# tberriel/OVO

Hardware: AMD Instinct MI355X
Metric: frames/s (CLIP+SAM2+fusion+query), 640x480 ScanNet, 1/2/4/8 MI355X (higher is better)
Workload: dtype bf16; 1 GPU; BASELINE.json configs[2]: PE-Core-L14-336 TextRegion descriptors (2 x 336^2 crops of a 640x480 frame) + SAM2 hiera_b+ image encoder @1024^2 + back-projection + cull/project/match/vote on a 1000000-point map + multi-view fusion + dense per-point fusion + 10-prompt instance and dense-map query; every frame a keyframe; masks from the precomputed-mask seam (32/frame); map_points=1000000, texts=10, masks_per_frame=32, sam2=image encoder, masks=precomputed-mask seam (mask_generator.py:94-95), encoder_batch=14, dense_query=resident class map, rows touched by the keyframe re-evaluated, parallelism=single GPU, points_end=1366868, instances_end=242

## Files before the change

include/ovo_hip.h:

```cpp
#ifndef OVO_HIP_H
#define OVO_HIP_H

#include <stddef.h>
#include <stdint.h>

#ifdef __cplusplus
extern "C" {
#endif

#define OVO_OK 0
#define OVO_E_ARG (-1)
#define OVO_E_LAUNCH (-2)
#define OVO_E_UNSUPPORTED (-3)

typedef void *ovo_stream_t;

const char *ovo_hip_last_error(void);
int ovo_hip_abi_version(void);

int ovo_marker(int id, ovo_stream_t stream);
int ovo_profile_start(void);
int ovo_profile_stop(double *ms, double *work, int64_t *launches, int n_kinds);
int ovo_profile_bytes(double *bytes, int n_kinds);

// ... 91 lines not shown
} ovo_gemm_t;
int ovo_gemm(const ovo_gemm_t *g, ovo_stream_t stream);
typedef struct {
    const float *cos, *sin;
    int32_t T, hd, cols, t0;
} ovo_rope_t;
int ovo_gemm_rope(const ovo_gemm_t *g, const ovo_rope_t *rope, ovo_stream_t stream);
int ovo_gemm_periodic(const ovo_gemm_t *g, int64_t add_rows, ovo_stream_t stream);
typedef struct {
    int32_t B, H, W, wh, ww;
} ovo_window_t;
int ovo_gemm_unwindow(const ovo_gemm_t *g, const ovo_window_t *win, ovo_stream_t stream);
int ovo_gemm_rowln(const ovo_gemm_t *g, const ovo_window_t *win, const float *ln_g, const float *ln_b, float eps, void *ln_out, int64_t ld_ln,
                   ovo_stream_t stream);
int ovo_gemm_fold_out(const ovo_gemm_t *g, void *xb, int64_t ld_xb, float *stats, int64_t ld_stats, ovo_stream_t stream);
int ovo_gemm_fold_stats(const float *x, int64_t ldx, int M, int D, void *xb, int64_t ld_xb, float *stats, ovo_stream_t stream);
int ovo_gemm_fold_in(const ovo_gemm_t *g, const ovo_rope_t *rope, const float *stats, int64_t ld_stats, int parts, int D, const float *rowsum, float eps,
                     ovo_stream_t stream);
int ovo_gemm_f32a(const ovo_gemm_t *g, const ovo_window_t *win, const float *x, int d, const float *gamma, const float *beta,
                  float eps, int mode, int pool2x2, ovo_stream_t stream);
int ovo_mlp_f32(float *x, int64_t rows, int d, const float *ln_g, const float *ln_b, float eps, const void *w1, int64_t ldw1,
                const float *b1, int hidden, const void *w2, int64_t ldw2, const float *b2, ovo_stream_t stream);
int ovo_neck_f32(const float *x, int64_t rows, int d, const void *w1, int64_t ldw1, const float *b1, int hidden, const void *w2, int64_t ldw2,
                 const float *b2, float *out, int n_out, ovo_stream_t stream);
int ovo_window_attention_f32(const float *x, int B, int H, int W, int window, int d, int d_out, int heads, int pool, const float *ln_g,
                             const float *ln_b, float eps, const void *qkv_w, int64_t ldw, const float *qkv_b, void *att, int ld_att,
                             ovo_stream_t stream);
int ovo_gemm_argmax(const ovo_gemm_t *g, uint64_t *best, int store_scores, int n_valid, ovo_stream_t stream);
int ovo_decode_best(const uint64_t *best, int64_t n, float th, int64_t *out_cls, float *out_conf, ovo_stream_t stream);

typedef struct {
    const void *q, *k, *v;
    void *o;
    int64_t q_sb, q_sh, q_st, k_sb, k_sh, k_st, v_sb, v_sh, v_st, o_sb, o_sh, o_st;
    int32_t B, H, Tq, Tk, hd;
    float scale;
    int32_t causal;
} ovo_attention_t;
int ovo_attention(const ovo_attention_t *a, ovo_stream_t stream);

int ovo_gemm_fewrows(const ovo_gemm_t *g, ovo_stream_t stream);
int ovo_attention_short(const void *qkv, int B, int T, int H, int hd, float scale, void *out, ovo_stream_t stream);
int ovo_merge_clips(const float *logits, int64_t ld_logits, int per_row, const float *clips, int B, int D, float *out, ovo_stream_t stream);

int ovo_layernorm(const float *x, int64_t x_stride, int64_t rows, int d, const float *gamma, const float *beta,
                  float eps, void *y, int64_t y_stride, int out_dtype, ovo_stream_t stream);

int ovo_vit_embed(const float *patch, const float *prefix, int n_prefix, const float *pos, int B, int P, int d,
                  const float *gamma, const float *beta, float eps, float *x, ovo_stream_t stream);

int ovo_im2col(const float *img, int B, int C, int H, int W, int ksz, int stride, int pad, void *out, int kpad,
               ovo_stream_t stream);

int ovo_resize_normalize(const void *src, int src_dtype, int C, int H, int W, int y0, int x0, int ch, int cw,
                         float *out, int oh, int ow, int antialias, float scale, const float *mean3_host,
                         const float *std3_host, ovo_stream_t stream);

int ovo_resize_window_normalize(const void *src, int src_dtype, int C, int H, int W, int y0, int x0, int ch, int cw, float *out,
                                int oh, int ow, int virt_h, int virt_w, int top, int left, int filter, float scale,
                                const float *mean3_host, const float *std3_host, ovo_stream_t stream);
int ovo_resize_normalize_batch(const void *const *srcs_host, int n_src, int src_dtype, int C, int H, int W, const int32_t *crops_host, int n_crop,
                               float *out, int oh, int ow, int antialias, float scale, const float *mean3_host, const float *std3_host,
                               ovo_stream_t stream);

int ovo_mask_boxes(const uint8_t *masks, int n, int H, int W, int32_t *boxes_xywh, ovo_stream_t stream);
int ovo_mask_crops(const void *image, int img_dtype, int H, int W, const uint8_t *masks, const int32_t *boxes_xywh, int n,
                   int also_bbox, int margin, int R, int round_out, float *out, ovo_stream_t stream);

int ovo_rope_qk(void *qkv, int B, int T, int H, int hd, const float *cos_t, const float *sin_t, int t0,
                ovo_stream_t stream);

int ovo_feature_masks(const uint8_t *masks, int N, int H, int W, int gh, int gw, void *w, int gpad, float *cnt,
                      ovo_stream_t stream);

int ovo_stitch_tokens_t(const float *tokens, int tokens_per_crop, int t0, int d, int P, int nh, int nw, void *out,
                        int gpad, ovo_stream_t stream);

int ovo_unit_tokens(const void *x_t, int d, int G, int gpad, void *u_t, void *u, ovo_stream_t stream);
int ovo_global_patch_filter(const float *r_t, void *weights, int N, int G, int gpad, float th, float *cnt, ovo_stream_t stream);

int ovo_scale_rows_bf16(const float *x, const float *cnt, int N, int d, void *y, ovo_stream_t stream);
int ovo_l2_normalize_rows(const float *x, int64_t N, int d, float *y, ovo_stream_t stream);
int ovo_cast_f32(const float *x, int64_t n, void *y, int dtype, ovo_stream_t stream);

typedef struct {
    int32_t image_size, patch, width, layers, heads, mlp_dim, out_dim;
    int32_t n_prefix;
    int32_t act;
    int32_t pre_ln;
    int32_t use_rope;
    int32_t pool;
    int32_t kpad;
    float ln_eps;
    int32_t q_prescaled;
} ovo_vit_config_t;

typedef struct {
    const float *ln1_g, *ln1_b;
    const void *qkv_w; const float *qkv_b;
    const void *out_w; const float *out_b;
    const float *ln2_g, *ln2_b;
    const void *fc1_w; const float *fc1_b;
    const void *fc2_w; const float *fc2_b;
    const void *qkv_wf; const float *qkv_bf, *qkv_cs;
    const void *fc1_wf; const float *fc1_bf, *fc1_cs;
} ovo_vit_layer_t;

typedef struct {
    const void *patch_w; const float *patch_b;
    const float *prefix;
    const float *pos;
    const float *ln_pre_g, *ln_pre_b, *ln_post_g, *ln_post_b;
    const void *proj_w;
    const float *rope_cos, *rope_sin;
    const ovo_vit_layer_t *layers;
    const void *map_q;
    const void *map_kv_w; const float *map_kv_b;
    const void *map_proj_w; const float *map_proj_b;
    const float *map_ln_g, *map_ln_b;
    const void *map_fc1_w; const float *map_fc1_b;
    const void *map_fc2_w; const float *map_fc2_b;
} ovo_vit_weights_t;

size_t ovo_vit_workspace_bytes(const ovo_vit_config_t *cfg, int B);
int ovo_vit_forward(const ovo_vit_config_t *cfg, const ovo_vit_weights_t *w, const float *images, int B, float *out,
                    void *ws, size_t ws_bytes, ovo_stream_t stream);

typedef struct {
    int32_t image_size;
    int32_t dims[4], heads[4], blocks[4], window[4];
    int32_t n_global, global_blocks[8];
    int32_t fpn_dim;
    int32_t hi_res;
    float ln_eps;
    int32_t q_prescaled;
} ovo_hiera_config_t;

typedef struct {
    const float *ln1_g, *ln1_b;
    const void *qkv_w; const float *qkv_b;
    const void *out_w; const float *out_b;
    const float *ln2_g, *ln2_b;
    const void *fc1_w; const float *fc1_b;
    const void *fc2_w; const float *fc2_b;
    const void *res_w; const float *res_b;
} ovo_hiera_block_t;

typedef struct {
    const void *patch_w; const float *patch_b;
    const float *pos;
    const ovo_hiera_block_t *blocks;
    const void *neck_w[4]; const float *neck_b[4];
    const void *s0_w; const float *s0_b;
    const void *s1_w; const float *s1_b;
} ovo_hiera_weights_t;

size_t ovo_hiera_workspace_bytes(const ovo_hiera_config_t *cfg, int B);
int ovo_hiera_patch_embed(const float *images, int B, int S, int E, const void *patch_w, int ldw, const float *bias, const float *pos,
                          float *x, ovo_stream_t stream);
int ovo_hiera_forward(const ovo_hiera_config_t *cfg, const ovo_hiera_weights_t *w, const float *images, int B,
                      float *feat0, float *feat1, float *feat2, void *ws, size_t ws_bytes, ovo_stream_t stream);


int ovo_row_epilogue(const float *x, int64_t R, int C, const float *base, int64_t base_rows, const float *gamma, const float *beta,
                     float eps, const float *pe, int64_t pe_rows, float *y, void *y16, void *ype16, ovo_stream_t stream);

int ovo_sam_upscale_ln(const void *g, const float *bias, const float *feat, const float *gamma, const float *beta, float eps,
                       int64_t P, int s, int C1, void *out, ovo_stream_t stream);

int ovo_sam_upscale_masks(const void *g, const float *bias, const float *feat, const float *hyper, int n_mask, int first, int64_t P,
                          int s2, int C2, float *out, ovo_stream_t stream);

int ovo_sam_linear(const void *A, const void *W, const float *bias, const float *add, int64_t add_rows, int ld_add, void *C, int ldc, int64_t M,
                   int N, int K, ovo_stream_t stream);
int ovo_sam_proj_ln(const void *A, const void *W, const float *bias, const float *res, const void *res16, int64_t res_rows, const float *gamma, const float *beta,
                    float eps, const float *pe, int64_t pe_rows, float *y32, void *y16, void *ype16, int64_t M, int N, int K, ovo_stream_t stream);
int ovo_sam_up1_ln(const void *A, const void *W, const float *bias, const float *feat, const float *gamma, const float *beta, float eps,
                   int64_t P, int s, int C1, int K, void *out, ovo_stream_t stream);
int ovo_sam_up2_masks(const void *A, const void *W, const float *bias, const float *feat, const float *hyper, int n_mask, int first, int64_t P,
                      int s2, int C2, int K, float *out, ovo_stream_t stream);

int ovo_sam_i2t_attention(const void *q, int64_t q_batch_stride, int q_token_stride, const void *k, const void *v, void *o, int64_t P, int S, int T,
                          int H, float scale, ovo_stream_t stream);
int ovo_sam_t2i_attention(const void *q, const void *k, const void *v, int64_t kv_batch_stride, int kv_token_stride, void *o, int64_t P, int S, int T,
                          int H, float scale, ovo_stream_t stream);

int ovo_amg_mask_stats(const float *logits, int n, int h, int w, int H, int W, float thr, float offset, int32_t *stats,
                       ovo_stream_t stream);
int ovo_amg_binarize(const float *logits, const int32_t *sel, int n_sel, int h, int w, int H, int W, float thr, uint8_t *out,
                     ovo_stream_t stream);
int ovo_paint_segmap(const uint8_t *masks, int n, int64_t pixels, int32_t *seg, ovo_stream_t stream);


int ovo_instance_moments(const float *xyz, const int32_t *ins, int64_t n, int n_slots, double *sums, int32_t *cnt, ovo_stream_t stream);

int ovo_near_fraction(const float *pts_by_instance, const int64_t *offsets, const int32_t *pairs, int n_pairs, int64_t max_points_a,
                      float th, int32_t *near_count, ovo_stream_t stream);

int ovo_remap_instances(int32_t *ins, int64_t n, const int32_t *table, int n_slots, ovo_stream_t stream);

size_t ovo_map_reanchor_workspace_bytes(int K);
int ovo_map_reanchor(const float *xyz, const int32_t *ids, const int32_t *ins, const uint8_t *rgb, int64_t n_src, float *xyz_out, int32_t *ids_out,
                     int32_t *ins_out, uint8_t *rgb_out, int64_t cap_out, const int64_t *seg_src_host, const int64_t *seg_dst_host,
                     const float *seg_T_host, int K, void *ws, size_t ws_bytes, ovo_stream_t stream);

size_t ovo_dense_repack_workspace_bytes(int K);
int ovo_dense_repack(const float *acc, const int32_t *cnt, const int64_t *cls, const float *conf, int D, int src_shards, int64_t src_rows_local,
                     int64_t n_src, float *acc_out, int32_t *cnt_out, int64_t *cls_out, float *conf_out, int64_t rows_out, int shard_rank,
                     int shard_count, int shard_block, int64_t n_fill, int64_t empty_cls, float empty_conf, const int64_t *seg_src_host,
                     const int64_t *seg_dst_host, int K, void *ws, size_t ws_bytes, ovo_stream_t stream);

typedef struct {
    float w2c[16];
    float K[9];
// ... 122 lines not shown
```

ovo_amd/_lib.py:

```python
from __future__ import annotations

import ctypes as C
import os
from typing import Optional

import torch

_HERE = os.path.dirname(os.path.abspath(__file__))
SO_PATH = os.path.join(_HERE, "lib", "libovo_hip.so")
ABI_VERSION = 20
E_UNSUPPORTED = -3


class OvoHipError(RuntimeError):
    pass


class Camera(C.Structure):
    _fields_ = [("aabb", C.c_float * 6), ("planes", C.c_float * 24), ("w2c", C.c_float * 16),
                ("K", C.c_float * 9), ("th", C.c_float), ("h", C.c_int32), ("w", C.c_int32)]


class Ratio(C.Structure):
    _fields_ = [("enabled", C.c_int32), ("r_h", C.c_float), ("r_w", C.c_float), ("crop_edge", C.c_int32)]


_P, _I64, _I32, _F32, _SZ = C.c_void_p, C.c_int64, C.c_int, C.c_float, C.c_size_t
_CAM = C.POINTER(Camera)


class Gemm(C.Structure):
    _fields_ = [("A", _P), ("lda", _I64), ("W", _P), ("ldw", _I64), ("bias", _P), ("C", _P), ("ldc", _I64),
                ("add", _P), ("ld_add", _I64), ("M", C.c_int32), ("N", C.c_int32), ("K", C.c_int32),
                ("in_dtype", C.c_int32), ("out_dtype", C.c_int32), ("act", C.c_int32), ("alpha", _F32)]


class Rope(C.Structure):
    _fields_ = [("cos", _P), ("sin", _P), ("T", C.c_int32), ("hd", C.c_int32), ("cols", C.c_int32), ("t0", C.c_int32)]


class Window(C.Structure):
    _fields_ = [(n, C.c_int32) for n in ("B", "H", "W", "wh", "ww")]


class Attention(C.Structure):
    _fields_ = [("q", _P), ("k", _P), ("v", _P), ("o", _P)] + \
               [(n, _I64) for n in ("q_sb", "q_sh", "q_st", "k_sb", "k_sh", "k_st", "v_sb", "v_sh", "v_st", "o_sb", "o_sh", "o_st")] + \
               [(n, C.c_int32) for n in ("B", "H", "Tq", "Tk", "hd")] + [("scale", _F32), ("causal", C.c_int32)]


class VitConfig(C.Structure):
    _fields_ = [(n, C.c_int32) for n in ("image_size", "patch", "width", "layers", "heads", "mlp_dim", "out_dim", "n_prefix",
                                          "act", "pre_ln", "use_rope", "pool", "kpad")] + [("ln_eps", _F32), ("q_prescaled", C.c_int32)]


class VitLayer(C.Structure):
    _fields_ = [(n, _P) for n in ("ln1_g", "ln1_b", "qkv_w", "qkv_b", "out_w", "out_b", "ln2_g", "ln2_b",
                                   "fc1_w", "fc1_b", "fc2_w", "fc2_b",
                                   "qkv_wf", "qkv_bf", "qkv_cs", "fc1_wf", "fc1_bf", "fc1_cs")]


class VitWeights(C.Structure):
    _fields_ = [(n, _P) for n in ("patch_w", "patch_b", "prefix", "pos", "ln_pre_g", "ln_pre_b", "ln_post_g", "ln_post_b",
# ... 72 lines not shown
    "ovo_frustum_ids": (_I32, [_P, _I64, _CAM, _P, _P, _P, _SZ, _P]),
    "ovo_project_points": (_I32, [_P, _I64, _I32, _CAM, _P, _P]),
    "ovo_match_points": (_I32, [_P, _I64, _I32, _CAM, _P, _P, _P, _P, _P, _SZ, _P]),
    "ovo_depth_filter": (_I32, [_P, _I32, _I32, _I32, _F32, _F32, _P, _P]),
    "ovo_track_project": (_I32, [_P, _P, _I64, _CAM, _P, _P, _I32, _I32, Ratio, _P, _P, _I32, _I32, _P, _P]),
    "ovo_vote_stats": (_I32, [_P, _I32, _I32, _P, _I64, _P, _P]),
    "ovo_assign_instances": (_I32, [_P, _P, _I64, _P, _I32, _P, _P, _P]),
    "ovo_map_explained": (_I32, [_P, _I64, _CAM, _P, _P, _P]),
    "ovo_map_backproject": (_I32, [_P, _P, _P, _I32, _I32, _I32, _I32, _P, _P, _I64, _I32, _P, _P, _P, _P, _P, _P, _SZ, _P]),
    "ovo_map_step": (_I32, [C.POINTER(MapStep), _P]),
    "ovo_track_step": (_I32, [C.POINTER(TrackStep), _P]),
    "ovo_track_workspace_bytes": (_SZ, [_I32, _I32]),
    "ovo_keyframe_step": (_I32, [C.POINTER(MapStep), C.POINTER(TrackStep), _P]),
    "ovo_round_chain_params_bytes": (_SZ, []),
    "ovo_round_chain": (_I32, [C.POINTER(RoundChain), C.POINTER(MapStep), C.POINTER(TrackStep), _I32, _P]),
    "ovo_host_alloc": (_P, [_SZ]),
    "ovo_host_free": (None, [_P]),
    "ovo_host_wait32": (_I32, [_P, C.c_int32, _I64]),
    "ovo_host_wait64": (_I32, [_P, _I64, _I64]),
    "ovo_fuse_views": (_I32, [_P, _I32, _P, _P, _I32, _I32, _P, _P, _P, _P]),
    "ovo_fuse_views_add": (_I32, [_P, _I32, _P, _P, _P, _I32, _P, _P, _P, _P]),
    "ovo_scatter_accum": (_I32, [_P, _I64, _P, _I32, _P, _I32, _P, _P, _P]),
    "ovo_similarity": (_I32, [_P, _I32, _I64, _I32, _P, _I32, _P, _I32, _F32, _F32, _F32, _P, _P, _P, _P]),
    "ovo_similarity_rows": (_I32, [_P, _I32, _P, _P, _I64, _I32, _P, _I32, _P, _I32, _F32, _F32, _F32, _P, _P, _P]),
    "ovo_scatter_accum_touched": (_I32, [_P, _I64, _P, _I32, _P, _I32, _P, _P, _P, _P, _P, _I32, _I32, _I32, _P]),
    "ovo_scatter_accum_query": (_I32, [_P, _P, _I64, _P, _P, _I32, _P, _I32, _P, _P, _I32, _I32, _I32, _P, _I32, _I32, _F32, _F32, _F32, _P, _P, _P]),
    "ovo_mask_boxes": (_I32, [_P, _I32, _I32, _I32, _P, _P]),
    "ovo_mask_crops": (_I32, [_P, _I32, _I32, _I32, _P, _P, _I32, _I32, _I32, _I32, _I32, _P, _P]),
    "ovo_row_argmax": (_I32, [_P, _I64, _I32, _I32, _F32, _F32, _F32, _P, _P, _P]),
    "ovo_mask_intersections": (_I32, [_P, _I32, _I64, _P, _P]),
    "ovo_pack_masks": (_I32, [_P, _I32, _I64, _P, _I64, _P]),
    "ovo_unpack_masks": (_I32, [_P, _I32, _I64, _I64, _P, _P]),
    "ovo_mask_or": (_I32, [_P, _I64, _P, _I32, _P]),
    "ovo_gather_rows": (_I32, [_P, _I64, _P, _I32, _P, _P]),
    "ovo_mask_area": (_I32, [_P, _I64, _P, _I32, _P, _P]),
    "ovo_gemm": (_I32, [C.POINTER(Gemm), _P]),
    "ovo_gemm_argmax": (_I32, [C.POINTER(Gemm), _P, _I32, _I32, _P]),
    "ovo_gemm_rope": (_I32, [C.POINTER(Gemm), C.POINTER(Rope), _P]),
    "ovo_gemm_periodic": (_I32, [C.POINTER(Gemm), _I64, _P]),
    "ovo_gemm_unwindow": (_I32, [C.POINTER(Gemm), C.POINTER(Window), _P]),
    "ovo_gemm_fold_out": (_I32, [C.POINTER(Gemm), _P, _I64, _P, _I64, _P]),
    "ovo_gemm_fold_stats": (_I32, [_P, _I64, _I32, _I32, _P, _I64, _P, _P]),
    "ovo_gemm_fold_in": (_I32, [C.POINTER(Gemm), C.POINTER(Rope), _P, _I64, _I32, _I32, _P, _F32, _P]),
    "ovo_gemm_rowln": (_I32, [C.POINTER(Gemm), C.POINTER(Window), _P, _P, _F32, _P, _I64, _P]),
    "ovo_gemm_f32a": (_I32, [C.POINTER(Gemm), C.POINTER(Window), _P, C.c_int, _P, _P, C.c_float, C.c_int, C.c_int, _P]),
    "ovo_decode_best": (_I32, [_P, _I64, _F32, _P, _P, _P]),
    "ovo_attention": (_I32, [C.POINTER(Attention), _P]),
    "ovo_gemm_fewrows": (_I32, [C.POINTER(Gemm), _P]),
    "ovo_attention_short": (_I32, [_P, _I32, _I32, _I32, _I32, _F32, _P, _P]),
    "ovo_merge_clips": (_I32, [_P, _I64, _I32, _P, _I32, _I32, _P, _P]),
    "ovo_layernorm": (_I32, [_P, _I64, _I64, _I32, _P, _P, _F32, _P, _I64, _I32, _P]),
    "ovo_vit_embed": (_I32, [_P, _P, _I32, _P, _I32, _I32, _I32, _P, _P, _F32, _P, _P]),
    "ovo_im2col": (_I32, [_P, _I32, _I32, _I32, _I32, _I32, _I32, _I32, _P, _I32, _P]),
    "ovo_resize_normalize": (_I32, [_P, _I32, _I32, _I32, _I32, _I32, _I32, _I32, _I32, _P, _I32, _I32, _I32, _F32,
                                    C.POINTER(C.c_float), C.POINTER(C.c_float), _P]),
    "ovo_resize_normalize_batch": (_I32, [_P, _I32, _I32, _I32, _I32, _I32, _P, _I32, _P, _I32, _I32, _I32, _F32, _P, _P, _P]),
    "ovo_resize_window_normalize": (_I32, [_P, _I32, _I32, _I32, _I32, _I32, _I32, _I32, _I32, _P, _I32, _I32, _I32, _I32, _I32, _I32, _I32, _F32,
                                           C.POINTER(C.c_float), C.POINTER(C.c_float), _P]),
    "ovo_rope_qk": (_I32, [_P, _I32, _I32, _I32, _I32, _P, _P, _I32, _P]),
    "ovo_feature_masks": (_I32, [_P, _I32, _I32, _I32, _I32, _I32, _P, _I32, _P, _P]),
    "ovo_stitch_tokens_t": (_I32, [_P, _I32, _I32, _I32, _I32, _I32, _I32, _P, _I32, _P]),
    "ovo_unit_tokens": (_I32, [_P, _I32, _I32, _I32, _P, _P, _P]),
    "ovo_global_patch_filter": (_I32, [_P, _P, _I32, _I32, _I32, _F32, _P, _P]),
    "ovo_scale_rows_bf16": (_I32, [_P, _P, _I32, _I32, _P, _P]),
    "ovo_mlp_f32": (_I32, [_P, _I64, _I32, _P, _P, _F32, _P, _I64, _P, _I32, _P, _I64, _P, _P]),
    "ovo_neck_f32": (_I32, [_P, _I64, _I32, _P, _I64, _P, _I32, _P, _I64, _P, _P, _I32, _P]),
    "ovo_window_attention_f32": (_I32, [_P, _I32, _I32, _I32, _I32, _I32, _I32, _I32, _I32, _P, _P, _F32, _P, _I64, _P, _P, _I32, _P]),
    "ovo_l2_normalize_rows": (_I32, [_P, _I64, _I32, _P, _P]),
    "ovo_cast_f32": (_I32, [_P, _I64, _P, _I32, _P]),
    "ovo_row_epilogue": (_I32, [_P, _I64, _I32, _P, _I64, _P, _P, _F32, _P, _I64, _P, _P, _P, _P]),
    "ovo_sam_upscale_ln": (_I32, [_P, _P, _P, _P, _P, _F32, _I64, _I32, _I32, _P, _P]),
    "ovo_sam_upscale_masks": (_I32, [_P, _P, _P, _P, _I32, _I32, _I64, _I32, _I32, _P, _P]),
    "ovo_sam_linear": (_I32, [_P, _P, _P, _P, _I64, _I32, _P, _I32, _I64, _I32, _I32, _P]),
    "ovo_sam_proj_ln": (_I32, [_P, _P, _P, _P, _P, _I64, _P, _P, _F32, _P, _I64, _P, _P, _P, _I64, _I32, _I32, _P]),
    "ovo_sam_up1_ln": (_I32, [_P, _P, _P, _P, _P, _P, _F32, _I64, _I32, _I32, _I32, _P, _P]),
    "ovo_sam_up2_masks": (_I32, [_P, _P, _P, _P, _P, _I32, _I32, _I64, _I32, _I32, _I32, _P, _P]),
    "ovo_instance_moments": (_I32, [_P, _P, _I64, _I32, _P, _P, _P]),
    "ovo_near_fraction": (_I32, [_P, _P, _P, _I32, _I64, _F32, _P, _P]),
    "ovo_remap_instances": (_I32, [_P, _I64, _P, _I32, _P]),
    "ovo_map_reanchor_workspace_bytes": (_SZ, [_I32]),
    "ovo_map_reanchor": (_I32, [_P, _P, _P, _P, _I64, _P, _P, _P, _P, _I64, _P, _P, _P, _I32, _P, _SZ, _P]),
    "ovo_dense_repack_workspace_bytes": (_SZ, [_I32]),
    "ovo_dense_repack": (_I32, [_P, _P, _P, _P, _I32, _I32, _I64, _I64, _P, _P, _P, _P, _I64, _I32, _I32, _I32, _I64, _I64, _F32, _P, _P, _I32, _P, _SZ, _P]),
    "ovo_render_workspace_bytes": (_SZ, [_I32, _I32]),
    "ovo_render_points": (_I32, [_P, _I64, C.POINTER(View), _P, _P, _P, _SZ, _P]),
    "ovo_render_resolve": (_I32, [_P, _I32, _I32, _I64, _P, _P, C.c_uint32, _P, _P, _P, _P, _I32, _I64, _F32, _P, _P, _P, _P, _P, _P, _P]),
    "ovo_instance_geometry": (_I32, [_P, _P, _I64, _I32, _P, _P, _P, _P, _P, _P, _P]),
    "ovo_render_boxes_workspace_bytes": (_SZ, [_I32]),
    "ovo_render_boxes": (_I32, [_P, _P, _I32, C.POINTER(View), _F32, _P, _F32, _P, _P, _P, _SZ, _P]),
    "ovo_icp_pyramid_bytes": (_SZ, [_I32, _I32, _I32]),
    "ovo_icp_prepare": (_I32, [_P, C.POINTER(IcpFrame), _P, _SZ, _P]),
    "ovo_icp_align_workspace_bytes": (_SZ, []),
    "ovo_icp_align": (_I32, [_P, C.POINTER(IcpFrame), _P, C.POINTER(IcpFrame), C.POINTER(IcpAlign), _P, _P, _P, _SZ, _P]),
    "ovo_sam_i2t_attention": (_I32, [_P, _I64, _I32, _P, _P, _P, _I64, _I32, _I32, _I32, _F32, _P]),
    "ovo_sam_t2i_attention": (_I32, [_P, _P, _P, _I64, _I32, _P, _I64, _I32, _I32, _I32, _F32, _P]),
    "ovo_paint_segmap": (_I32, [_P, _I32, _I64, _P, _P]),
    "ovo_amg_mask_stats": (_I32, [_P, _I32, _I32, _I32, _I32, _I32, _F32, _F32, _P, _P]),
    "ovo_amg_binarize": (_I32, [_P, _P, _I32, _I32, _I32, _I32, _I32, _F32, _P, _P]),
    "ovo_vit_workspace_bytes": (_SZ, [C.POINTER(VitConfig), _I32]),
    "ovo_vit_forward": (_I32, [C.POINTER(VitConfig), C.POINTER(VitWeights), _P, _I32, _P, _P, _SZ, _P]),
    "ovo_hiera_workspace_bytes": (_SZ, [C.POINTER(HieraConfig), _I32]),
    "ovo_hiera_forward": (_I32, [C.POINTER(HieraConfig), C.POINTER(HieraWeights), _P, _I32, _P, _P, _P, _P, _SZ, _P]),
    "ovo_hiera_patch_embed": (_I32, [_P, _I32, _I32, _I32, _P, _I32, _P, _P, _P, _P]),
    "ovo_eval_cell_keys": (_I32, [_P, _I64, C.POINTER(EvalGrid), _P, _P]),
    "ovo_eval_grid_records": (_I32, [_P, _P, _I64, _P, _P]),
    "ovo_knn5_labels": (_I32, [_P, _P, _I64, C.POINTER(EvalGrid), _P, _P, _I64, _P, _P, _P, _P, _P, _P]),
    "ovo_confusion": (_I32, [_P, _P, _I64, _I32, C.POINTER(C.c_int64), _I32, _P, _P, _P]),
}

_lib: Optional[C.CDLL] = None


def exported_symbols():
    return sorted(_SIGNATURES)


def load() -> C.CDLL:
    global _lib
    if _lib is not None:
        return _lib
    if not os.path.exists(SO_PATH):
        raise OvoHipError(f"{SO_PATH} is missing: run `python -m ovo_amd.build` (needs hipcc). "
                          "ovo_amd has no CPU fallback.")
    lib = C.CDLL(SO_PATH)
    for name, (res, args) in _SIGNATURES.items():
        fn = getattr(lib, name)
        fn.restype, fn.argtypes = res, args
    if lib.ovo_hip_abi_version() != ABI_VERSION:
        raise OvoHipError(f"ABI mismatch: library {lib.ovo_hip_abi_version()} vs binding {ABI_VERSION}")
    _lib = lib
    return lib


def check(status: int) -> None:
    if status != 0:
        raise OvoHipError(f"libovo_hip error {status}: {load().ovo_hip_last_error().decode()}")


_raw_stream = getattr(torch._C, "_cuda_getCurrentRawStream", None)


def stream() -> C.c_void_p:
    if _raw_stream is not None:
        return C.c_void_p(_raw_stream(torch.cuda.current_device()))
    return C.c_void_p(torch.cuda.current_stream().cuda_stream)


def ptr(t: Optional[torch.Tensor]) -> C.c_void_p:
    if t is None:
        return C.c_void_p(0)
    return C.c_void_p(t.data_ptr())


def dev(t: torch.Tensor, dtype: torch.dtype, name: str = "tensor") -> torch.Tensor:
    if not t.is_cuda:
        raise OvoHipError(f"{name} must live on the GPU (got {t.device}); ovo_amd has no CPU path")
# ... 128 lines not shown
```

ovo_amd/csrc/core.hip:

```cpp
#include <stdarg.h>
#include <stdio.h>
#include <stdlib.h>

#include <string.h>

#include <atomic>
#include <chrono>
#include <vector>

#include "common.h"

static thread_local char g_err[512] = "";

void ovo_set_error(const char *fmt, ...) {
    va_list ap;
    va_start(ap, fmt);
    vsnprintf(g_err, sizeof(g_err), fmt, ap);
    va_end(ap);
}

namespace {
struct Rec { hipEvent_t a, b; int kind; double work, bytes; int shape[3], flags; int cslot; double per_item, fixed; };
struct Prof {
    bool on = false;
// ... 20 lines not shown
void ovo_prof_shape(int a, int b, int c) {
    if (!g_prof.on || g_prof.recs.empty()) return;
    Rec &r = g_prof.recs.back();
    r.shape[0] = a; r.shape[1] = b; r.shape[2] = c;
}
void ovo_prof_flags(int flags) {
    if (!g_prof.on || g_prof.recs.empty()) return;
    g_prof.recs.back().flags = flags;
}
void ovo_prof_bytes(double bytes) {
    if (!g_prof.on || g_prof.recs.empty()) return;
    g_prof.recs.back().bytes = bytes;
}
static double g_last_bytes[OVO_PROF_KINDS];
void ovo_prof_end(hipStream_t s) {
    if (!g_prof.on || g_prof.recs.empty()) return;
    (void)hipEventRecord(g_prof.recs.back().b, s);
}
void ovo_prof_count(const int32_t *device_count, double per_item, double fixed, hipStream_t s) {
    constexpr int SLOTS = 1 << 16;
    if (!g_prof.on || g_prof.recs.empty() || !device_count) return;
    if (!g_prof.counts && hipHostMalloc((void **)&g_prof.counts, SLOTS * sizeof(int32_t), hipHostMallocDefault) != hipSuccess) { g_prof.counts = nullptr; return; }
    if (g_prof.n_counts >= SLOTS) return;
    Rec &r = g_prof.recs.back();
    r.cslot = g_prof.n_counts++; r.per_item = per_item; r.fixed = fixed;
    (void)hipMemcpyAsync(g_prof.counts + r.cslot, device_count, sizeof(int32_t), hipMemcpyDeviceToHost, s);
}

template <typename T>
static int host_wait(const T *flag, T value, int64_t timeout_us) {
    OVO_REQUIRE(flag, "null flag");
    const volatile T *f = flag;
    const auto t0 = std::chrono::steady_clock::now();
    for (unsigned spin = 0;; ++spin) {
        if (*f == value) { std::atomic_thread_fence(std::memory_order_acquire); return OVO_OK; }
        if ((spin & 255) == 255 &&
            std::chrono::duration_cast<std::chrono::microseconds>(std::chrono::steady_clock::now() - t0).count() > timeout_us) {
            ovo_set_error("ovo_host_wait: timed out after %lld us (flag %lld, expected %lld)", (long long)timeout_us, (long long)*f, (long long)value);
            return OVO_E_LAUNCH;
        }
        __builtin_ia32_pause();
    }
}

__global__ void k_marker(int id, int *sink) { if (sink && id < 0) *sink = id; }

extern "C" {
int ovo_marker(int id, ovo_stream_t stream) {
    k_marker<<<1, 1, 0, (hipStream_t)stream>>>(id, nullptr);
    OVO_CHECK_LAUNCH();
    return OVO_OK;
}
const char *ovo_hip_last_error(void) { return g_err; }
int ovo_hip_abi_version(void) { return 20; }

int ovo_profile_start(void) {
    g_prof.recs.clear();
    g_prof.used = 0;
    g_prof.n_counts = 0;
    g_prof.on = true;
    return OVO_OK;
}

int ovo_profile_stop(double *ms, double *work, int64_t *launches, int n_kinds) {
    g_prof.on = false;
    OVO_REQUIRE(ms && work && launches && n_kinds > 0 && n_kinds <= OVO_PROF_KINDS, "bad argument");
    for (int i = 0; i < n_kinds; ++i) { ms[i] = 0; work[i] = 0; launches[i] = 0; }
    for (int i = 0; i < OVO_PROF_KINDS; ++i) g_last_bytes[i] = 0;
    OVO_HIP(hipDeviceSynchronize());
    FILE *dump = getenv("OVO_PROF_DUMP") ? fopen(getenv("OVO_PROF_DUMP"), "a") : nullptr;
    for (const Rec &r : g_prof.recs) {
        float t = 0.f;
        if (hipEventElapsedTime(&t, r.a, r.b) != hipSuccess || r.kind >= n_kinds) continue;
        double wk = r.work, by = r.bytes;
        if (r.cslot >= 0 && g_prof.counts) wk = by = r.per_item * (double)g_prof.counts[r.cslot] + r.fixed;
        ms[r.kind] += t; work[r.kind] += wk; launches[r.kind] += 1; g_last_bytes[r.kind] += by;
        if (dump) fprintf(dump, "%d %d %d %d %.0f %.4f %d\n", r.kind, r.shape[0], r.shape[1], r.shape[2], wk, t, r.flags);
    }
    if (dump) fclose(dump);
    g_prof.recs.clear();
    g_prof.used = 0;
    return OVO_OK;
}

int ovo_profile_bytes(double *bytes, int n_kinds) {
    OVO_REQUIRE(bytes && n_kinds > 0 && n_kinds <= OVO_PROF_KINDS, "bad argument");
    for (int i = 0; i < n_kinds; ++i) bytes[i] = g_last_bytes[i];
    return OVO_OK;
}

void *ovo_host_alloc(size_t bytes) {
    void *p = nullptr;
    if (hipHostMalloc(&p, bytes ? bytes : 1, hipHostMallocMapped | hipHostMallocCoherent) != hipSuccess) {
        ovo_set_error("ovo_host_alloc: hipHostMalloc(%zu) failed", bytes);
        return nullptr;
    }
    memset(p, 0, bytes);
    return p;
}
void ovo_host_free(void *p) { if (p) (void)hipHostFree(p); }

int ovo_host_wait32(const int32_t *flag, int32_t value, int64_t timeout_us) { return host_wait(flag, value, timeout_us); }
int ovo_host_wait64(const int64_t *flag, int64_t value, int64_t timeout_us) { return host_wait(flag, value, timeout_us); }
}
```

ovo_amd/csrc/encoder.hip:

```cpp
#include <hip/hip_fp16.h>

#include "common.h"

namespace {

__device__ __forceinline__ float bf2f(uint16_t v) { return __uint_as_float((uint32_t)v << 16); }
__device__ __forceinline__ uint16_t f2bf(float x) {
    const __bf16 h = (__bf16)x;
    return *(const uint16_t *)&h;
}
__device__ __forceinline__ uint2 pack4_bf16(float a, float b, float c, float d) {
    return make_uint2((uint32_t)f2bf(a) | ((uint32_t)f2bf(b) << 16), (uint32_t)f2bf(c) | ((uint32_t)f2bf(d) << 16));
}

__device__ __forceinline__ void ln_row_wide(const float *__restrict__ x, int d, const float *__restrict__ gamma,
                                            const float *__restrict__ beta, float eps, void *__restrict__ y, int out_bf16, int lane,
                                            const float *__restrict__ extra_add) {
    const int d4 = d >> 2;
    float s = 0.f;
    for (int i = lane; i < d4; i += 64) {
        float4 v = ((const float4 *)x)[i];
        if (extra_add) { const float4 e = ((const float4 *)extra_add)[i]; v.x += e.x; v.y += e.y; v.z += e.z; v.w += e.w; }
        s += (v.x + v.y) + (v.z + v.w);
    }
    const float mean = wave_sum(s) / (float)d;
    float q = 0.f;
    for (int i = lane; i < d4; i += 64) {
        float4 v = ((const float4 *)x)[i];
        if (extra_add) { const float4 e = ((const float4 *)extra_add)[i]; v.x += e.x; v.y += e.y; v.z += e.z; v.w += e.w; }
        const float a = v.x - mean, b = v.y - mean, c = v.z - mean, e2 = v.w - mean;
        q += (a * a + b * b) + (c * c + e2 * e2);
    }
    const float rstd = rsqrtf(wave_sum(q) / (float)d + eps);
    for (int i = lane; i < d4; i += 64) {
        float4 v = ((const float4 *)x)[i];
        if (extra_add) { const float4 e = ((const float4 *)extra_add)[i]; v.x += e.x; v.y += e.y; v.z += e.z; v.w += e.w; }
        const float4 g = ((const float4 *)gamma)[i], b = ((const float4 *)beta)[i];
        const float o0 = (v.x - mean) * rstd * g.x + b.x, o1 = (v.y - mean) * rstd * g.y + b.y;
        const float o2 = (v.z - mean) * rstd * g.z + b.z, o3 = (v.w - mean) * rstd * g.w + b.w;
        if (out_bf16) ((uint2 *)y)[i] = pack4_bf16(o0, o1, o2, o3);
        else ((float4 *)y)[i] = make_float4(o0, o1, o2, o3);
    }
}

template <int NV>
__device__ __forceinline__ void ln_row_regs(const float *__restrict__ x, int d, const float *__restrict__ gamma,
                                            const float *__restrict__ beta, float eps, void *__restrict__ y, int out_bf16, int lane,
                                            const float *__restrict__ extra_add) {
    const int d4 = d >> 2;
    float4 v[NV];
#pragma unroll
    for (int j = 0; j < NV; ++j) {
        const int i = lane + 64 * j;
        v[j] = i < d4 ? ((const float4 *)x)[i] : make_float4(0.f, 0.f, 0.f, 0.f);
    }
// ... 20 lines not shown
#pragma unroll
    for (int j = 0; j < NV; ++j) {
        const int i = lane + 64 * j;
        if (i < d4) {
            const float4 g = ((const float4 *)gamma)[i], b = ((const float4 *)beta)[i];
            const float o0 = (v[j].x - mean) * rstd * g.x + b.x, o1 = (v[j].y - mean) * rstd * g.y + b.y;
            const float o2 = (v[j].z - mean) * rstd * g.z + b.z, o3 = (v[j].w - mean) * rstd * g.w + b.w;
            if (out_bf16) ((uint2 *)y)[i] = pack4_bf16(o0, o1, o2, o3);
            else ((float4 *)y)[i] = make_float4(o0, o1, o2, o3);
        }
    }
}

__device__ __forceinline__ void ln_row(const float *__restrict__ x, int d, const float *__restrict__ gamma,
                                       const float *__restrict__ beta, float eps, void *__restrict__ y, int out_bf16, int lane,
                                       const float *__restrict__ extra_add = nullptr) {
    const int nv = ((d >> 2) + 63) >> 6;
    if (nv <= 2) ln_row_regs<2>(x, d, gamma, beta, eps, y, out_bf16, lane, extra_add);
    else if (nv <= 4) ln_row_regs<4>(x, d, gamma, beta, eps, y, out_bf16, lane, extra_add);
    else if (nv <= 8) ln_row_regs<8>(x, d, gamma, beta, eps, y, out_bf16, lane, extra_add);
    else ln_row_wide(x, d, gamma, beta, eps, y, out_bf16, lane, extra_add);
}

__global__ void __launch_bounds__(256) k_layernorm(const float *__restrict__ x, long long xs, long long rows, int d,
                                                   const float *__restrict__ gamma, const float *__restrict__ beta, float eps,
                                                   char *__restrict__ y, long long ys, int out_bf16) {
    const int lane = threadIdx.x & 63;
    const long long waves = (long long)gridDim.x * 4;
    for (long long r = (long long)blockIdx.x * 4 + (threadIdx.x >> 6); r < rows; r += waves)
        ln_row(x + r * xs, d, gamma, beta, eps, y + r * ys * (out_bf16 ? 2 : 4), out_bf16, lane);
}

__global__ void __launch_bounds__(256) k_vit_embed(const float *__restrict__ patch, const float *__restrict__ prefix, int n_prefix,
                                                   const float *__restrict__ pos, int B, int P, int d, const float *__restrict__ gamma,
                                                   const float *__restrict__ beta, float eps, float *__restrict__ x) {
    const int lane = threadIdx.x & 63;
    const int T = n_prefix + P;
    const long long rows = (long long)B * T, waves = (long long)gridDim.x * 4;
    for (long long r = (long long)blockIdx.x * 4 + (threadIdx.x >> 6); r < rows; r += waves) {
        const int b = (int)(r / T), t = (int)(r % T);
        const float *src = t < n_prefix ? prefix + (long long)t * d : patch + ((long long)b * P + (t - n_prefix)) * d;
        const float *pe = pos ? pos + (long long)t * d : nullptr;
        float *dst = x + r * d;
        if (gamma) ln_row(src, d, gamma, beta, eps, dst, 0, lane, pe);
        else
            for (int i = lane; i < (d >> 2); i += 64) {
                float4 v = ((const float4 *)src)[i];
                if (pe) { const float4 e = ((const float4 *)pe)[i]; v.x += e.x; v.y += e.y; v.z += e.z; v.w += e.w; }
                ((float4 *)dst)[i] = v;
            }
    }
}

__global__ void __launch_bounds__(256) k_im2col(const float *__restrict__ img, int B, int C, int H, int W, int ksz, int stride, int pad,
                                                int oh, int ow, uint16_t *__restrict__ out, int kpad) {
    const uint32_t k8 = (uint32_t)kpad >> 3;
    const uint32_t total = (uint32_t)B * oh * ow * k8;
    const int kk = ksz * ksz, kreal = C * kk;
    for (uint32_t i = blockIdx.x * blockDim.x + threadIdx.x; i < total; i += gridDim.x * blockDim.x) {
        const uint32_t row = i / k8, kb = (i - row * k8) * 8;
        const uint32_t t1 = row / (uint32_t)ow, ox = row - t1 * (uint32_t)ow;
        const uint32_t b = t1 / (uint32_t)oh, oy = t1 - b * (uint32_t)oh;
        int c = (int)(kb / (uint32_t)kk), rem = (int)kb - c * kk, ky = rem / ksz, kx = rem - ky * ksz;
        const int y0 = (int)oy * stride - pad, x0 = (int)ox * stride - pad;
        uint16_t v[8];
#pragma unroll
        for (int e = 0; e < 8; ++e) {
            float f = 0.f;
            if ((int)kb + e < kreal) {
                const int y = y0 + ky, x = x0 + kx;
                if (y >= 0 && y < H && x >= 0 && x < W) f = img[(((long long)b * C + c) * H + y) * W + x];
            }
            v[e] = f2bf(f);
            if (++kx == ksz) { kx = 0; if (++ky == ksz) { ky = 0; ++c; } }
        }
        uint4 p;
        p.x = v[0] | ((uint32_t)v[1] << 16); p.y = v[2] | ((uint32_t)v[3] << 16); p.z = v[4] | ((uint32_t)v[5] << 16); p.w = v[6] | ((uint32_t)v[7] << 16);
        *(uint4 *)(out + (long long)row * kpad + kb) = p;
    }
}

struct ResizeArgs {
    const void *src; int src_u8, hwc; int C, H, W, y0, x0, ch, cw, oh, ow, aa;
    int vh, vw, top, left;
    float scale, mean[4], std[4];
};
__device__ __forceinline__ float src_px(const ResizeArgs &a, int c, int y, int x) {
    const long long i = a.hwc ? ((long long)(a.y0 + y) * a.W + (a.x0 + x)) * a.C + c : ((long long)c * a.H + (a.y0 + y)) * a.W + (a.x0 + x);
    return a.src_u8 ? (float)((const uint8_t *)a.src)[i] : ((const float *)a.src)[i];
}
typedef uint32_t __attribute__((aligned(1))) u32_unaligned;
__device__ __forceinline__ void src_px_all(const ResizeArgs &a, int y, int x, float (&v)[4]) {
    if (a.hwc && a.src_u8 && a.C == 3) {
        const long long i = ((long long)(a.y0 + y) * a.W + (a.x0 + x)) * 3;
        const uint8_t *p = (const uint8_t *)a.src + i;
        if (i + 4 <= (long long)a.H * a.W * 3) {
            const uint32_t w = *(const u32_unaligned *)p;
            v[0] = (float)(w & 0xffu); v[1] = (float)((w >> 8) & 0xffu); v[2] = (float)((w >> 16) & 0xffu);
        } else { v[0] = (float)p[0]; v[1] = (float)p[1]; v[2] = (float)p[2]; }
        return;
    }
    for (int c = 0; c < a.C; ++c) v[c] = src_px(a, c, y, x);
}
__device__ __forceinline__ float tri(float x) { x = fabsf(x); return x < 1.f ? 1.f - x : 0.f; }
__device__ __forceinline__ float cubic_aa(float x) {
    x = fabsf(x);
    if (x < 1.f) return ((1.5f * x - 2.5f) * x) * x + 1.f;
    if (x < 2.f) return (((x - 5.f) * x + 8.f) * x - 4.f) * -0.5f;
    return 0.f;
}
__device__ __forceinline__ float aa_filter(int kind, float x) { return kind == 2 ? cubic_aa(x) : tri(x); }

template <int T>
__device__ __forceinline__ void aa_taps(const ResizeArgs &a, int ymin, int xmin, int ny, int nx, float cy, float cx, float ivy, float ivx, float wy_tot,
                                        float wx_tot, float (&v)[4]) {
    float wy[T], wx[T];
#pragma unroll
    for (int i = 0; i < T; ++i) {
        wy[i] = i < ny ? aa_filter(a.aa, ((float)(ymin + i) - cy + 0.5f) * ivy) / wy_tot : 0.f;
        wx[i] = i < nx ? aa_filter(a.aa, ((float)(xmin + i) - cx + 0.5f) * ivx) / wx_tot : 0.f;
    }
#pragma unroll
    for (int iy = 0; iy < T; ++iy) {
        if (iy >= ny) break;
        float rowacc[4] = {0.f, 0.f, 0.f, 0.f};
#pragma unroll
        for (int ix = 0; ix < T; ++ix) {
            if (ix >= nx) break;
            float px[4];
            src_px_all(a, ymin + iy, xmin + ix, px);
            for (int c = 0; c < a.C; ++c) rowacc[c] += wx[ix] * px[c];
        }
        for (int c = 0; c < a.C; ++c) v[c] += wy[iy] * rowacc[c];
    }
}

#define OVO_RS_TAPS 10
__device__ __forceinline__ void resize_norm_body(const ResizeArgs &a, float *__restrict__ out) {
    const int wx_ = blockIdx.x * 64 + (threadIdx.x & 63), wy_ = blockIdx.y * 4 + (threadIdx.x >> 6);
    if (wx_ >= a.ow || wy_ >= a.oh) return;
    const int ox = wx_ + a.left, oy = wy_ + a.top;
    const float sy = (float)a.ch / (float)a.vh, sx = (float)a.cw / (float)a.vw;
    float v[4] = {0.f, 0.f, 0.f, 0.f};
    if (!a.aa) {
        float fy = sy * ((float)oy + 0.5f) - 0.5f; fy = fy < 0.f ? 0.f : fy;
        float fx = sx * ((float)ox + 0.5f) - 0.5f; fx = fx < 0.f ? 0.f : fx;
        const int y0 = (int)fy, x0 = (int)fx;
        const int y1 = y0 + (y0 < a.ch - 1 ? 1 : 0), x1 = x0 + (x0 < a.cw - 1 ? 1 : 0);
        const float ly = fy - (float)y0, lx = fx - (float)x0;
        float p00[4], p01[4], p10[4], p11[4];
        src_px_all(a, y0, x0, p00); src_px_all(a, y0, x1, p01); src_px_all(a, y1, x0, p10); src_px_all(a, y1, x1, p11);
        for (int c = 0; c < a.C; ++c)
            v[c] = (1.f - ly) * ((1.f - lx) * p00[c] + lx * p01[c]) + ly * ((1.f - lx) * p10[c] + lx * p11[c]);
    } else {
        const float half = a.aa == 2 ? 2.f : 1.f;
        const float supy = (sy >= 1.f ? sy : 1.f) * half, supx = (sx >= 1.f ? sx : 1.f) * half;
        const float ivy = sy >= 1.f ? 1.f / sy : 1.f, ivx = sx >= 1.f ? 1.f / sx : 1.f;
        const float cy = sy * ((float)oy + 0.5f), cx = sx * ((float)ox + 0.5f);
        int ymin = (int)(cy - supy + 0.5f); ymin = ymin < 0 ? 0 : ymin;
        int ymax = (int)(cy + supy + 0.5f); ymax = ymax > a.ch ? a.ch : ymax;
        int xmin = (int)(cx - supx + 0.5f); xmin = xmin < 0 ? 0 : xmin;
        int xmax = (int)(cx + supx + 0.5f); xmax = xmax > a.cw ? a.cw : xmax;
        float wy_tot = 0.f, wx_tot = 0.f;
        for (int y = ymin; y < ymax; ++y) wy_tot += aa_filter(a.aa, ((float)y - cy + 0.5f) * ivy);
        for (int x = xmin; x < xmax; ++x) wx_tot += aa_filter(a.aa, ((float)x - cx + 0.5f) * ivx);
        const int ny = ymax - ymin, nx = xmax - xmin;
        const int bound = (int)(2.f * (supy > supx ? supy : supx)) + 1;
        if (bound <= 3 && ny <= 3 && nx <= 3) aa_taps<3>(a, ymin, xmin, ny, nx, cy, cx, ivy, ivx, wy_tot, wx_tot, v);
        else if (bound <= 6 && ny <= 6 && nx <= 6) aa_taps<6>(a, ymin, xmin, ny, nx, cy, cx, ivy, ivx, wy_tot, wx_tot, v);
        else if (ny <= OVO_RS_TAPS && nx <= OVO_RS_TAPS) {
            aa_taps<OVO_RS_TAPS>(a, ymin, xmin, ny, nx, cy, cx, ivy, ivx, wy_tot, wx_tot, v);
        } else {
            for (int c = 0; c < a.C; ++c) {
                float acc = 0.f;
                for (int y = ymin; y < ymax; ++y) {
                    const float wyy = aa_filter(a.aa, ((float)y - cy + 0.5f) * ivy) / wy_tot;
                    float rowacc = 0.f;
                    for (int x = xmin; x < xmax; ++x) rowacc += (aa_filter(a.aa, ((float)x - cx + 0.5f) * ivx) / wx_tot) * src_px(a, c, y, x);
                    acc += wyy * rowacc;
                }
                v[c] = acc;
            }
        }
    }
    for (int c = 0; c < a.C; ++c) out[((long long)c * a.oh + wy_) * a.ow + wx_] = (v[c] * a.scale - a.mean[c]) / a.std[c];
}
__global__ void __launch_bounds__(256) k_resize_norm(ResizeArgs a, float *__restrict__ out) { resize_norm_body(a, out); }

constexpr int RESIZE_BATCH_MAX = 64;
struct ResizeBatch { const void *src[RESIZE_BATCH_MAX]; int y0[RESIZE_BATCH_MAX], x0[RESIZE_BATCH_MAX], ch[RESIZE_BATCH_MAX], cw[RESIZE_BATCH_MAX]; };
__global__ void __launch_bounds__(256) k_resize_norm_batch(ResizeArgs a, ResizeBatch b, float *__restrict__ out) {
    const int z = blockIdx.z;
    a.src = b.src[z]; a.y0 = b.y0[z]; a.x0 = b.x0[z]; a.ch = b.ch[z]; a.cw = b.cw[z];
    resize_norm_body(a, out + (long long)z * a.C * a.oh * a.ow);
}

template <int T>
__global__ void __launch_bounds__(256) k_resize_tri_hwc3(ResizeArgs a, ResizeBatch b, float *__restrict__ out) {
    const int z = blockIdx.z;
    const uint8_t *src = (const uint8_t *)b.src[z];
    const int y0c = b.y0[z], x0c = b.x0[z], ch = b.ch[z], cw = b.cw[z];
    const int wx_ = blockIdx.x * 64 + (threadIdx.x & 63), wy_ = blockIdx.y * 4 + (threadIdx.x >> 6);
    if (wx_ >= a.ow || wy_ >= a.oh) return;
    const int ox = wx_ + a.left, oy = wy_ + a.top;
    const float sy = (float)ch / (float)a.vh, sx = (float)cw / (float)a.vw;
    const float supy = sy >= 1.f ? sy : 1.f, supx = sx >= 1.f ? sx : 1.f;
    const float ivy = sy >= 1.f ? 1.f / sy : 1.f, ivx = sx >= 1.f ? 1.f / sx : 1.f;
    const float cy = sy * ((float)oy + 0.5f), cx = sx * ((float)ox + 0.5f);
    int ymin = (int)(cy - supy + 0.5f); ymin = ymin < 0 ? 0 : ymin;
    int ymax = (int)(cy + supy + 0.5f); ymax = ymax > ch ? ch : ymax;
    int xmin = (int)(cx - supx + 0.5f); xmin = xmin < 0 ? 0 : xmin;
    int xmax = (int)(cx + supx + 0.5f); xmax = xmax > cw ? cw : xmax;
    float wy[T], wx[T], wy_tot = 0.f, wx_tot = 0.f;
#pragma unroll
    for (int i = 0; i < T; ++i) {
        wy[i] = ymin + i < ymax ? tri(((float)(ymin + i) - cy + 0.5f) * ivy) : 0.f;
        wx[i] = xmin + i < xmax ? tri(((float)(xmin + i) - cx + 0.5f) * ivx) : 0.f;
        wy_tot += wy[i]; wx_tot += wx[i];
    }
#pragma unroll
    for (int i = 0; i < T; ++i) { wy[i] = wy[i] / wy_tot; wx[i] = wx[i] / wx_tot; }
    const long long last = (long long)a.H * a.W * 3 - 4;
    float v0 = 0.f, v1 = 0.f, v2 = 0.f;
#pragma unroll
    for (int iy = 0; iy < T; ++iy) {
        int y = ymin + iy; y = y < ch - 1 ? y : ch - 1;
        const long long row = (long long)(y0c + y) * a.W + x0c;
        float r0 = 0.f, r1 = 0.f, r2 = 0.f;
#pragma unroll
        for (int ix = 0; ix < T; ++ix) {
            int x = xmin + ix; x = x < cw - 1 ? x : cw - 1;
            const long long off = (row + x) * 3;
            uint32_t w;
            if (off <= last) w = *(const u32_unaligned *)(src + off);
            else w = (uint32_t)src[off] | ((uint32_t)src[off + 1] << 8) | ((uint32_t)src[off + 2] << 16);
            r0 += wx[ix] * (float)(w & 0xffu); r1 += wx[ix] * (float)((w >> 8) & 0xffu); r2 += wx[ix] * (float)((w >> 16) & 0xffu);
        }
        v0 += wy[iy] * r0; v1 += wy[iy] * r1; v2 += wy[iy] * r2;
    }
    float *o = out + (long long)z * 3 * a.oh * a.ow + (long long)wy_ * a.ow + wx_;
    const long long plane = (long long)a.oh * a.ow;
    o[0] = (v0 * a.scale - a.mean[0]) / a.std[0];
    o[plane] = (v1 * a.scale - a.mean[1]) / a.std[1];
    o[2 * plane] = (v2 * a.scale - a.mean[2]) / a.std[2];
}
inline int resize_tap_bound(int ch, int cw, int vh, int vw) {
    const float sy = (float)ch / (float)vh, sx = (float)cw / (float)vw;
    const float supy = sy >= 1.f ? sy : 1.f, supx = sx >= 1.f ? sx : 1.f;
    return (int)(2.f * (supy > supx ? supy : supx)) + 1;
}
inline void launch_resize_batch(const ResizeArgs &a, const ResizeBatch &b, int nz, float *out, hipStream_t s) {
    dim3 grid((a.ow + 63) / 64, (a.oh + 3) / 4, nz);
    int bound = 0;
    for (int z = 0; z < nz; ++z) { const int t = resize_tap_bound(b.ch[z], b.cw[z], a.vh, a.vw); bound = t > bound ? t : bound; }
    const bool generic = ovo_knob_set("OVO_RESIZE_GENERIC");
    if (!generic && a.hwc && a.src_u8 && a.C == 3 && a.aa == 1 && bound <= 3) k_resize_tri_hwc3<3><<<grid, 256, 0, s>>>(a, b, out);
    else if (!generic && a.hwc && a.src_u8 && a.C == 3 && a.aa == 1 && bound <= 6) k_resize_tri_hwc3<6><<<grid, 256, 0, s>>>(a, b, out);
    else k_resize_norm_batch<<<grid, 256, 0, s>>>(a, b, out);
}

__global__ void __launch_bounds__(256) k_mask_boxes(const uint8_t *__restrict__ masks, int H, int W, int32_t *__restrict__ boxes) {
    __shared__ int s[4];
    if (threadIdx.x == 0) { s[0] = W; s[1] = H; s[2] = -1; s[3] = -1; }
    __syncthreads();
    const uint8_t *m = masks + (long long)blockIdx.x * H * W;
    int x0 = W, y0 = H, x1 = -1, y1 = -1;
    for (int i = threadIdx.x; i < H * W; i += blockDim.x) {
        if (m[i]) {
            const int y = i / W, x = i - y * W;
            x0 = x < x0 ? x : x0; x1 = x > x1 ? x : x1; y0 = y < y0 ? y : y0; y1 = y > y1 ? y : y1;
        }
    }
    if (x1 >= 0) { atomicMin(&s[0], x0); atomicMin(&s[1], y0); atomicMax(&s[2], x1); atomicMax(&s[3], y1); }
    __syncthreads();
    if (threadIdx.x == 0) {
        int32_t *b = boxes + 4 * blockIdx.x;
        if (s[2] < 0) { b[0] = b[1] = b[2] = b[3] = 0; }
        else { b[0] = s[0]; b[1] = s[1]; b[2] = s[2] - s[0]; b[3] = s[3] - s[1]; }
    }
}

struct CropArgs {
    const void *img; int img_u8, H, W;
    const uint8_t *masks; const int32_t *boxes;
    int n, also_bbox, margin, R, round_out;
};
__global__ void __launch_bounds__(256) k_mask_crops(CropArgs a, float *__restrict__ out) {
    const int ox = blockIdx.x * 64 + (threadIdx.x & 63), oy = blockIdx.y * 4 + (threadIdx.x >> 6);
    const int parts = a.also_bbox ? 2 : 1, i = blockIdx.z / parts, part = blockIdx.z % parts;
    if (ox >= a.R || oy >= a.R) return;
    const int32_t *b = a.boxes + 4 * i;
    int bx = b[0], by = b[1], bw = b[2], bh = b[3];
    int ch, cw, offy = 0, offx = 0;
    const uint8_t *mask = nullptr;
    if (part == 0) {
        mask = a.masks + (long long)i * a.H * a.W;
        if (a.also_bbox) { ch = bh; cw = bw; }
        else {
            ch = cw = bh > bw ? bh : bw;
            if (bh > bw) offx = (bh - bw) / 2; else offy = (bw - bh) / 2;
        }
    } else {
        bx -= a.margin; by -= a.margin; bw += 2 * a.margin; bh += 2 * a.margin;
        if (bx < 0) { bw += bx; bx = 0; }
        if (by < 0) { bh += by; by = 0; }
        if (bx + bw > a.W) bw = a.W - bx;
        if (by + bh > a.H) bh = a.H - by;
        ch = bh; cw = bw;
    }
    float *o = out + ((long long)(i * parts + part) * 3) * a.R * a.R + (long long)oy * a.R + ox;
    const long long plane = (long long)a.R * a.R;
// ... 178 lines not shown

__global__ void __launch_bounds__(256) k_cast(const float4 *__restrict__ x, long long n4, uint2 *__restrict__ y, int dtype) {
    for (long long i = (long long)blockIdx.x * blockDim.x + threadIdx.x; i < n4; i += (long long)gridDim.x * blockDim.x) {
        const float4 v = x[i];
        if (dtype == 2) y[i] = pack4_bf16(v.x, v.y, v.z, v.w);
        else {
            const __half2 a = __floats2half2_rn(v.x, v.y), b = __floats2half2_rn(v.z, v.w);
            y[i] = make_uint2(*(const uint32_t *)&a, *(const uint32_t *)&b);
        }
    }
}

}

extern "C" {

int ovo_layernorm(const float *x, int64_t x_stride, int64_t rows, int d, const float *gamma, const float *beta, float eps,
                  void *y, int64_t y_stride, int out_dtype, ovo_stream_t stream) {
    OVO_REQUIRE(rows >= 0 && d > 0 && d % 4 == 0, "d must be a multiple of 4");
    OVO_REQUIRE(out_dtype == 0 || out_dtype == 2, "out_dtype: 0 = f32, 2 = bf16");
    if (rows == 0) return OVO_OK;
    OVO_REQUIRE(x && gamma && beta && y && x_stride % 4 == 0 && y_stride % 4 == 0, "null pointer / misaligned stride");
    k_layernorm<<<ovo_grid(rows * 64, 256), 256, 0, (hipStream_t)stream>>>(x, x_stride, rows, d, gamma, beta, eps, (char *)y,
                                                                          y_stride, out_dtype == 2);
    OVO_CHECK_LAUNCH();
    return OVO_OK;
}

int ovo_vit_embed(const float *patch, const float *prefix, int n_prefix, const float *pos, int B, int P, int d,
                  const float *gamma, const float *beta, float eps, float *x, ovo_stream_t stream) {
    OVO_REQUIRE(patch && x && B > 0 && P > 0 && d > 0 && d % 4 == 0 && n_prefix >= 0, "bad argument");
    OVO_REQUIRE(n_prefix == 0 || prefix, "prefix tokens missing");
    OVO_REQUIRE((gamma == nullptr) == (beta == nullptr), "gamma and beta go together");
    k_vit_embed<<<ovo_grid((long long)B * (n_prefix + P) * 64, 256), 256, 0, (hipStream_t)stream>>>(patch, prefix, n_prefix, pos, B, P, d,
                                                                                                    gamma, beta, eps, x);
    OVO_CHECK_LAUNCH();
    return OVO_OK;
}

int ovo_im2col(const float *img, int B, int C, int H, int W, int ksz, int stride, int pad, void *out, int kpad,
               ovo_stream_t stream) {
    OVO_REQUIRE(img && out && B > 0 && C > 0 && H > 0 && W > 0 && ksz > 0 && stride > 0 && pad >= 0, "bad argument");
    OVO_REQUIRE(kpad >= C * ksz * ksz && kpad % 32 == 0, "kpad must cover C*k*k and be a multiple of 32");
    const int oh = (H + 2 * pad - ksz) / stride + 1, ow = (W + 2 * pad - ksz) / stride + 1;
    OVO_REQUIRE(oh > 0 && ow > 0, "empty output");
    OVO_REQUIRE(kpad % 8 == 0 && ((uintptr_t)out & 15) == 0, "kpad must be a multiple of 8 and the output 16-byte aligned");
    OVO_REQUIRE((long long)B * oh * ow * (kpad / 8) < (1ll << 32) - (1ll << 22), "more than 2^32 16-byte pieces: split the batch");
    k_im2col<<<ovo_grid((long long)B * oh * ow * (kpad / 8), 256), 256, 0, (hipStream_t)stream>>>(img, B, C, H, W, ksz, stride, pad, oh, ow,
                                                                                                 (uint16_t *)out, kpad);
    OVO_CHECK_LAUNCH();
    return OVO_OK;
}

int ovo_resize_window_normalize(const void *src, int src_dtype, int C, int H, int W, int y0, int x0, int ch, int cw, float *out,
                                int oh, int ow, int virt_h, int virt_w, int top, int left, int filter, float scale,
                                const float *mean3_host, const float *std3_host, ovo_stream_t stream) {
    OVO_REQUIRE(src && out && (src_dtype == 0 || src_dtype == 3 || src_dtype == 4), "src_dtype: 0 = f32 [C,H,W], 3 = u8 [C,H,W], 4 = u8 [H,W,C]");
    OVO_REQUIRE(C >= 1 && C <= 4 && ch > 0 && cw > 0 && oh > 0 && ow > 0, "bad shape");
    OVO_REQUIRE(y0 >= 0 && x0 >= 0 && y0 + ch <= H && x0 + cw <= W, "crop outside the image");
    OVO_REQUIRE(top >= 0 && left >= 0 && top + oh <= virt_h && left + ow <= virt_w, "window outside the resized image");
    OVO_REQUIRE(filter >= 0 && filter <= 2, "filter: 0 = bilinear, 1 = antialiased bilinear, 2 = antialiased bicubic");
    ResizeArgs a;
    a.src = src; a.src_u8 = src_dtype >= 3; a.hwc = src_dtype == 4; a.C = C; a.H = H; a.W = W; a.y0 = y0; a.x0 = x0; a.ch = ch; a.cw = cw;
    a.oh = oh; a.ow = ow; a.aa = filter; a.scale = scale;
    a.vh = virt_h; a.vw = virt_w; a.top = top; a.left = left;
    for (int c = 0; c < 4; ++c) { a.mean[c] = mean3_host && c < C ? mean3_host[c] : 0.f; a.std[c] = std3_host && c < C ? std3_host[c] : 1.f; }
    if (a.hwc && a.src_u8 && C == 3 && filter == 1) {
        ResizeBatch b = {};
        b.src[0] = src; b.y0[0] = y0; b.x0[0] = x0; b.ch[0] = ch; b.cw[0] = cw;
        launch_resize_batch(a, b, 1, out, (hipStream_t)stream);
    } else {
        dim3 grid((ow + 63) / 64, (oh + 3) / 4);
        k_resize_norm<<<grid, 256, 0, (hipStream_t)stream>>>(a, out);
    }
    OVO_CHECK_LAUNCH();
    return OVO_OK;
}

int ovo_resize_normalize(const void *src, int src_dtype, int C, int H, int W, int y0, int x0, int ch, int cw, float *out,
                         int oh, int ow, int antialias, float scale, const float *mean3_host, const float *std3_host,
                         ovo_stream_t stream) {
    return ovo_resize_window_normalize(src, src_dtype, C, H, W, y0, x0, ch, cw, out, oh, ow, oh, ow, 0, 0, antialias, scale, mean3_host,
                                       std3_host, stream);
}

int ovo_resize_normalize_batch(const void *const *srcs_host, int n_src, int src_dtype, int C, int H, int W, const int32_t *crops_host, int n_crop, float *out,
                               int oh, int ow, int antialias, float scale, const float *mean3_host, const float *std3_host, ovo_stream_t stream) {
    OVO_REQUIRE(srcs_host && crops_host && out && n_src > 0 && n_crop > 0, "null / empty argument");
    OVO_REQUIRE(src_dtype == 0 || src_dtype == 3 || src_dtype == 4, "src_dtype: 0 = f32 [C,H,W], 3 = u8 [C,H,W], 4 = u8 [H,W,C]");
    OVO_REQUIRE(C >= 1 && C <= 4 && oh > 0 && ow > 0 && antialias >= 0 && antialias <= 2, "bad shape");
    ResizeArgs a;
    a.src = nullptr; a.src_u8 = src_dtype >= 3; a.hwc = src_dtype == 4; a.C = C; a.H = H; a.W = W; a.y0 = a.x0 = 0; a.ch = H; a.cw = W;
    a.oh = oh; a.ow = ow; a.aa = antialias; a.scale = scale; a.vh = oh; a.vw = ow; a.top = 0; a.left = 0;
    for (int c = 0; c < 4; ++c) { a.mean[c] = mean3_host && c < C ? mean3_host[c] : 0.f; a.std[c] = std3_host && c < C ? std3_host[c] : 1.f; }
    for (int k = 0; k < n_crop; ++k) {
        const int32_t *r = crops_host + 4 * k;
        OVO_REQUIRE(r[2] > 0 && r[3] > 0 && r[0] >= 0 && r[1] >= 0 && r[0] + r[2] <= H && r[1] + r[3] <= W, "crop outside the image");
    }
    const int total = n_src * n_crop;
    for (int z0 = 0; z0 < total; z0 += RESIZE_BATCH_MAX) {
        const int nz = total - z0 < RESIZE_BATCH_MAX ? total - z0 : RESIZE_BATCH_MAX;
        ResizeBatch b;
        for (int z = 0; z < nz; ++z) {
            const int i = (z0 + z) / n_crop, k = (z0 + z) % n_crop;
            OVO_REQUIRE(srcs_host[i], "null source image");
            b.src[z] = srcs_host[i]; b.y0[z] = crops_host[4 * k]; b.x0[z] = crops_host[4 * k + 1]; b.ch[z] = crops_host[4 * k + 2]; b.cw[z] = crops_host[4 * k + 3];
// ... 104 lines not shown
```

ovo_amd/csrc/hiera.hip:

```cpp
#include <algorithm>
#include "gemm_common.h"

namespace {

__device__ __forceinline__ uint16_t f2bf(float x) {
    const __bf16 h = (__bf16)x;
    return *(const uint16_t *)&h;
}
__device__ __forceinline__ float bf2f(uint16_t v) { return __uint_as_float((uint32_t)v << 16); }

struct Grid {
    int B, H, W, ws;
    int nwh, nww, wh, ww;
    long long rows;
};
__host__ __device__ inline Grid make_grid(int B, int H, int W, int ws) {
    Grid g; g.B = B; g.H = H; g.W = W; g.ws = ws;
    if (ws > 0) { g.wh = g.ww = ws; g.nwh = (H + ws - 1) / ws; g.nww = (W + ws - 1) / ws; }
    else { g.wh = H; g.ww = W; g.nwh = g.nww = 1; }
    g.rows = (long long)B * g.nwh * g.nww * g.wh * g.ww;
    return g;
}
__device__ __forceinline__ long long row_of(const Grid &g, int b, int y, int x) {
    const int wy = y / g.wh, wx = x / g.ww;
    return ((((long long)b * g.nwh + wy) * g.nww + wx) * g.wh + (y - wy * g.wh)) * g.ww + (x - wx * g.ww);
}

template <int LPR, int NV>
__global__ void __launch_bounds__(256) k_ln_window(const float *__restrict__ x, Grid g, int d, int kp, const float *__restrict__ gamma,
                                                   const float *__restrict__ beta, float eps, uint16_t *__restrict__ out) {
    constexpr int RPW = 64 / LPR;
    const int lane = threadIdx.x & 63, sl = lane % LPR, sub = lane / LPR;
    const uint32_t waves = gridDim.x * 4u;
    const int d4 = d >> 2, kp4 = kp >> 2;
    const uint32_t per_win = (uint32_t)(g.wh * g.ww), n_rows = (uint32_t)g.rows;
    const uint32_t n_iter = (n_rows + RPW - 1) / RPW;
    for (uint32_t it = blockIdx.x * 4u + (threadIdx.x >> 6); it < n_iter; it += waves) {
        uint32_t r = it * RPW + sub;
        if (LPR == 64) r = __builtin_amdgcn_readfirstlane(r);
        bool real = r < n_rows;
        const float *src = x;
        if (real) {
            const uint32_t win = r / per_win, in = r - win * per_win;
            const uint32_t ly = in / (uint32_t)g.ww, lx = in - ly * (uint32_t)g.ww;
            const uint32_t q2 = win / (uint32_t)g.nww, wx = win - q2 * (uint32_t)g.nww;
            const uint32_t b = q2 / (uint32_t)g.nwh, wy = q2 - b * (uint32_t)g.nwh;
            const int y = (int)(wy * g.wh + ly), xx = (int)(wx * g.ww + lx);
            if (y >= g.H || xx >= g.W) {
                uint2 *o = (uint2 *)(out + (long long)r * kp);
                for (int i = sl; i < kp4; i += LPR) o[i] = make_uint2(0, 0);
                real = false;
            } else src = x + (((long long)b * g.H + y) * g.W + xx) * d;
        }
        float4 v[NV];
// ... 154 lines not shown
}

inline int padk(int v) { return (v + 63) / 64 * 64; }
inline size_t align256(size_t v) { return (v + 255) & ~(size_t)255; }

struct BlockShape {
    int din, dout, kin, kout, heads, hd, H, Ho;
    bool pool; int stage_end;
    Grid g, go, gi;
    long long n_win, tok_out, att_rows; int tk, tq;
    size_t n_x, n_h, n_qkv, n_att, n_u, n_tmp, n_cast;
};
struct Plan {
    int n_blocks, S4;
    Grid level[2];
    size_t n_col, n_cast, n_lat[4];
    BlockShape b[64];
};

int make_plan(const ovo_hiera_config_t &c, int B, Plan &p) {
    int idx = 0, H = p.S4 = c.image_size / 4;
    const size_t tok0 = (size_t)B * H * H;
    p.level[0] = make_grid(B, H, H, 0); p.level[1] = make_grid(B, H / 2, H / 2, 0);
    p.n_col = tok0 * 192; p.n_cast = tok0 * c.fpn_dim;
    for (int s = 0; s < 4; ++s) p.n_lat[s] = (tok0 >> (2 * s)) * c.fpn_dim;
    for (int s = 0; s < 4; ++s)
        for (int b = 0; b < c.blocks[s]; ++b) {
            if (idx >= 64) return -1;
            BlockShape &k = p.b[idx];
            const bool first = k.pool = s > 0 && b == 0;
            k.din = first ? c.dims[s - 1] : c.dims[s]; k.dout = c.dims[s]; k.kin = padk(k.din); k.kout = padk(k.dout);
            k.heads = c.heads[s]; k.hd = k.heads > 0 ? k.dout / k.heads : 0;
            int ws = first ? c.window[s - 1] : c.window[s];
            for (int j = 0; j < c.n_global; ++j) if (c.global_blocks[j] == idx) ws = 0;
            k.H = H;
            k.Ho = H = first ? H / 2 : H;
            k.stage_end = b == c.blocks[s] - 1 ? s : -1;
            k.g = make_grid(B, k.H, k.H, ws); k.go = make_grid(B, H, H, ws > 0 ? (first ? ws / 2 : ws) : 0); k.gi = make_grid(B, H, H, 0);
            k.n_win = (long long)B * k.g.nwh * k.g.nww; k.tk = k.g.wh * k.g.ww; k.tq = first ? k.tk / 4 : k.tk;
            k.tok_out = (long long)B * H * H; k.att_rows = k.n_win * k.tq;
            const size_t rows = (size_t)k.g.rows, tin = (size_t)B * k.H * k.H, tout = (size_t)k.tok_out;
            k.n_x = std::max(tin * k.din, tout * k.dout);
            k.n_h = std::max(rows * k.kin, tout * k.kout);
            k.n_qkv = rows * 3 * k.dout; k.n_tmp = rows * k.dout;
            k.n_att = (first ? rows / 4 : rows) * k.kout;
            k.n_u = tout * 4 * k.dout; k.n_cast = tout * k.kout;
            ++idx;
        }
    p.n_blocks = idx;
    return 0;
}
struct Ws {
    uint16_t *col; float *x, *xr, *tmp; uint16_t *h, *qkv, *qp, *att, *u, *cast; float *lat[4];
    size_t bytes;
};

bool neck_fused(const ovo_hiera_config_t &c, int B, int s) {
    if (!c.hi_res || s > 1 || ovo_knob_set("OVO_HIERA_NECK_TWO_PASS")) return false;
    const long long rows = ((long long)B * (c.image_size / 4) * (c.image_size / 4)) >> (2 * s);
    return ovo_gemm_detail::neck_stream_covers(rows, c.dims[s], padk(c.dims[s]), c.fpn_dim, s == 0 ? 32 : 64);
}

Ws carve(const ovo_hiera_config_t &c, const Plan &p, int B, void *base) {
    size_t max_x = 0, max_h = 0, max_qkv = 0, max_att = 0, max_u = 0, max_tmp = 0, max_cast = p.n_cast;
    for (int i = 0; i < p.n_blocks; ++i) {
        const BlockShape &k = p.b[i];
        max_x = std::max(max_x, k.n_x); max_h = std::max(max_h, k.n_h); max_qkv = std::max(max_qkv, k.n_qkv); max_att = std::max(max_att, k.n_att);
        max_u = std::max(max_u, k.n_u); max_tmp = std::max(max_tmp, k.n_tmp); max_cast = std::max(max_cast, k.n_cast);
    }
    Ws w; size_t off = 0;
    auto take = [&](size_t n) { char *r = base ? (char *)base + off : nullptr; off += align256(n); return r; };
    w.col = (uint16_t *)take(p.n_col * 2); w.x = (float *)take(max_x * 4); w.xr = (float *)take(max_x * 4); w.tmp = (float *)take(max_tmp * 4);
    w.h = (uint16_t *)take(max_h * 2); w.qkv = (uint16_t *)take(max_qkv * 2);
    w.qp = (uint16_t *)take(max_att * 2); w.att = (uint16_t *)take(max_att * 2);
    w.u = (uint16_t *)take(max_u * 2); w.cast = (uint16_t *)take(max_cast * 2);
    for (int s = 0; s < 4; ++s) w.lat[s] = neck_fused(c, B, s) ? nullptr : (float *)take(p.n_lat[s] * 4);
    w.bytes = off;
    return w;
}

ovo_gemm_t gemm_desc(const void *A, long long lda, const void *W, long long ldw, const float *bias, void *C, long long ldc, int out_dtype,
                     const float *add, long long ld_add, long long M, int N, int K, int act) {
    ovo_gemm_t g;
    g.A = A; g.lda = lda; g.W = W; g.ldw = ldw; g.bias = bias; g.C = C; g.ldc = ldc; g.add = add; g.ld_add = ld_add;
    g.M = (int)M; g.N = N; g.K = K; g.in_dtype = 2; g.out_dtype = out_dtype; g.act = act; g.alpha = 1.0f;
    return g;
}
ovo_window_t window_of(const Grid &g) { return {g.B, g.H, g.W, g.wh, g.ww}; }

#define TRY(call) do { const int rc__ = (call); if (rc__ != OVO_OK) return rc__; } while (0)
#define TRY_FUSED(ran, call) \
    do { const int rc__ = (call); if (rc__ != OVO_OK && rc__ != OVO_E_UNSUPPORTED) return rc__; (ran) = rc__ == OVO_OK; } while (0)
#define LAUNCHED() OVO_CHECK_LAUNCH()

int gemm(const void *A, long long lda, const void *W, long long ldw, const float *bias, void *C, long long ldc, int out_dtype,
         const float *add, long long ld_add, long long M, int N, int K, int act, ovo_stream_t s) {
    const ovo_gemm_t g = gemm_desc(A, lda, W, ldw, bias, C, ldc, out_dtype, add, ld_add, M, N, K, act);
    return ovo_gemm(&g, s);
}

int gemm_from_f32(const float *x, const Grid &g, int d, int kp, const float *gamma, const float *beta, float eps, int mode, uint16_t *h, bool &h_done,
                  const void *W, const float *bias, void *C, long long ldc, int out_dtype, int N, int act, ovo_stream_t s) {
    const ovo_gemm_t q = gemm_desc(h, kp, W, kp, bias, C, ldc, out_dtype, nullptr, 0, g.rows, N, kp, act);
    if (!h_done) {
        const ovo_window_t w = window_of(g); bool streamed;
        TRY_FUSED(streamed, ovo_gemm_detail::gemm_f32a_stream(&q, g.ws > 0 ? &w : nullptr, x, d, gamma, beta, eps, mode, 0, s));
        if (streamed) return OVO_OK;
        OVO_REQUIRE(d <= 2048 && g.rows < (1ll << 31), "LayerNorm rows of more than 2048 columns / more than 2^31 rows");
        if (mode == 1) launch_ln_window(x, g, d, kp, gamma, beta, eps, h, (hipStream_t)s);
        else k_cast_pad<<<ovo_grid(g.rows * kp, 256), 256, 0, (hipStream_t)s>>>(x, g.rows, d, kp, h);
        h_done = true;
    }
    return ovo_gemm(&q, s);
}

constexpr int PE_TH = 8, PE_TW = 32, PE_IH = 4 * PE_TH + 3, PE_RS = 136, PE_WS = 200;
template <int NT>
__global__ void __launch_bounds__(512) __attribute__((amdgpu_waves_per_eu(4, 4))) k_patch_embed7(const float *__restrict__ img, int S, const uint16_t *__restrict__ w, int ldw,
                                                      const float *__restrict__ bias, const float *__restrict__ pos, float *__restrict__ out, int B,
                                                      int n_tiles) {
    using namespace ovo_gemm_detail;
    constexpr int E = 16 * NT;
    extern __shared__ __attribute__((aligned(16))) unsigned char pe_lds[];
    uint16_t *s_img = (uint16_t *)pe_lds;
    uint16_t *s_w = s_img + 3 * PE_IH * PE_RS;
    const int S4 = S >> 2, tiles_x = S4 / PE_TW, n_pos = tiles_x * (S4 / PE_TH);
    for (int i = threadIdx.x; i < E * 24; i += 512) {
        const int e = i / 24, r = i - 24 * e;
        uint4 p = make_uint4(0u, 0u, 0u, 0u);
        if (r < 21) {
            const uint16_t *q = w + (long long)e * ldw + 7 * r;
            const uint32_t w0 = q[0], w1 = q[1], w2 = q[2], w3 = q[3], w4 = q[4], w5 = q[5], w6 = q[6];
            p.x = w0 << 16; p.y = w1 | (w2 << 16); p.z = w3 | (w4 << 16); p.w = w5 | (w6 << 16);
        }
        *(uint4 *)(s_w + e * PE_WS + 8 * r) = p;
    }
    for (int i = threadIdx.x; i < 3 * PE_IH; i += 512) s_img[i * PE_RS] = 0;
    const int lane = threadIdx.x & 63, wave = threadIdx.x >> 6, g = lane >> 4, l16 = lane & 15;
    constexpr int NV = (3 * PE_IH * 32 + 511) / 512;
    float4 v[NV];
    float h;
    auto load_tile = [&](int t) {
        const int tt = t % n_pos, b = t / n_pos;
        const int oy0 = (tt / tiles_x) * PE_TH, ox0 = (tt % tiles_x) * PE_TW;
        const int y_first = 4 * oy0 - 3, x_first = 4 * ox0 - 3;
        const float *src = img + (long long)b * 3 * S * S;
        const float *col0 = src + 4 * ox0 + 4 * (threadIdx.x & 31);
#pragma unroll
        for (int j = 0; j < NV; ++j) {
            int row = (threadIdx.x >> 5) + 16 * j;
            if (row > 3 * PE_IH - 1) row = 3 * PE_IH - 1;
            const int c = row / PE_IH, y = y_first + (row - c * PE_IH);
            const int yc = y < 0 ? 0 : (y > S - 1 ? S - 1 : y);
            const float4 u = *(const float4 *)(col0 + (c * S + yc) * S);
            const bool ok = y == yc;
            v[j].x = ok ? u.x : 0.f; v[j].y = ok ? u.y : 0.f; v[j].z = ok ? u.z : 0.f; v[j].w = ok ? u.w : 0.f;
        }
        {
            int row = threadIdx.x / 3;
            const int col = threadIdx.x - 3 * row;
            if (row > 3 * PE_IH - 1) row = 3 * PE_IH - 1;
            const int c = row / PE_IH, y = y_first + (row - c * PE_IH), x = x_first + col;
            const int yc = y < 0 ? 0 : (y > S - 1 ? S - 1 : y), xc = x < 0 ? 0 : x;
            const float u = src[(c * S + yc) * S + xc];
            h = (y == yc && x == xc) ? u : 0.f;
        }
    };
    if ((int)blockIdx.x < n_tiles) load_tile(blockIdx.x);
    for (int t = blockIdx.x; t < n_tiles; t += gridDim.x) {
        const int tt = t % n_pos, b = t / n_pos;
        const int oy0 = (tt / tiles_x) * PE_TH, ox0 = (tt % tiles_x) * PE_TW;
        __syncthreads();
        f32x4 acc[2][NT];
#pragma unroll
        for (int m = 0; m < 2; ++m) {
            const long long tok = (long long)(oy0 + wave) * S4 + ox0 + 16 * m + l16;
#pragma unroll
            for (int n = 0; n < NT; ++n) acc[m][n] = *(const f32x4 *)(pos + tok * E + 16 * n + 4 * g);
        }
#pragma unroll
        for (int j = 0; j < NV; ++j) {
            const int row = (threadIdx.x >> 5) + 16 * j;
            if (16 * j + 15 < 3 * PE_IH || row < 3 * PE_IH) {
                uint2 p;
                p.x = f2bf(v[j].x) | ((uint32_t)f2bf(v[j].y) << 16); p.y = f2bf(v[j].z) | ((uint32_t)f2bf(v[j].w) << 16);
                *(uint2 *)(s_img + row * PE_RS + 4 + 4 * (threadIdx.x & 31)) = p;
            }
        }
        {
            const int i = threadIdx.x, row = i / 3, col = i - 3 * row;
            if (row < 3 * PE_IH) s_img[row * PE_RS + 1 + col] = f2bf(h);
        }
        __syncthreads();
#pragma unroll
        for (int n = 0; n < NT; ++n) {
            const f32x4 bb = *(const f32x4 *)(bias + 16 * n + 4 * g);
#pragma unroll
            for (int m = 0; m < 2; ++m) acc[m][n] += bb;
        }
        if (t + (int)gridDim.x < n_tiles) load_tile(t + gridDim.x);
#pragma unroll 1
        for (int s = 0; s < 6; ++s) {
            int r = 4 * s + g;
            if (r > 20) r = 20;
            const int c = r / 7, ky = r - 7 * c;
            bf16x8 pb[2];
#pragma unroll
            for (int m = 0; m < 2; ++m) {
                const int oy = wave, ox = 16 * m + l16;
                const uint2 *q = (const uint2 *)(s_img + (c * PE_IH + 4 * oy + ky) * PE_RS + 4 * ox);
                const uint2 lo = q[0], hi = q[1];
                uint4 u; u.x = lo.x; u.y = lo.y; u.z = hi.x; u.w = hi.y;
                pb[m] = *(const bf16x8 *)&u;
            }
#pragma unroll
            for (int n = 0; n < NT; ++n) {
                const bf16x8 wa = *(const bf16x8 *)(s_w + (16 * n + l16) * PE_WS + 32 * s + 8 * g);
#pragma unroll
                for (int m = 0; m < 2; ++m) acc[m][n] = Mfma<bf16x8>::run(wa, pb[m], acc[m][n]);
            }
        }
#pragma unroll
        for (int m = 0; m < 2; ++m) {
            const long long tok = (long long)(oy0 + wave) * S4 + ox0 + 16 * m + l16;
            float *dst = out + ((long long)b * S4 * S4 + tok) * E;
#pragma unroll
            for (int n = 0; n < NT; ++n) {
                float4 o;
                o.x = acc[m][n][0]; o.y = acc[m][n][1]; o.z = acc[m][n][2]; o.w = acc[m][n][3];
                *(float4 *)(dst + 16 * n + 4 * g) = o;
            }
        }
    }
}

template <int NT>
int launch_patch_embed7(const float *img, int S, const void *w, int ldw, const float *bias, const float *pos, float *out, int B, hipStream_t s) {
    const size_t lds = (size_t)(3 * PE_IH * PE_RS + 16 * NT * PE_WS) * 2;
    static bool set = false;
    if (!set) {
        hipError_t e = hipFuncSetAttribute((const void *)k_patch_embed7<NT>, hipFuncAttributeMaxDynamicSharedMemorySize, (int)lds);
        if (e != hipSuccess) { ovo_set_error("ovo_hiera_forward: hipFuncSetAttribute: %s", hipGetErrorString(e)); return OVO_E_LAUNCH; }
        set = true;
    }
    const int S4 = S / 4, n_tiles = B * (S4 / PE_TH) * (S4 / PE_TW);
    const bool prof = ovo_prof_enabled();
    if (prof) {
        const double tok = (double)B * S4 * S4;
        ovo_prof_begin(8, 2.0 * tok * 147.0 * 16 * NT, s); ovo_prof_shape((int)tok, 16 * NT, 147); ovo_prof_flags(1 | 2 | 256);
        ovo_prof_bytes(12.0 * B * S * S + 4.0 * 16 * NT * (tok + (double)S4 * S4));
    }
    k_patch_embed7<NT><<<n_tiles < 512 ? n_tiles : 512, 512, lds, s>>>(img, S, (const uint16_t *)w, ldw, bias, pos, out, B, n_tiles);
    if (prof) ovo_prof_end(s);
    OVO_CHECK_LAUNCH();
    return OVO_OK;
}

int patch_embed_direct(const float *img, int S, int E, const void *w, int ldw, const float *bias, const float *pos, float *out, int B, hipStream_t s) {
    if (ovo_knob_set("OVO_HIERA_PATCH_GEMM")) return OVO_E_UNSUPPORTED;
    if (S % 128 != 0 || ldw < 147) return OVO_E_UNSUPPORTED;
    switch (E) {
        case 96: return launch_patch_embed7<6>(img, S, w, ldw, bias, pos, out, B, s);
        case 112: return launch_patch_embed7<7>(img, S, w, ldw, bias, pos, out, B, s);
        case 144: return launch_patch_embed7<9>(img, S, w, ldw, bias, pos, out, B, s);
        default: return OVO_E_UNSUPPORTED;
    }
}

struct Fwd {
    const ovo_hiera_config_t &c; const ovo_hiera_weights_t &w; const Ws &k;
    int B; float *feat0, *feat1; ovo_stream_t stream; hipStream_t hs;
    float *x, *spare;
    const float *residual;
    bool h_done;
    long long att_rows; int att_kout;
};

int patch_embed(const Plan &p, const float *images, Fwd &f) {
    const ovo_hiera_config_t &c = f.c;
    const long long T0 = (long long)p.S4 * p.S4; bool direct;
    TRY_FUSED(direct, patch_embed_direct(images, c.image_size, c.dims[0], f.w.patch_w, 192, f.w.patch_b, f.w.pos, f.x, f.B, f.hs));
    if (direct) return OVO_OK;
    TRY(ovo_im2col(images, f.B, 3, c.image_size, c.image_size, 7, 4, 3, f.k.col, 192, f.stream));
    for (int b = 0; b < f.B; ++b)
        TRY(gemm(f.k.col + (size_t)b * T0 * 192, 192, f.w.patch_w, 192, f.w.patch_b, f.x + (size_t)b * T0 * c.dims[0], c.dims[0], 0, f.w.pos, c.dims[0], T0,
                 c.dims[0], 192, 0, f.stream));
    return OVO_OK;
}

int skip_path(const BlockShape &s, const ovo_hiera_block_t &L, Fwd &f) {
    f.residual = s.din == s.dout ? f.x : f.spare;
    if (s.din == s.dout) return OVO_OK;
    bool streamed = false;
    if (s.g.ws > 0) {
        const ovo_gemm_t q = gemm_desc(nullptr, s.kin, L.res_w, s.kin, L.res_b, f.spare, s.dout, 0, nullptr, 0, s.g.rows, s.dout, s.kin, 0);
        const ovo_window_t wd = window_of(s.g);
        TRY_FUSED(streamed, ovo_gemm_detail::gemm_f32a_stream(&q, &wd, f.x, s.din, L.ln1_g, L.ln1_b, f.c.ln_eps, 1, 1, f.stream));
    }
    if (!streamed) {
        TRY(gemm_from_f32(f.x, s.g, s.din, s.kin, L.ln1_g, L.ln1_b, f.c.ln_eps, 1, f.k.h, f.h_done, L.res_w, L.res_b, f.k.tmp, s.dout, 0, s.dout, 0, f.stream));
        k_pool_unwindow<<<ovo_grid(s.tok_out * s.dout, 256), 256, 0, f.hs>>>(f.k.tmp, s.g, s.dout, f.spare);
    }
    return OVO_OK;
}

int attention(const BlockShape &s, const ovo_hiera_block_t &L, Fwd &f) {
    const Ws &k = f.k;
    const int dout = s.dout, hd = s.hd;
    if (s.kout != dout && (f.att_rows != s.att_rows || f.att_kout != s.kout)) {
        OVO_HIP(hipMemsetAsync(k.att, 0, (size_t)s.att_rows * s.kout * 2, f.hs));
        f.att_rows = s.att_rows; f.att_kout = s.kout;
    } else if (s.kout == dout) f.att_rows = -1;
    bool fused = false, q_pooled = false;
    if (s.g.ws > 0 && !f.h_done && f.c.q_prescaled)
        TRY_FUSED(fused, ovo_gemm_detail::win_attn_launch(f.x, f.B, s.H, s.H, s.g.ws, s.din, dout, s.heads, s.pool ? 1 : 0, L.ln1_g, L.ln1_b, f.c.ln_eps, L.qkv_w, s.kin,
                                                          L.qkv_b, k.att, s.kout, f.hs));
    if (fused) return OVO_OK;
    if (s.pool && s.g.ws > 0 && !f.h_done) {
        const ovo_gemm_t q = gemm_desc(nullptr, s.kin, L.qkv_w, s.kin, L.qkv_b, k.qkv, 3 * dout, 2, nullptr, 0, s.g.rows, 3 * dout, s.kin, 0);
        const ovo_window_t wd = window_of(s.g);
        TRY_FUSED(q_pooled, ovo_gemm_detail::gemm_f32a_stream(&q, &wd, f.x, s.din, L.ln1_g, L.ln1_b, f.c.ln_eps, 1, 0, f.stream, k.qp, dout));
    }
    if (!q_pooled) TRY(gemm_from_f32(f.x, s.g, s.din, s.kin, L.ln1_g, L.ln1_b, f.c.ln_eps, 1, k.h, f.h_done, L.qkv_w, L.qkv_b, k.qkv, 3 * dout, 2, 3 * dout, 0, f.stream));
    if (s.pool && !q_pooled) {
        const long long total8 = s.att_rows * (dout / 8);
        if (dout % 8 == 0 && total8 < (1ll << 32) - (1ll << 22) && (((uintptr_t)k.qkv | (uintptr_t)k.qp) & 15) == 0)
            k_qpool8<<<ovo_grid(total8, 256, 256 * 16), 256, 0, f.hs>>>(k.qkv, (uint32_t)total8, s.g.wh, s.g.ww, dout, k.qp);
        else k_qpool<<<ovo_grid(s.att_rows * dout, 256), 256, 0, f.hs>>>(k.qkv, s.n_win, s.g.wh, s.g.ww, dout, k.qp);
    }
    ovo_attention_t a = {};
    a.k = k.qkv + dout; a.v = k.qkv + 2 * dout; a.o = k.att;
    a.k_sb = a.v_sb = (int64_t)s.tk * 3 * dout; a.k_sh = a.v_sh = hd; a.k_st = a.v_st = 3 * dout;
// ... 38 lines not shown

int neck_level(const BlockShape &b, Fwd &f) {
    const int s = b.stage_end;
    if (s < 0) return OVO_OK;
    const ovo_hiera_weights_t &w = f.w;
    if (neck_fused(f.c, f.B, s)) {
        TRY(ovo_gemm_detail::neck_stream_launch(f.x, b.tok_out, b.dout, w.neck_w[s], b.kout, w.neck_b[s], f.c.fpn_dim, s == 0 ? w.s0_w : w.s1_w, f.c.fpn_dim,
                                                s == 0 ? w.s0_b : w.s1_b, s == 0 ? f.feat0 : f.feat1, s == 0 ? 32 : 64, f.hs));
        LAUNCHED();
        return OVO_OK;
    }
    bool cast_done = false;
    return gemm_from_f32(f.x, b.gi, b.dout, b.kout, nullptr, nullptr, 0.f, 2, f.k.cast, cast_done, w.neck_w[s], w.neck_b[s], f.k.lat[s], f.c.fpn_dim, 0, f.c.fpn_dim,
                         0, f.stream);
}

int neck_tail(const Plan &p, Fwd &f, float *feat2) {
    const ovo_hiera_config_t &c = f.c; const Ws &k = f.k;
    const int S16 = p.S4 / 4, fd = c.fpn_dim;
    float *top = ((uintptr_t)feat2 & 15) == 0 ? feat2 : k.lat[2];
    k_topdown_add<<<ovo_grid((long long)p.n_lat[2] / 4, 256), 256, 0, f.hs>>>(k.lat[2], k.lat[3], top, f.B, S16, S16, fd);
    LAUNCHED();
    if (top != feat2) OVO_HIP(hipMemcpyAsync(feat2, top, p.n_lat[2] * 4, hipMemcpyDeviceToDevice, f.hs));
    for (int s = 0; s < 2; ++s) {
        float *feat = s ? f.feat1 : f.feat0;
        const int n = s ? 64 : 32;
        bool cast_done = false;
        if (!c.hi_res) OVO_HIP(hipMemcpyAsync(feat, k.lat[s], p.n_lat[s] * 4, hipMemcpyDeviceToDevice, f.hs));
        else if (!neck_fused(c, f.B, s))
            TRY(gemm_from_f32(k.lat[s], p.level[s], fd, fd, nullptr, nullptr, 0.f, 2, k.cast, cast_done, s ? f.w.s1_w : f.w.s0_w, s ? f.w.s1_b : f.w.s0_b, feat, n, 0, n, 0, f.stream));
    }
    LAUNCHED();
    return OVO_OK;
}

}

extern "C" {

size_t ovo_hiera_workspace_bytes(const ovo_hiera_config_t *cfg, int B) {
    if (!cfg || B <= 0) return 0;
    Plan p;
    if (make_plan(*cfg, B, p) != 0) return 0;
    return carve(*cfg, p, B, nullptr).bytes;
}

int ovo_hiera_patch_embed(const float *images, int B, int S, int E, const void *patch_w, int ldw, const float *bias, const float *pos,
                          float *x, ovo_stream_t stream) {
    OVO_REQUIRE(images && patch_w && bias && pos && x && B > 0 && S > 0 && E > 0, "bad argument");
    OVO_REQUIRE((long long)B * (S / 4) * (S / 4) < (1ll << 31) / 256, "too many tokens for one launch");
    return patch_embed_direct(images, S, E, patch_w, ldw, bias, pos, x, B, (hipStream_t)stream);
}

int ovo_hiera_forward(const ovo_hiera_config_t *cfg, const ovo_hiera_weights_t *w, const float *images, int B, float *feat0,
                      float *feat1, float *feat2, void *ws, size_t ws_bytes, ovo_stream_t stream) {
    OVO_REQUIRE(cfg && w && images && feat0 && feat1 && feat2 && ws && B > 0, "null argument");
    const ovo_hiera_config_t &c = *cfg;
    OVO_REQUIRE(c.image_size % 32 == 0 && c.fpn_dim % 32 == 0 && c.n_global >= 0 && c.n_global <= 8, "bad config");
    for (int s = 0; s < 4; ++s)
        OVO_REQUIRE(c.dims[s] % 8 == 0 && c.heads[s] > 0 && c.dims[s] % c.heads[s] == 0 && (c.dims[s] / c.heads[s]) % 8 == 0 &&
                        c.blocks[s] > 0 && c.window[s] > 0, "bad stage config");
    Plan p;
    OVO_REQUIRE(make_plan(c, B, p) == 0, "too many blocks");
    OVO_REQUIRE(w->patch_w && w->patch_b && w->pos && w->blocks, "missing weights");
    for (int i = 0; i < p.n_blocks; ++i) {
        const BlockShape &s = p.b[i];
        OVO_REQUIRE(!s.pool || (s.g.wh % 2 == 0 && s.H % 2 == 0), "query pooling needs even windows");
        OVO_REQUIRE(s.din == s.dout || (w->blocks[i].res_w && w->blocks[i].res_b && s.pool), "stage-change block without projection weights");
        OVO_REQUIRE(s.stage_end < 0 || (w->neck_w[s.stage_end] && w->neck_b[s.stage_end]), "missing neck weights");
    }
    OVO_REQUIRE(!c.hi_res || (w->s0_w && w->s0_b && w->s1_w && w->s1_b), "missing conv_s0 / conv_s1 weights");
    for (int s = 0; s < 2; ++s)
        OVO_REQUIRE(!neck_fused(c, B, s) || (((uintptr_t)(s ? feat1 : feat0) | (uintptr_t)w->neck_w[s] | (uintptr_t)(s ? w->s1_w : w->s0_w)) & 15) == 0,
                    "feat0 / feat1 and the neck weights must be 16-byte aligned");
    const Ws k = carve(c, p, B, ws);
    OVO_REQUIRE(ws_bytes >= k.bytes, "workspace too small");
    Fwd f = {c, *w, k, B, feat0, feat1, stream, (hipStream_t)stream, k.x, k.xr, k.x, false, -1, 0};
    TRY(patch_embed(p, images, f));
    for (int i = 0; i < p.n_blocks; ++i) {
        const BlockShape &s = p.b[i]; const ovo_hiera_block_t &L = w->blocks[i];
        TRY(skip_path(s, L, f));
        TRY(attention(s, L, f));
        TRY(out_projection(s, L, f));
        TRY(mlp(s, L, f));
        TRY(neck_level(s, f));
    }
    return neck_tail(p, f, feat2);
}

}
```

ovo_amd/csrc/vit.hip:

```cpp
#include "common.h"
#include "gemm_common.h"

namespace {

struct Ws {
    uint16_t *col;
    float *patch;
    float *x;
    uint16_t *h;
    uint16_t *qkv;
    uint16_t *att;
    uint16_t *u;
    float *stats;
    size_t bytes;
};

inline size_t align256(size_t v) { return (v + 255) & ~(size_t)255; }

Ws carve(const ovo_vit_config_t &c, int B, void *base) {
    const size_t G = c.image_size / c.patch, P = G * G, T = P + c.n_prefix, M = (size_t)B * T;
    Ws w;
    char *p = (char *)base;
    size_t off = 0;
    auto take = [&](size_t n) { char *r = p ? p + off : nullptr; off += align256(n); return r; };
    w.col = (uint16_t *)take((size_t)B * P * c.kpad * 2);
    w.patch = (float *)take((size_t)B * P * c.width * 4);
    w.x = (float *)take(M * c.width * 4);
    w.h = (uint16_t *)take(M * c.width * 2);
    w.qkv = (uint16_t *)take(M * 3 * c.width * 2);
    w.att = (uint16_t *)take(M * c.width * 2);
    w.u = (uint16_t *)take(M * c.mlp_dim * 2);
    w.stats = (float *)take(M * 16 * 2 * 4);
    w.bytes = off;
    return w;
}

int gemm(const void *A, long long lda, const void *W, long long ldw, const float *bias, void *C, long long ldc, int out_dtype,
         const float *add, long long ld_add, int M, int N, int K, int act, ovo_stream_t s) {
    ovo_gemm_t g;
    g.A = A; g.lda = lda; g.W = W; g.ldw = ldw; g.bias = bias; g.C = C; g.ldc = ldc; g.add = add; g.ld_add = ld_add;
    g.M = M; g.N = N; g.K = K; g.in_dtype = 2; g.out_dtype = out_dtype; g.act = act; g.alpha = 1.0f;
    return ovo_gemm(&g, s);
}

}

#define TRY(call)                  \
    do {                           \
        const int rc__ = (call);   \
        if (rc__ != OVO_OK) return rc__; \
    } while (0)

extern "C" {

size_t ovo_vit_workspace_bytes(const ovo_vit_config_t *cfg, int B) {
    if (!cfg || B <= 0) return 0;
    return carve(*cfg, B, nullptr).bytes;
}

int ovo_vit_forward(const ovo_vit_config_t *cfg, const ovo_vit_weights_t *w, const float *images, int B, float *out,
                    void *ws, size_t ws_bytes, ovo_stream_t stream) {
    OVO_REQUIRE(cfg && w && images && out && ws && B > 0, "null argument");
    const ovo_vit_config_t &c = *cfg;
    OVO_REQUIRE(c.patch > 0 && c.image_size >= c.patch && c.width % c.heads == 0 && c.layers >= 0, "bad config");
    OVO_REQUIRE(c.width % 32 == 0 && c.mlp_dim % 32 == 0 && c.kpad % 32 == 0 && c.kpad >= 3 * c.patch * c.patch, "dims must be multiples of 32");
    OVO_REQUIRE(w->patch_w && w->layers && w->ln_post_g && w->ln_post_b, "missing weights");
    OVO_REQUIRE(c.n_prefix == 0 || w->prefix, "class embedding missing");
    OVO_REQUIRE(!c.pre_ln || (w->ln_pre_g && w->ln_pre_b), "ln_pre weights missing");
    OVO_REQUIRE(!c.use_rope || (w->rope_cos && w->rope_sin), "rope tables missing");
    OVO_REQUIRE(c.pool == 0 || c.pool == 2 || (c.pool == 1 && w->proj_w && c.n_prefix == 1 && c.out_dim % 4 == 0), "pool=1 needs a class token and proj");
    OVO_REQUIRE(c.pool != 2 || (w->map_q && w->map_kv_w && w->map_kv_b && w->map_proj_w && w->map_proj_b && w->map_ln_g && w->map_ln_b &&
                                w->map_fc1_w && w->map_fc1_b && w->map_fc2_w && w->map_fc2_b && c.out_dim == c.width), "pool=2 needs the map_* weights");
    const int G = c.image_size / c.patch, P = G * G, T = P + c.n_prefix, M = B * T, hd = c.width / c.heads;
    OVO_REQUIRE(hd % 8 == 0 && hd <= 128, "head_dim must be a multiple of 8, <= 128");
    Ws k = carve(c, B, ws);
    OVO_REQUIRE(ws_bytes >= k.bytes, "workspace too small");
    const int D = c.width;

    TRY(ovo_im2col(images, B, 3, c.image_size, c.image_size, c.patch, c.patch, 0, k.col, c.kpad, stream));
    TRY(gemm(k.col, c.kpad, w->patch_w, c.kpad, w->patch_b, k.patch, D, 0, nullptr, 0, B * P, D, c.kpad, 0, stream));
    TRY(ovo_vit_embed(k.patch, w->prefix, c.n_prefix, w->pos, B, P, D, c.pre_ln ? w->ln_pre_g : nullptr,
                      c.pre_ln ? w->ln_pre_b : nullptr, c.ln_eps, k.x, stream));

    const float scale = c.q_prescaled ? 0.0f : 1.0f / sqrtf((float)hd);
    namespace gd = ovo_gemm_detail;
    const int fold_env = ovo_knob_int("OVO_VIT_LNFOLD", 1);
    const int parts = gd::gemm_fold_parts(D);
    bool fold = fold_env && c.layers > 0 && parts <= 16 && gd::gemm_fold_ok(M, D, D) && gd::gemm_fold_ok(M, D, c.mlp_dim) && gd::gemm_fold_ok(M, 3 * D, D) &&
                gd::gemm_fold_ok(M, c.mlp_dim, D) && (c.act == 0 || c.act == 1) && (!c.use_rope || hd == 64);
    for (int l = 0; l < c.layers && fold; ++l) {
        const ovo_vit_layer_t &L = w->layers[l];
        fold = L.qkv_wf && L.qkv_bf && L.qkv_cs && L.fc1_wf && L.fc1_bf && L.fc1_cs;
    }
    if (fold) {
        TRY(gd::gemm_fold_rowstats(k.x, D, M, D, k.h, D, k.stats, stream));
        int have = 1;
        for (int l = 0; l < c.layers; ++l) {
            const ovo_vit_layer_t &L = w->layers[l];
            ovo_gemm_t g;
            g.A = k.h; g.lda = D; g.W = L.qkv_wf; g.ldw = D; g.bias = L.qkv_bf; g.C = k.qkv; g.ldc = 3 * D; g.add = nullptr; g.ld_add = 0;
            g.M = M; g.N = 3 * D; g.K = D; g.in_dtype = 2; g.out_dtype = 2; g.act = 0; g.alpha = 1.0f;
            const ovo_rope_t r = {w->rope_cos, w->rope_sin, T, hd, 2 * D, c.n_prefix};
            const gd::FoldIn f1 = {k.stats, M, have, D, L.qkv_cs, c.ln_eps};
            TRY(gd::gemm_fold_consumer(&g, c.use_rope ? &r : nullptr, f1, stream));
            ovo_attention_t a = {};
            a.q = k.qkv; a.k = k.qkv + D; a.v = k.qkv + 2 * D; a.o = k.att;
            a.q_sb = a.k_sb = a.v_sb = (int64_t)T * 3 * D; a.q_sh = a.k_sh = a.v_sh = hd; a.q_st = a.k_st = a.v_st = 3 * D;
            a.o_sb = (int64_t)T * D; a.o_sh = hd; a.o_st = D;
            a.B = B; a.H = c.heads; a.Tq = T; a.Tk = T; a.hd = hd; a.scale = scale;
            TRY(ovo_attention(&a, stream));
            const gd::FoldOut fo = {k.h, D, k.stats, M};
            g.A = k.att; g.lda = D; g.W = L.out_w; g.ldw = D; g.bias = L.out_b; g.C = k.x; g.ldc = D; g.add = k.x; g.ld_add = D;
            g.M = M; g.N = D; g.K = D; g.out_dtype = 0; g.act = 0;
            TRY(gd::gemm_fold_producer(&g, fo, stream));
            have = parts;
            g.A = k.h; g.lda = D; g.W = L.fc1_wf; g.ldw = D; g.bias = L.fc1_bf; g.C = k.u; g.ldc = c.mlp_dim; g.add = nullptr; g.ld_add = 0;
            g.M = M; g.N = c.mlp_dim; g.K = D; g.out_dtype = 2; g.act = c.act;
            const gd::FoldIn f2 = {k.stats, M, have, D, L.fc1_cs, c.ln_eps};
            TRY(gd::gemm_fold_consumer(&g, nullptr, f2, stream));
            if (l + 1 < c.layers) {
                g.A = k.u; g.lda = c.mlp_dim; g.W = L.fc2_w; g.ldw = c.mlp_dim; g.bias = L.fc2_b; g.C = k.x; g.ldc = D; g.add = k.x; g.ld_add = D;
                g.M = M; g.N = D; g.K = c.mlp_dim; g.out_dtype = 0; g.act = 0;
                TRY(gd::gemm_fold_producer(&g, fo, stream));
            } else {
                TRY(gemm(k.u, c.mlp_dim, L.fc2_w, c.mlp_dim, L.fc2_b, k.x, D, 0, k.x, D, M, D, c.mlp_dim, 0, stream));
            }
        }
    }
    for (int l = 0; l < c.layers && !fold; ++l) {
        const ovo_vit_layer_t &L = w->layers[l];
        TRY(ovo_layernorm(k.x, D, M, D, L.ln1_g, L.ln1_b, c.ln_eps, k.h, D, 2, stream));
        if (c.use_rope) {
            ovo_gemm_t g;
            g.A = k.h; g.lda = D; g.W = L.qkv_w; g.ldw = D; g.bias = L.qkv_b; g.C = k.qkv; g.ldc = 3 * D; g.add = nullptr; g.ld_add = 0;
            g.M = M; g.N = 3 * D; g.K = D; g.in_dtype = 2; g.out_dtype = 2; g.act = 0; g.alpha = 1.0f;
            const ovo_rope_t r = {w->rope_cos, w->rope_sin, T, hd, 2 * D, c.n_prefix};
            TRY(ovo_gemm_rope(&g, &r, stream));
        } else {
            TRY(gemm(k.h, D, L.qkv_w, D, L.qkv_b, k.qkv, 3 * D, 2, nullptr, 0, M, 3 * D, D, 0, stream));
        }
        ovo_attention_t a = {};
        a.q = k.qkv; a.k = k.qkv + D; a.v = k.qkv + 2 * D; a.o = k.att;
        a.q_sb = a.k_sb = a.v_sb = (int64_t)T * 3 * D; a.q_sh = a.k_sh = a.v_sh = hd; a.q_st = a.k_st = a.v_st = 3 * D;
        a.o_sb = (int64_t)T * D; a.o_sh = hd; a.o_st = D;
        a.B = B; a.H = c.heads; a.Tq = T; a.Tk = T; a.hd = hd; a.scale = scale;
        TRY(ovo_attention(&a, stream));
        TRY(gemm(k.att, D, L.out_w, D, L.out_b, k.x, D, 0, k.x, D, M, D, D, 0, stream));
        TRY(ovo_layernorm(k.x, D, M, D, L.ln2_g, L.ln2_b, c.ln_eps, k.h, D, 2, stream));
        TRY(gemm(k.h, D, L.fc1_w, D, L.fc1_b, k.u, c.mlp_dim, 2, nullptr, 0, M, c.mlp_dim, D, c.act, stream));
        TRY(gemm(k.u, c.mlp_dim, L.fc2_w, c.mlp_dim, L.fc2_b, k.x, D, 0, k.x, D, M, D, c.mlp_dim, 0, stream));
    }

    if (c.pool == 0) {
        TRY(ovo_layernorm(k.x, D, M, D, w->ln_post_g, w->ln_post_b, c.ln_eps, out, D, 0, stream));
    } else if (c.pool == 2) {
        float *y = k.patch;
        TRY(ovo_layernorm(k.x, D, M, D, w->ln_post_g, w->ln_post_b, c.ln_eps, k.h, D, 2, stream));
        TRY(gemm(k.h, D, w->map_kv_w, D, w->map_kv_b, k.qkv, 2 * D, 2, nullptr, 0, M, 2 * D, D, 0, stream));
        ovo_attention_t a = {};
        a.q = w->map_q; a.k = k.qkv; a.v = k.qkv + D; a.o = k.att;
        a.q_sb = 0; a.q_sh = hd; a.q_st = D;
        a.k_sb = a.v_sb = (int64_t)T * 2 * D; a.k_sh = a.v_sh = hd; a.k_st = a.v_st = 2 * D;
        a.o_sb = D; a.o_sh = hd; a.o_st = D;
        a.B = B; a.H = c.heads; a.Tq = 1; a.Tk = T; a.hd = hd; a.scale = scale;
        TRY(ovo_attention(&a, stream));
        TRY(gemm(k.att, D, w->map_proj_w, D, w->map_proj_b, y, D, 0, nullptr, 0, B, D, D, 0, stream));
        TRY(ovo_layernorm(y, D, B, D, w->map_ln_g, w->map_ln_b, c.ln_eps, k.h, D, 2, stream));
        TRY(gemm(k.h, D, w->map_fc1_w, D, w->map_fc1_b, k.u, c.mlp_dim, 2, nullptr, 0, B, c.mlp_dim, D, c.act, stream));
        TRY(gemm(k.u, c.mlp_dim, w->map_fc2_w, c.mlp_dim, w->map_fc2_b, out, D, 0, y, D, B, D, c.mlp_dim, 0, stream));
    } else {
        TRY(ovo_layernorm(k.x, (int64_t)T * D, B, D, w->ln_post_g, w->ln_post_b, c.ln_eps, k.h, D, 2, stream));
        TRY(gemm(k.h, D, w->proj_w, D, nullptr, out, c.out_dim, 0, nullptr, 0, B, c.out_dim, D, 0, stream));
    }
    return OVO_OK;
}

}
```

ovo_amd/encoders/hiera.py:

```python
from __future__ import annotations

import ctypes as C
from dataclasses import dataclass
from typing import Dict, List, Optional, Tuple

import numpy as np
import torch
import torch.nn.functional as F

from .. import _lib as L

IMAGENET_MEAN = (0.485, 0.456, 0.406)
IMAGENET_STD = (0.229, 0.224, 0.225)


@dataclass(frozen=True)
class HieraSpec:
    name: str
    embed_dim: int
    num_heads: int
    stages: Tuple[int, int, int, int]
    global_blocks: Tuple[int, ...]
    window_spec: Tuple[int, int, int, int]
    pos_bkg: Tuple[int, int]
# ... 158 lines not shown
        self._ws: Optional[torch.Tensor] = None

    def preprocess(self, image: torch.Tensor, out: Optional[torch.Tensor] = None) -> torch.Tensor:
        s = self.spec.image_size
        img = L.dev(image, image.dtype, "image")
        hwc = img.dtype == torch.uint8 and img.shape[-1] == 3 and img.shape[0] != 3
        h, w = (img.shape[0], img.shape[1]) if hwc else (img.shape[1], img.shape[2])
        if out is None:
            out = torch.empty((1, 3, s, s), dtype=torch.float32, device=img.device)
        mean, std = (C.c_float * 3)(*IMAGENET_MEAN), (C.c_float * 3)(*IMAGENET_STD)
        scale = 1.0 / 255.0 if img.dtype == torch.uint8 else 1.0
        L.check(L.load().ovo_resize_normalize(L.ptr(img), 4 if hwc else L.DTYPE_CODE[img.dtype], 3, h, w, 0, 0, h, w, L.ptr(out), s, s, 1, scale,
                                              mean, std, L.stream()))
        return out

    def preprocess_batch(self, images, out: Optional[torch.Tensor] = None) -> torch.Tensor:
        s = self.spec.image_size
        imgs = [L.dev(im, im.dtype, "image") for im in images]
        first = imgs[0]
        if out is None:
            out = torch.empty((len(imgs), 3, s, s), dtype=torch.float32, device=first.device)
        if not all(im.dtype == first.dtype and im.shape == first.shape and im.device == first.device for im in imgs) or first.dtype not in (torch.uint8, torch.float32):
            for k, im in enumerate(imgs):
                self.preprocess(im, out=out[k:k + 1])
            return out
        hwc = first.dtype == torch.uint8 and first.shape[-1] == 3 and first.shape[0] != 3
        h, w = (first.shape[0], first.shape[1]) if hwc else (first.shape[1], first.shape[2])
        mean, std = (C.c_float * 3)(*IMAGENET_MEAN), (C.c_float * 3)(*IMAGENET_STD)
        srcs = (C.c_void_p * len(imgs))(*[im.data_ptr() for im in imgs])
        rect = (C.c_int32 * 4)(0, 0, h, w)
        L.check(L.load().ovo_resize_normalize_batch(srcs, len(imgs), 4 if hwc else L.DTYPE_CODE[first.dtype], 3, h, w, rect, 1, L.ptr(out), s, s, 1,
                                                    1.0 / 255.0 if first.dtype == torch.uint8 else 1.0, mean, std, L.stream()))
        return out

    def forward(self, images: torch.Tensor):
        s = self.spec
        x = L.dev(images, torch.float32, "images")
        b = x.shape[0]
        if tuple(x.shape[1:]) != (3, s.image_size, s.image_size):
            raise L.OvoHipError(f"expected [B, 3, {s.image_size}, {s.image_size}], got {tuple(x.shape)}")
        lib = L.load()
        need = lib.ovo_hiera_workspace_bytes(C.byref(self._cfg), b)
        if self._ws is None or self._ws.numel() < need:
            self._ws = torch.empty(need, dtype=torch.uint8, device=self.device)
        c0, c1 = (32, 64) if self.hi_res else (s.fpn_dim, s.fpn_dim)
        s4 = s.image_size // 4
        f0 = torch.empty((b, s4, s4, c0), dtype=torch.float32, device=x.device)
        f1 = torch.empty((b, s4 // 2, s4 // 2, c1), dtype=torch.float32, device=x.device)
        f2 = torch.empty((b, s4 // 4, s4 // 4, s.fpn_dim), dtype=torch.float32, device=x.device)
        L.check(lib.ovo_hiera_forward(C.byref(self._cfg), C.byref(self._weights), L.ptr(x), b, L.ptr(f0), L.ptr(f1), L.ptr(f2),
                                      L.ptr(self._ws), need, L.stream()))
        return f0, f1, f2

    def encode_frame(self, image):
        if isinstance(image, np.ndarray):
            image = torch.from_numpy(np.ascontiguousarray(image.transpose(2, 0, 1))).to(self.device)
        f0, f1, f2 = self.forward(self.preprocess(image))
        return {"image_embed": f2, "high_res_feats": (f0, f1)}
```

ovo_amd/encoders/vit.py:

```python
from __future__ import annotations

import ctypes as C
import math
import os
from dataclasses import dataclass, field
from typing import Dict, List, Optional, Sequence, Tuple

import torch

from .. import _lib as L

CLIP_MEAN = (0.48145466, 0.4578275, 0.40821073)
CLIP_STD = (0.26862954, 0.26130258, 0.27577711)


@dataclass(frozen=True)
class ViTSpec:
    name: str
    image_size: int
    patch: int
    width: int
    layers: int
    heads: int
    mlp_dim: int
# ... 259 lines not shown
            out = torch.empty((len(imgs) * nc, 3, s.image_size, s.image_size), dtype=torch.float32, device=first.device)
        if not same:
            for i, im in enumerate(imgs):
                self.preprocess(im, given, scale, antialias, out=out[i * nc:(i + 1) * nc])
            return out
        mean, std = (C.c_float * 3)(*s.mean), (C.c_float * 3)(*s.std)
        srcs = (C.c_void_p * len(imgs))(*[im.data_ptr() for im in imgs])
        rects = (C.c_int32 * (4 * nc))(*[int(v) for r in crops for v in r])
        L.check(L.load().ovo_resize_normalize_batch(srcs, len(imgs), 4 if hwc else L.DTYPE_CODE[first.dtype], 3, h, w, rects, nc, L.ptr(out), s.image_size,
                                                    s.image_size, int(antialias), float(scale), mean, std, L.stream()))
        return out

    def clip_window(self, h: int, w: int) -> Tuple[int, int, int, int]:
        S = self.spec.image_size
        if self.spec.resize_mode == "squash":
            return S, S, 0, 0
        vh, vw = (int(S * h / w), S) if w <= h else (S, int(S * w / h))
        return vh, vw, int(round((vh - S) / 2.0)), int(round((vw - S) / 2.0))

    def preprocess_clip(self, images: torch.Tensor, scale: float = 1.0, out: Optional[torch.Tensor] = None) -> torch.Tensor:
        s = self.spec
        x = L.dev(images, images.dtype, "images")
        if x.dtype not in (torch.uint8, torch.float32):
            raise L.OvoHipError("images must be u8 or f32")
        b, _, h, w = x.shape
        if out is None:
            out = torch.empty((b, 3, s.image_size, s.image_size), dtype=torch.float32, device=x.device)
        vh, vw, top, left = self.clip_window(h, w)
        filt = 2 if s.interpolation == "bicubic" else 1
        mean, std = (C.c_float * 3)(*s.mean), (C.c_float * 3)(*s.std)
        lib = L.load()
        for i in range(b):
            L.check(lib.ovo_resize_window_normalize(L.ptr(x[i]), L.DTYPE_CODE[x.dtype], 3, h, w, 0, 0, h, w, L.ptr(out[i]), s.image_size, s.image_size,
                                                    vh, vw, top, left, filt, float(scale), mean, std, L.stream()))
        return out

    def forward(self, images: torch.Tensor, tokens: bool = False, out: Optional[torch.Tensor] = None) -> torch.Tensor:
        s = self.spec
        x = L.dev(images, torch.float32, "images")
        b = x.shape[0]
        if tuple(x.shape[1:]) != (3, s.image_size, s.image_size):
            raise L.OvoHipError(f"expected [B, 3, {s.image_size}, {s.image_size}], got {tuple(x.shape)}")
        cfg = self._config(0 if tokens else (2 if s.map_pool else 1))
        if out is None:
            shape = (b, s.tokens, s.width) if tokens else (b, s.out_dim)
            out = torch.empty(shape, dtype=torch.float32, device=x.device)
        lib = L.load()
        if self.split_streams and b >= 2:
            return self._forward_split(lib, cfg, x, out)
        ws, need = self._workspace(cfg, b)
        L.check(lib.ovo_vit_forward(C.byref(cfg), C.byref(self._weights), L.ptr(x), b, L.ptr(out), L.ptr(ws), need, L.stream()))
        return out

    def _forward_split(self, lib, cfg, x: torch.Tensor, out: torch.Tensor) -> torch.Tensor:
        b = x.shape[0]
        h0 = (b + 1) // 2
        main = torch.cuda.current_stream(x.device)
        if self._side is None:
            self._side = torch.cuda.Stream(device=x.device)
        need0 = lib.ovo_vit_workspace_bytes(C.byref(cfg), h0)
        need1 = lib.ovo_vit_workspace_bytes(C.byref(cfg), b - h0)
        if self._ws2 is None or self._ws2[0].numel() < need0 or self._ws2[1].numel() < need1:
            self._ws2 = (torch.empty(need0, dtype=torch.uint8, device=x.device), torch.empty(max(need1, 1), dtype=torch.uint8, device=x.device))
        self._side.wait_stream(main)
        L.check(lib.ovo_vit_forward(C.byref(cfg), C.byref(self._weights), L.ptr(x[:h0]), h0, L.ptr(out[:h0]), L.ptr(self._ws2[0]), need0, L.stream()))
        with torch.cuda.stream(self._side):
            L.check(lib.ovo_vit_forward(C.byref(cfg), C.byref(self._weights), L.ptr(x[h0:]), b - h0, L.ptr(out[h0:]), L.ptr(self._ws2[1]), need1,
                                        L.stream()))
        main.wait_stream(self._side)
        return out

    encode_image = forward
```

ovo_amd/entities/token_lookahead.py:

```python
from __future__ import annotations

import contextlib
import os
from typing import Dict

import torch

from .. import _lib as L
from ..utils.streams import side_stream


class TokenLookahead:
    def __init__(self, textregion, device) -> None:
        self.tr = textregion
        self.stream = side_stream(device, "OVO_VIT_CUS", int(os.environ.get("OVO_VIT_PRIORITY", "0")))
        self.widest = 0
        self._slots = [dict(batch=None, tokens=None, free=None, left=0) for _ in range(2)]
        self._next = 0
        self.reset()

    def reset(self) -> None:
        for slot in self._slots:
            slot["left"], slot["free"] = 0, None
        self._pending: Dict[int, tuple] = {}
        self._single = None
        self._newest = None
        self._outside = None
        self._last_read = None

    def idle(self) -> bool:
        return not self._pending and all(slot["left"] == 0 for slot in self._slots)

    def encode(self, images, ready=(), stream=None) -> bool:
        images = list(images)
        if not images or not all(isinstance(i, torch.Tensor) and i.is_cuda for i in images):
            return False
        slot = self._slots[self._next]
        if slot["left"] > 0:
            raise L.OvoHipError("TokenLookahead.encode: the batch before the previous one still has unconsumed images")
        self._next ^= 1
        tr, dev = self.tr, images[0].device
        h, w = images[0].shape[:2]
        crops = tr.forward_crops(h, w)
        nc, spec = len(crops), tr.vlm.spec
        n = len(images) * nc
        if slot["batch"] is None or slot["batch"].shape[0] < n:
            slot["batch"] = torch.empty((n, 3, spec.image_size, spec.image_size), dtype=torch.float32, device=dev)
            slot["tokens"] = torch.empty((n, spec.tokens, spec.width), dtype=torch.float32, device=dev)
        side = stream if stream is not None else self.stream
        for ev in (slot["free"], self._outside, *ready):
            if ev is not None:
                side.wait_event(ev)
        slot["free"] = self._outside = None
        with torch.cuda.stream(side):
            srcs = [image if image.dtype == torch.uint8 and image.is_contiguous() else image.permute(2, 0, 1).contiguous() for image in images]
            tr.vlm.preprocess_batch(srcs, crops, scale=1.0 / 255.0, out=slot["batch"][:n])
            tr.vlm.forward(slot["batch"][:n], tokens=True, out=slot["tokens"][:n])
            done = torch.cuda.Event()
            done.record(side)
        slot["left"] = len(images)
        self._newest = done
        self.widest = max(self.widest, len(images))
        for k, image in enumerate(images):
            self._pending[id(image)] = (image, slot["tokens"][k * nc:(k + 1) * nc], done, slot)
        return True

    def encode_one(self, image, ready=None) -> bool:
        if self._single is not None:
            self.discard(self._single)
        after = self._last_read
        if after is None:
            after = torch.cuda.Event()
            after.record()
        if not self.encode([image], [after, ready]):
            return False
        self._single = image
        return True

    def take(self, image):
        if self._single is not None and self._single is not image:
            self.discard(self._single)
        hit = self._pending.get(id(image))
        if hit is None or hit[0] is not image:
            return None
        torch.cuda.current_stream().wait_event(hit[2])
        return hit[1]

    def release(self, image) -> None:
        hit = self._drop(image)
        if hit is not None:
            slot = hit[3]
            slot["free"] = torch.cuda.Event()
            slot["free"].record()
            if slot["left"] == 0:
                self._last_read = slot["free"]

    def discard(self, image) -> None:
        hit = self._drop(image)
        if hit is not None and hit[3]["free"] is None:
            hit[3]["free"] = hit[2]

    def _drop(self, image):
        hit = self._pending.get(id(image))
        if hit is None or hit[0] is not image:
            return None
        del self._pending[id(image)]
        if image is self._single:
            self._single = None
        hit[3]["left"] -= 1
        return hit
# ... 9 lines not shown
```

ovo_amd/pipeline.py:

```python
from __future__ import annotations

import contextlib
import os
import time
from dataclasses import dataclass, field
from typing import Dict, List, Optional

import numpy as np
import torch

from . import _lib as L
from . import parallel, synthetic as syn
from .encoders.hiera import SPECS as HIERA_SPECS, HipHiera
from .encoders.vit import SPECS as VIT_SPECS, HipViT
from .entities.clip_generator import CLIPGenerator
from .entities.dense_map import DenseMap
from .entities.ovo import OVO
from .entities.round_chain import RoundLauncher
from .slam.orbslam import reanchor_map
from .slam.vanilla_mapper import VanillaMapper
from .utils import clip_utils, geometry_utils as G, segment_utils
from .utils.streams import side_stream


# ... 124 lines not shown
        self.last: Dict[str, object] = {}
        self.mask_source = None
        self.mask_exchanges = 0
        self._queued: Dict[int, QueuedRound] = {}
        self.slam.ring_slots(max(64, 4 * self.world + 8))
        self.ovo._track_ring_slots = max(32, 4 * self.world + 8)
        self.pipeline_rounds = not os.environ.get("OVO_NO_ROUND_PIPELINE")
        self.round_launcher = RoundLauncher(self.device)
        self.chain_stream = None if os.environ.get("OVO_NO_CHAIN_STREAM") else torch.cuda.Stream(device=self.device, priority=int(os.environ.get("OVO_CHAIN_PRIORITY", "0")))
        if self.world > 1:
            self.xchg = torch.zeros((self.MAX_DESC, self.D), dtype=torch.float32, device=self.device)
            self._gather(self.xchg)
            torch.cuda.synchronize()

    def exchange_device_ms(self, last: Optional[int] = None) -> Optional[float]:
        ev = self.exchange_events[-last:] if last else self.exchange_events
        return sum(a.elapsed_time(b) for a, b in ev) / len(ev) if ev else None

    def drain(self) -> None:
        for first in sorted(self._queued):
            q = self._queued.pop(first)
            for p in q.pend:
                self.ovo.detect_and_track_finish(p)
            self._record_keyframes(q)
        self.slam.settle()

    def _gather(self, t: torch.Tensor) -> torch.Tensor:
        if self.emulate:
            return t[None].expand(self.world, *t.shape).contiguous()
        return parallel.allgather(t)

    def prime(self, H: int, W: int) -> None:
        if self.encoder_batch <= 1:
            return
        for _ in range(2):
            blank = [Frame(-1 - k, torch.zeros((H, W, 3), dtype=torch.uint8, device=self.device), None, None, None, None, None)
                     for k in range(self.encoder_batch)]
            self._launch_encoders(blank)
            torch.cuda.synchronize()
            if self.ovo.lookahead is not None:
                self.ovo.lookahead.reset()
        self._sam_by_frame.clear(); self._encoded.clear(); self._group_first.clear()

    def _sam_side(self):
        return torch.cuda.current_stream() if self.serial else (self.sam_stream or torch.cuda.current_stream())

    def _launch_encoders(self, group: List[Frame]) -> None:
        if self.sam is not None:
            side = self._sam_side()
            for g in group:
                if g.ready is not None:
                    side.wait_event(g.ready)
            with torch.cuda.stream(side):
                s = self.sam.spec.image_size
                if self._sam_in is None or self._sam_in.shape[0] < len(group):
                    self._sam_in = torch.empty((len(group), 3, s, s), dtype=torch.float32, device=self.device)
                self.sam.preprocess_batch([_hwc(g.rgb) for g in group], out=self._sam_in[:len(group)])
                self.sam_out = self.sam.forward(self._sam_in[:len(group)])
                for k, g in enumerate(group):
                    self._sam_by_frame[g.index] = (self.sam_out, k)
        if self.prefetch:
            self.ovo.prefetch_image_features_batch([g.rgb for g in group], [g.ready for g in group if g.ready is not None],
                                                   stream=torch.cuda.current_stream() if self.serial else None)
        for g in group:
            self._encoded[g.index] = True
        self._group_first[group[0].index] = len(group)

    def _encoders_for(self, f: Frame, mine_upcoming: List[Frame]):
        if self.encoder_batch > 1:
            def width(rem):
                return min(self.encoder_batch, rem)
            if f.index not in self._encoded:
                self._launch_encoders([f] + mine_upcoming[:width(1 + len(mine_upcoming)) - 1])
            n_group = self._group_first.pop(f.index, 0)
            if n_group:
                rest = [g for g in mine_upcoming[n_group - 1:] if g.index not in self._encoded]
                nxt = rest[:width(len(rest))]
                if nxt:
                    self._launch_encoders(nxt)
            self._encoded.pop(f.index, None)
            if self.amg is None:
                return None
            hit = self._sam_by_frame.get(f.index)
            outs, k = hit
            emb = {"image_embed": outs[2][k:k + 1], "high_res_feats": (outs[0][k:k + 1], outs[1][k:k + 1])}
            side = self._sam_side()
            with torch.cuda.stream(side):
                return self.amg.generate_launch(f.rgb, embeddings=emb)
        amg_pending = None
        if self.sam is not None:
            side = self.sam_stream or torch.cuda.current_stream()
            if f.ready is not None:
                side.wait_event(f.ready)
            with torch.cuda.stream(side):
                if self.amg is not None:
                    amg_pending = self.amg.generate_launch(f.rgb)
                else:
                    self.sam_out = self.sam.forward(self.sam.preprocess(_hwc(f.rgb)))
                    self._sam_by_frame[f.index] = (self.sam_out, 0)
        if self.prefetch:
            self.ovo.prefetch_image_features(f.rgb, f.ready)
        return amg_pending

    def step(self, f: Frame, upcoming: Optional[List[Frame]] = None) -> Dict[str, object]:
        if self.world > 1:
            raise L.OvoHipError("several ranks step whole rounds: use step_round()")
        return self.step_round([f], upcoming)

    def step_round(self, group: List[Frame], upcoming: Optional[List[Frame]] = None) -> Dict[str, object]:
        if len(group) != self.world:
            raise L.OvoHipError(f"a round is {self.world} keyframes, got {len(group)}")
# ... 264 lines not shown
```

Before: 478.4 frames/s.

## Fuse frame resize/normalize into encoder patch im2col and add fused embed+stats kernel

Adds frame-direct forward paths for the ViT (CLIP) and Hiera (SAM2) encoders. Resampling and normalisation of the u8 HWC frames now happen inside the im2col / patch-embed kernels, so the full fp32 preprocessed image batch is never written and re-read. A fused embed+layernorm kernel also emits a bf16 copy and per-row sum statistics for the next layer. This cuts memory traffic and kernel launches in preprocessing, at the cost of new code paths and possible rounding differences from sampling directly into bf16.

After: 480.1 frames/s (median of 3 runs). Within noise of the previous version (+0.4%).

```diff
diff --git a/include/ovo_hip.h b/include/ovo_hip.h
--- a/include/ovo_hip.h
+++ b/include/ovo_hip.h
@@ -167,6 +167,12 @@
 int ovo_im2col(const float *img, int B, int C, int H, int W, int ksz, int stride, int pad, void *out, int kpad,
                ovo_stream_t stream);
 
+int ovo_vit_embed_stats(const float *patch, const float *prefix, int n_prefix, const float *pos, int B, int P, int d, const float *gamma,
+                        const float *beta, float eps, float *x, void *xb, float *stats, ovo_stream_t stream);
+
+int ovo_frames_im2col(const void *const *frames_host, int n_src, int H, int W, const int32_t *crops_host, int n_crop, int S, int patch, float scale,
+                      const float *mean3_host, const float *std3_host, void *col, int kpad, ovo_stream_t stream);
+
 int ovo_resize_normalize(const void *src, int src_dtype, int C, int H, int W, int y0, int x0, int ch, int cw,
                          float *out, int oh, int ow, int antialias, float scale, const float *mean3_host,
                          const float *std3_host, ovo_stream_t stream);
@@ -240,6 +246,9 @@
 size_t ovo_vit_workspace_bytes(const ovo_vit_config_t *cfg, int B);
 int ovo_vit_forward(const ovo_vit_config_t *cfg, const ovo_vit_weights_t *w, const float *images, int B, float *out,
                     void *ws, size_t ws_bytes, ovo_stream_t stream);
+int ovo_vit_forward_frames(const ovo_vit_config_t *cfg, const ovo_vit_weights_t *w, const void *const *frames_host, int n_src, int H, int W,
+                           const int32_t *crops_host, int n_crop, float scale, const float *mean3_host, const float *std3_host, float *out, void *ws,
+                           size_t ws_bytes, ovo_stream_t stream);
 
 typedef struct {
     int32_t image_size;
@@ -275,6 +284,12 @@
                           float *x, ovo_stream_t stream);
 int ovo_hiera_forward(const ovo_hiera_config_t *cfg, const ovo_hiera_weights_t *w, const float *images, int B,
                       float *feat0, float *feat1, float *feat2, void *ws, size_t ws_bytes, ovo_stream_t stream);
+int ovo_hiera_patch_embed_frames(const void *const *frames_host, const int32_t *hw_host, int B, int S, int E, float scale, const float *mean3_host,
+                                 const float *std3_host, const void *patch_w, int ldw, const float *bias, const float *pos, float *x, void *scratch,
+                                 size_t scratch_bytes, ovo_stream_t stream);
+int ovo_hiera_forward_frames(const ovo_hiera_config_t *cfg, const ovo_hiera_weights_t *w, const void *const *frames_host, const int32_t *hw_host, int B,
+                             float scale, const float *mean3_host, const float *std3_host, float *feat0, float *feat1, float *feat2, void *ws,
+                             size_t ws_bytes, ovo_stream_t stream);
 
 
 int ovo_row_epilogue(const float *x, int64_t R, int C, const float *base, int64_t base_rows, const float *gamma, const float *beta,
diff --git a/ovo_amd/_lib.py b/ovo_amd/_lib.py
--- a/ovo_amd/_lib.py
+++ b/ovo_amd/_lib.py
@@ -8,7 +8,7 @@
 
 _HERE = os.path.dirname(os.path.abspath(__file__))
 SO_PATH = os.path.join(_HERE, "lib", "libovo_hip.so")
-ABI_VERSION = 20
+ABI_VERSION = 21
 E_UNSUPPORTED = -3
 
 
@@ -187,6 +187,8 @@
     "ovo_layernorm": (_I32, [_P, _I64, _I64, _I32, _P, _P, _F32, _P, _I64, _I32, _P]),
     "ovo_vit_embed": (_I32, [_P, _P, _I32, _P, _I32, _I32, _I32, _P, _P, _F32, _P, _P]),
     "ovo_im2col": (_I32, [_P, _I32, _I32, _I32, _I32, _I32, _I32, _I32, _P, _I32, _P]),
+    "ovo_vit_embed_stats": (_I32, [_P, _P, _I32, _P, _I32, _I32, _I32, _P, _P, _F32, _P, _P, _P, _P]),
+    "ovo_frames_im2col": (_I32, [_P, _I32, _I32, _I32, _P, _I32, _I32, _I32, _F32, _P, _P, _P, _I32, _P]),
     "ovo_resize_normalize": (_I32, [_P, _I32, _I32, _I32, _I32, _I32, _I32, _I32, _I32, _P, _I32, _I32, _I32, _F32,
                                     C.POINTER(C.c_float), C.POINTER(C.c_float), _P]),
     "ovo_resize_normalize_batch": (_I32, [_P, _I32, _I32, _I32, _I32, _I32, _P, _I32, _P, _I32, _I32, _I32, _F32, _P, _P, _P]),
@@ -237,6 +239,9 @@
     "ovo_hiera_workspace_bytes": (_SZ, [C.POINTER(HieraConfig), _I32]),
     "ovo_hiera_forward": (_I32, [C.POINTER(HieraConfig), C.POINTER(HieraWeights), _P, _I32, _P, _P, _P, _P, _SZ, _P]),
     "ovo_hiera_patch_embed": (_I32, [_P, _I32, _I32, _I32, _P, _I32, _P, _P, _P, _P]),
+    "ovo_vit_forward_frames": (_I32, [C.POINTER(VitConfig), C.POINTER(VitWeights), _P, _I32, _I32, _I32, _P, _I32, _F32, _P, _P, _P, _P, _SZ, _P]),
+    "ovo_hiera_patch_embed_frames": (_I32, [_P, _P, _I32, _I32, _I32, _F32, _P, _P, _P, _I32, _P, _P, _P, _P, _SZ, _P]),
+    "ovo_hiera_forward_frames": (_I32, [C.POINTER(HieraConfig), C.POINTER(HieraWeights), _P, _P, _I32, _F32, _P, _P, _P, _P, _P, _P, _SZ, _P]),
     "ovo_eval_cell_keys": (_I32, [_P, _I64, C.POINTER(EvalGrid), _P, _P]),
     "ovo_eval_grid_records": (_I32, [_P, _P, _I64, _P, _P]),
     "ovo_knn5_labels": (_I32, [_P, _P, _I64, C.POINTER(EvalGrid), _P, _P, _I64, _P, _P, _P, _P, _P, _P]),
diff --git a/ovo_amd/csrc/core.hip b/ovo_amd/csrc/core.hip
--- a/ovo_amd/csrc/core.hip
+++ b/ovo_amd/csrc/core.hip
@@ -96,7 +96,7 @@
     return OVO_OK;
 }
 const char *ovo_hip_last_error(void) { return g_err; }
-int ovo_hip_abi_version(void) { return 20; }
+int ovo_hip_abi_version(void) { return 21; }
 
 int ovo_profile_start(void) {
     g_prof.recs.clear();
diff --git a/ovo_amd/csrc/encoder.hip b/ovo_amd/csrc/encoder.hip
--- a/ovo_amd/csrc/encoder.hip
+++ b/ovo_amd/csrc/encoder.hip
@@ -1,6 +1,7 @@
 #include <hip/hip_fp16.h>
 
 #include "common.h"
+#include "resize_tri.h"
 
 namespace {
 
@@ -127,6 +128,74 @@
     }
 }
 
+__global__ void __launch_bounds__(256) k_vit_embed_stats(const float *__restrict__ patch, const float *__restrict__ prefix, int n_prefix,
+                                                         const float *__restrict__ pos, int B, int P, int d, const float *__restrict__ gamma,
+                                                         const float *__restrict__ beta, float eps, float *__restrict__ x, uint16_t *__restrict__ xb,
+                                                         float2 *__restrict__ stats) {
+    constexpr int NV = 4;
+    const int lane = threadIdx.x & 63;
+    const int T = n_prefix + P, d4 = d >> 2;
+    const long long rows = (long long)B * T, waves = (long long)gridDim.x * 4;
+    for (long long r = (long long)blockIdx.x * 4 + (threadIdx.x >> 6); r < rows; r += waves) {
+        const int b = (int)(r / T), t = (int)(r % T);
+        const float *src = t < n_prefix ? prefix + (long long)t * d : patch + ((long long)b * P + (t - n_prefix)) * d;
+        const float *pe = pos ? pos + (long long)t * d : nullptr;
+        float4 v[NV];
+#pragma unroll
+        for (int j = 0; j < NV; ++j) {
+            const int i = lane + 64 * j;
+            v[j] = i < d4 ? ((const float4 *)src)[i] : make_float4(0.f, 0.f, 0.f, 0.f);
+        }
+        if (pe) {
+#pragma unroll
+            for (int j = 0; j < NV; ++j) {
+                const int i = lane + 64 * j;
+                if (i < d4) { const float4 e = ((const float4 *)pe)[i]; v[j].x += e.x; v[j].y += e.y; v[j].z += e.z; v[j].w += e.w; }
+            }
+        }
+        if (gamma) {
+            float s = 0.f;
+#pragma unroll
+            for (int j = 0; j < NV; ++j)
+                if (lane + 64 * j < d4) s += (v[j].x + v[j].y) + (v[j].z + v[j].w);
+            const float mean = wave_sum(s) / (float)d;
+            float q = 0.f;
+#pragma unroll
+            for (int j = 0; j < NV; ++j)
+                if (lane + 64 * j < d4) {
+                    const float a = v[j].x - mean, b2 = v[j].y - mean, c = v[j].z - mean, e2 = v[j].w - mean;
+                    q += (a * a + b2 * b2) + (c * c + e2 * e2);
+                }
+            const float rstd = rsqrtf(wave_sum(q) / (float)d + eps);
+#pragma unroll
+            for (int j = 0; j < NV; ++j) {
+                const int i = lane + 64 * j;
+                if (i < d4) {
+                    const float4 g = ((const float4 *)gamma)[i], bt = ((const float4 *)beta)[i];
+                    const float o0 = (v[j].x - mean) * rstd * g.x + bt.x, o1 = (v[j].y - mean) * rstd * g.y + bt.y;
+                    const float o2 = (v[j].z - mean) * rstd * g.z + bt.z, o3 = (v[j].w - mean) * rstd * g.w + bt.w;
+                    v[j] = make_float4(o0, o1, o2, o3);
+                }
+            }
+        }
+        float s1 = 0.f, s2 = 0.f;
+#pragma unroll
+        for (int j = 0; j < NV; ++j) {
+#pragma clang fp contract(off)
+            const int i = lane + 64 * j;
+            if (i < d4) {
+                ((float4 *)(x + r * d))[i] = v[j];
+                ((uint2 *)(xb + r * d))[i] = pack4_bf16(v[j].x, v[j].y, v[j].z, v[j].w);
+                s1 += (v[j].x + v[j].y) + (v[j].z + v[j].w);
+                s2 += (v[j].x * v[j].x + v[j].y * v[j].y) + (v[j].z * v[j].z + v[j].w * v[j].w);
+            }
+        }
+#pragma unroll
+        for (int o = 32; o > 0; o >>= 1) { s1 += __shfl_xor(s1, o); s2 += __shfl_xor(s2, o); }
+        if (lane == 0) stats[r] = make_float2(s1, s2);
+    }
+}
+
 __global__ void __launch_bounds__(256) k_im2col(const float *__restrict__ img, int B, int C, int H, int W, int ksz, int stride, int pad,
                                                 int oh, int ow, uint16_t *__restrict__ out, int kpad) {
     const uint32_t k8 = (uint32_t)kpad >> 3;
@@ -155,16 +224,10 @@
     }
 }
 
-struct ResizeArgs {
-    const void *src; int src_u8, hwc; int C, H, W, y0, x0, ch, cw, oh, ow, aa;
-    int vh, vw, top, left;
-    float scale, mean[4], std[4];
-};
 __device__ __forceinline__ float src_px(const ResizeArgs &a, int c, int y, int x) {
     const long long i = a.hwc ? ((long long)(a.y0 + y) * a.W + (a.x0 + x)) * a.C + c : ((long long)c * a.H + (a.y0 + y)) * a.W + (a.x0 + x);
     return a.src_u8 ? (float)((const uint8_t *)a.src)[i] : ((const float *)a.src)[i];
 }
-typedef uint32_t __attribute__((aligned(1))) u32_unaligned;
 __device__ __forceinline__ void src_px_all(const ResizeArgs &a, int y, int x, float (&v)[4]) {
     if (a.hwc && a.src_u8 && a.C == 3) {
         const long long i = ((long long)(a.y0 + y) * a.W + (a.x0 + x)) * 3;
@@ -177,7 +240,6 @@
     }
     for (int c = 0; c < a.C; ++c) v[c] = src_px(a, c, y, x);
 }
-__device__ __forceinline__ float tri(float x) { x = fabsf(x); return x < 1.f ? 1.f - x : 0.f; }
 __device__ __forceinline__ float cubic_aa(float x) {
     x = fabsf(x);
     if (x < 1.f) return ((1.5f * x - 2.5f) * x) * x + 1.f;
@@ -262,8 +324,6 @@
 }
 __global__ void __launch_bounds__(256) k_resize_norm(ResizeArgs a, float *__restrict__ out) { resize_norm_body(a, out); }
 
-constexpr int RESIZE_BATCH_MAX = 64;
-struct ResizeBatch { const void *src[RESIZE_BATCH_MAX]; int y0[RESIZE_BATCH_MAX], x0[RESIZE_BATCH_MAX], ch[RESIZE_BATCH_MAX], cw[RESIZE_BATCH_MAX]; };
 __global__ void __launch_bounds__(256) k_resize_norm_batch(ResizeArgs a, ResizeBatch b, float *__restrict__ out) {
     const int z = blockIdx.z;
     a.src = b.src[z]; a.y0 = b.y0[z]; a.x0 = b.x0[z]; a.ch = b.ch[z]; a.cw = b.cw[z];
@@ -278,51 +338,16 @@
     const int wx_ = blockIdx.x * 64 + (threadIdx.x & 63), wy_ = blockIdx.y * 4 + (threadIdx.x >> 6);
     if (wx_ >= a.ow || wy_ >= a.oh) return;
     const int ox = wx_ + a.left, oy = wy_ + a.top;
-    const float sy = (float)ch / (float)a.vh, sx = (float)cw / (float)a.vw;
-    const float supy = sy >= 1.f ? sy : 1.f, supx = sx >= 1.f ? sx : 1.f;
-    const float ivy = sy >= 1.f ? 1.f / sy : 1.f, ivx = sx >= 1.f ? 1.f / sx : 1.f;
-    const float cy = sy * ((float)oy + 0.5f), cx = sx * ((float)ox + 0.5f);
-    int ymin = (int)(cy - supy + 0.5f); ymin = ymin < 0 ? 0 : ymin;
-    int ymax = (int)(cy + supy + 0.5f); ymax = ymax > ch ? ch : ymax;
-    int xmin = (int)(cx - supx + 0.5f); xmin = xmin < 0 ? 0 : xmin;
-    int xmax = (int)(cx + supx + 0.5f); xmax = xmax > cw ? cw : xmax;
-    float wy[T], wx[T], wy_tot = 0.f, wx_tot = 0.f;
-#pragma unroll
-    for (int i = 0; i < T; ++i) {
-        wy[i] = ymin + i < ymax ? tri(((float)(ymin + i) - cy + 0.5f) * ivy) : 0.f;
-        wx[i] = xmin + i < xmax ? tri(((float)(xmin + i) - cx + 0.5f) * ivx) : 0.f;
-        wy_tot += wy[i]; wx_tot += wx[i];
-    }
-#pragma unroll
-    for (int i = 0; i < T; ++i) { wy[i] = wy[i] / wy_tot; wx[i] = wx[i] / wx_tot; }
-    const long long last = (long long)a.H * a.W * 3 - 4;
-    float v0 = 0.f, v1 = 0.f, v2 = 0.f;
-#pragma unroll
-    for (int iy = 0; iy < T; ++iy) {
-        int y = ymin + iy; y = y < ch - 1 ? y : ch - 1;
-        const long long row = (long long)(y0c + y) * a.W + x0c;
-        float r0 = 0.f, r1 = 0.f, r2 = 0.f;
-#pragma unroll
-        for (int ix = 0; ix < T; ++ix) {
-            int x = xmin + ix; x = x < cw - 1 ? x : cw - 1;
-            const long long off = (row + x) * 3;
-            uint32_t w;
-            if (off <= last) w = *(const u32_unaligned *)(src + off);
-            else w = (uint32_t)src[off] | ((uint32_t)src[off + 1] << 8) | ((uint32_t)src[off + 2] << 16);
-            r0 += wx[ix] * (float)(w & 0xffu); r1 += wx[ix] * (float)((w >> 8) & 0xffu); r2 += wx[ix] * (float)((w >> 16) & 0xffu);
-        }
-        v0 += wy[iy] * r0; v1 += wy[iy] * r1; v2 += wy[iy] * r2;
-    }
+    int ymin, xmin;
+    float wy[T], wx[T], v[3];
+    tri_taps<T>(ch, a.vh, oy, ymin, wy);
+    tri_taps<T>(cw, a.vw, ox, xmin, wx);
+    tri_sample<T>(src, a.W, (long long)a.H * a.W * 3 - 4, y0c, x0c, ch, cw, ymin, wy, xmin, wx, a.scale, a.mean, a.std, v);
     float *o = out + (long long)z * 3 * a.oh * a.ow + (long long)wy_ * a.ow + wx_;
     const long long plane = (long long)a.oh * a.ow;
-    o[0] = (v0 * a.scale - a.mean[0]) / a.std[0];
-    o[plane] = (v1 * a.scale - a.mean[1]) / a.std[1];
-    o[2 * plane] = (v2 * a.scale - a.mean[2]) / a.std[2];
-}
-inline int resize_tap_bound(int ch, int cw, int vh, int vw) {
-    const float sy = (float)ch / (float)vh, sx = (float)cw / (float)vw;
-    const float supy = sy >= 1.f ? sy : 1.f, supx = sx >= 1.f ? sx : 1.f;
-    return (int)(2.f * (supy > supx ? supy : supx)) + 1;
+    o[0] = v[0];
+    o[plane] = v[1];
+    o[2 * plane] = v[2];
 }
 inline void launch_resize_batch(const ResizeArgs &a, const ResizeBatch &b, int nz, float *out, hipStream_t s) {
     dim3 grid((a.ow + 63) / 64, (a.oh + 3) / 4, nz);
@@ -332,6 +357,46 @@
     if (!generic && a.hwc && a.src_u8 && a.C == 3 && a.aa == 1 && bound <= 3) k_resize_tri_hwc3<3><<<grid, 256, 0, s>>>(a, b, out);
     else if (!generic && a.hwc && a.src_u8 && a.C == 3 && a.aa == 1 && bound <= 6) k_resize_tri_hwc3<6><<<grid, 256, 0, s>>>(a, b, out);
     else k_resize_norm_batch<<<grid, 256, 0, s>>>(a, b, out);
+}
+
+constexpr int FI_PW = 8, FI_MAXP = 16;
+template <int T>
+__global__ void __launch_bounds__(256) k_frames_im2col(FrameBatch f, Normalise n, int S, int p, int G, uint16_t *__restrict__ col, int kpad) {
+    __shared__ TriTap<T> s_ty[FI_MAXP], s_tx[FI_PW * FI_MAXP];
+    __shared__ uint16_t s_px[3 * FI_MAXP * FI_PW * FI_MAXP];
+    const int z = blockIdx.z, py = blockIdx.y, px0 = blockIdx.x * FI_PW, npx = G - px0 < FI_PW ? G - px0 : FI_PW, cols = npx * p;
+    const int ch = f.ch[z], cw = f.cw[z];
+    for (int i = threadIdx.x; i < p + cols; i += 256) {
+        if (i < p) tri_tap_store<T>(s_ty + i, ch, S, py * p + i);
+        else tri_tap_store<T>(s_tx + (i - p), cw, S, px0 * p + (i - p));
+    }
+    __syncthreads();
+    const uint8_t *src = f.src[z];
+    const long long last = (long long)f.H[z] * f.W[z] * 3 - 4;
+    for (int i = threadIdx.x; i < p * cols; i += 256) {
+        const int ky = i / cols, xg = i - ky * cols;
+        const TriTap<T> ty = s_ty[ky], tx = s_tx[xg];
+        float o[3];
+        tri_sample<T>(src, f.W[z], last, f.y0[z], f.x0[z], ch, cw, ty.first, ty.w, tx.first, tx.w, n.scale, n.mean, n.std, o);
+#pragma unroll
+        for (int c = 0; c < 3; ++c) s_px[(c * p + ky) * cols + xg] = f2bf(o[c]);
+    }
+    __syncthreads();
+    const int k8 = kpad >> 3, pp = p * p, kreal = 3 * pp;
+    uint16_t *rows = col + (((long long)z * G + py) * G + px0) * kpad;
+    for (int i = threadIdx.x; i < npx * k8; i += 256) {
+        const int j = i / k8, kb = (i - j * k8) * 8;
+        int c = kb / pp, rem = kb - c * pp, ky = rem / p, kx = rem - ky * p;
+        uint16_t v[8];
+#pragma unroll
+        for (int e = 0; e < 8; ++e) {
+            v[e] = kb + e < kreal ? s_px[(c * p + ky) * cols + j * p + kx] : (uint16_t)0;
+            if (++kx == p) { kx = 0; if (++ky == p) { ky = 0; ++c; } }
+        }
+        uint4 q;
+        q.x = v[0] | ((uint32_t)v[1] << 16); q.y = v[2] | ((uint32_t)v[3] << 16); q.z = v[4] | ((uint32_t)v[5] << 16); q.w = v[6] | ((uint32_t)v[7] << 16);
+        *(uint4 *)(rows + (long long)j * kpad + kb) = q;
+    }
 }
 
 __global__ void __launch_bounds__(256) k_mask_boxes(const uint8_t *__restrict__ masks, int H, int W, int32_t *__restrict__ boxes) {
@@ -616,6 +681,54 @@
     return OVO_OK;
 }
 
+int ovo_vit_embed_stats(const float *patch, const float *prefix, int n_prefix, const float *pos, int B, int P, int d, const float *gamma,
+                        const float *beta, float eps, float *x, void *xb, float *stats, ovo_stream_t stream) {
+    OVO_REQUIRE(patch && x && xb && stats && B > 0 && P > 0 && d > 0 && d % 4 == 0 && n_prefix >= 0, "bad argument");
+    OVO_REQUIRE(n_prefix == 0 || prefix, "prefix tokens missing");
+    OVO_REQUIRE((gamma == nullptr) == (beta == nullptr), "gamma and beta go together");
+    if (d > 1024 || knob_no_front_fuse()) return OVO_E_UNSUPPORTED;
+    k_vit_embed_stats<<<ovo_grid((long long)B * (n_prefix + P) * 64, 256), 256, 0, (hipStream_t)stream>>>(patch, prefix, n_prefix, pos, B, P, d, gamma, beta, eps, x,
+                                                                                                          (uint16_t *)xb, (float2 *)stats);
+    OVO_CHECK_LAUNCH();
+    return OVO_OK;
+}
+
+int ovo_frames_im2col(const void *const *frames_host, int n_src, int H, int W, const int32_t *crops_host, int n_crop, int S, int patch, float scale,
+                      const float *mean3_host, const float *std3_host, void *col, int kpad, ovo_stream_t stream) {
+    OVO_REQUIRE(frames_host && crops_host && col && n_src > 0 && n_crop > 0 && H > 0 && W > 0 && S > 0 && patch > 0 && S >= patch, "null / empty argument");
+    OVO_REQUIRE(kpad >= 3 * patch * patch && kpad % 8 == 0 && ((uintptr_t)col & 15) == 0, "kpad must cover 3 p^2 and be a multiple of 8, the output 16-byte aligned");
+    int bound = 0;
+    for (int k = 0; k < n_crop; ++k) {
+        const int32_t *r = crops_host + 4 * k;
+        OVO_REQUIRE(r[2] > 0 && r[3] > 0 && r[0] >= 0 && r[1] >= 0 && r[0] + r[2] <= H && r[1] + r[3] <= W, "crop outside the image");
+        const int t = resize_tap_bound(r[2], r[3], S, S);
+        bound = t > bound ? t : bound;
+    }
+    for (int i = 0; i < n_src; ++i) OVO_REQUIRE(frames_host[i], "null source image");
+    const int G = S / patch;
+    if (knob_no_front_fuse() || bound > 6 || patch > FI_MAXP || G > 65535) return OVO_E_UNSUPPORTED;
+    Normalise n;
+    n.scale = scale;
+    for (int c = 0; c < 3; ++c) { n.mean[c] = mean3_host ? mean3_host[c] : 0.f; n.std[c] = std3_host ? std3_host[c] : 1.f; }
+    const int total = n_src * n_crop;
+    for (int z0 = 0; z0 < total; z0 += RESIZE_BATCH_MAX) {
+        const int nz = total - z0 < RESIZE_BATCH_MAX ? total - z0 : RESIZE_BATCH_MAX;
+        FrameBatch f = {};
+        for (int z = 0; z < nz; ++z) {
+            const int i = (z0 + z) / n_crop, k = (z0 + z) % n_crop;
+            f.src[z] = (const uint8_t *)frames_host[i]; f.H[z] = H; f.W[z] = W;
+            f.y0[z] = crops_host[4 * k]; f.x0[z] = crops_host[4 * k + 1]; f.ch[z] = crops_host[4 * k + 2]; f.cw[z] = crops_host[4 * k + 3];
+        }
+        uint16_t *out = (uint16_t *)col + (long long)z0 * G * G * kpad;
+        const dim3 grid((G + FI_PW - 1) / FI_PW, G, nz);
+        const hipStream_t s = (hipStream_t)stream;
+        if (bound <= 3) k_frames_im2col<3><<<grid, 256, 0, s>>>(f, n, S, patch, G, out, kpad);
+        else k_frames_im2col<6><<<grid, 256, 0, s>>>(f, n, S, patch, G, out, kpad);
+    }
+    OVO_CHECK_LAUNCH();
+    return OVO_OK;
+}
+
 int ovo_resize_window_normalize(const void *src, int src_dtype, int C, int H, int W, int y0, int x0, int ch, int cw, float *out,
                                 int oh, int ow, int virt_h, int virt_w, int top, int left, int filter, float scale,
                                 const float *mean3_host, const float *std3_host, ovo_stream_t stream) {
diff --git a/ovo_amd/csrc/hiera.hip b/ovo_amd/csrc/hiera.hip
--- a/ovo_amd/csrc/hiera.hip
+++ b/ovo_amd/csrc/hiera.hip
@@ -1,5 +1,6 @@
 #include <algorithm>
 #include "gemm_common.h"
+#include "resize_tri.h"
 
 namespace {
 
@@ -260,7 +261,7 @@
 }
 struct Ws {
     uint16_t *col; float *x, *xr, *tmp; uint16_t *h, *qkv, *qp, *att, *u, *cast; float *lat[4];
-    size_t bytes;
+    size_t bytes, n_u;
 };
 
 bool neck_fused(const ovo_hiera_config_t &c, int B, int s) {
@@ -283,7 +284,7 @@
     w.qp = (uint16_t *)take(max_att * 2); w.att = (uint16_t *)take(max_att * 2);
     w.u = (uint16_t *)take(max_u * 2); w.cast = (uint16_t *)take(max_cast * 2);
     for (int s = 0; s < 4; ++s) w.lat[s] = neck_fused(c, B, s) ? nullptr : (float *)take(p.n_lat[s] * 4);
-    w.bytes = off;
+    w.bytes = off; w.n_u = max_u;
     return w;
 }
 
@@ -322,9 +323,12 @@
     return ovo_gemm(&q, s);
 }
 
-constexpr int PE_TH = 8, PE_TW = 32, PE_IH = 4 * PE_TH + 3, PE_RS = 136, PE_WS = 200;
-template <int NT>
-__global__ void __launch_bounds__(512) __attribute__((amdgpu_waves_per_eu(4, 4))) k_patch_embed7(const float *__restrict__ img, int S, const uint16_t *__restrict__ w, int ldw,
+constexpr int PE_TH = 8, PE_TW = 32, PE_IH = 4 * PE_TH + 3, PE_IW = 4 * PE_TW + 3, PE_RS = 136, PE_WS = 200;
+struct PeFrames { FrameBatch f; Normalise n; };
+template <int T> struct PeSrc { typedef PeFrames type; };
+template <> struct PeSrc<0> { typedef const float *__restrict__ type; };
+template <int NT, int T = 0>
+__global__ void __launch_bounds__(512) __attribute__((amdgpu_waves_per_eu(4, 4))) k_patch_embed7(typename PeSrc<T>::type img, int S, const uint16_t *__restrict__ w, int ldw,
                                                       const float *__restrict__ bias, const float *__restrict__ pos, float *__restrict__ out, int B,
                                                       int n_tiles) {
     using namespace ovo_gemm_detail;
@@ -332,6 +336,8 @@
     extern __shared__ __attribute__((aligned(16))) unsigned char pe_lds[];
     uint16_t *s_img = (uint16_t *)pe_lds;
     uint16_t *s_w = s_img + 3 * PE_IH * PE_RS;
+    typedef TriTap<(T > 0 ? T : 1)> Tap;
+    Tap *s_ty = (Tap *)(s_w + E * PE_WS), *s_tx = s_ty + PE_IH;
     const int S4 = S >> 2, tiles_x = S4 / PE_TW, n_pos = tiles_x * (S4 / PE_TH);
     for (int i = threadIdx.x; i < E * 24; i += 512) {
         const int e = i / 24, r = i - 24 * e;
@@ -349,35 +355,42 @@
     float4 v[NV];
     float h;
     auto load_tile = [&](int t) {
-        const int tt = t % n_pos, b = t / n_pos;
-        const int oy0 = (tt / tiles_x) * PE_TH, ox0 = (tt % tiles_x) * PE_TW;
-        const int y_first = 4 * oy0 - 3, x_first = 4 * ox0 - 3;
-        const float *src = img + (long long)b * 3 * S * S;
-        const float *col0 = src + 4 * ox0 + 4 * (threadIdx.x & 31);
-#pragma unroll
-        for (int j = 0; j < NV; ++j) {
-            int row = (threadIdx.x >> 5) + 16 * j;
-            if (row > 3 * PE_IH - 1) row = 3 * PE_IH - 1;
-            const int c = row / PE_IH, y = y_first + (row - c * PE_IH);
-            const int yc = y < 0 ? 0 : (y > S - 1 ? S - 1 : y);
-            const float4 u = *(const float4 *)(col0 + (c * S + yc) * S);
-            const bool ok = y == yc;
-            v[j].x = ok ? u.x : 0.f; v[j].y = ok ? u.y : 0.f; v[j].z = ok ? u.z : 0.f; v[j].w = ok ? u.w : 0.f;
-        }
-        {
-            int row = threadIdx.x / 3;
-            const int col = threadIdx.x - 3 * row;
-            if (row > 3 * PE_IH - 1) row = 3 * PE_IH - 1;
-            const int c = row / PE_IH, y = y_first + (row - c * PE_IH), x = x_first + col;
-            const int yc = y < 0 ? 0 : (y > S - 1 ? S - 1 : y), xc = x < 0 ? 0 : x;
-            const float u = src[(c * S + yc) * S + xc];
-            h = (y == yc && x == xc) ? u : 0.f;
+        if constexpr (T == 0) {
+            const int tt = t % n_pos, b = t / n_pos;
+            const int oy0 = (tt / tiles_x) * PE_TH, ox0 = (tt % tiles_x) * PE_TW;
+            const int y_first = 4 * oy0 - 3, x_first = 4 * ox0 - 3;
+            const float *src = img + (long long)b * 3 * S * S;
+            const float *col0 = src + 4 * ox0 + 4 * (threadIdx.x & 31);
+#pragma unroll
+            for (int j = 0; j < NV; ++j) {
+                int row = (threadIdx.x >> 5) + 16 * j;
+                if (row > 3 * PE_IH - 1) row = 3 * PE_IH - 1;
+                const int c = row / PE_IH, y = y_first + (row - c * PE_IH);
+                const int yc = y < 0 ? 0 : (y > S - 1 ? S - 1 : y);
+                const float4 u = *(const float4 *)(col0 + (c * S + yc) * S);
+                const bool ok = y == yc;
+                v[j].x = ok ? u.x : 0.f; v[j].y = ok ? u.y : 0.f; v[j].z = ok ? u.z : 0.f; v[j].w = ok ? u.w : 0.f;
+            }
+            {
+                int row = threadIdx.x / 3;
+                const int col = threadIdx.x - 3 * row;
+                if (row > 3 * PE_IH - 1) row = 3 * PE_IH - 1;
+                const int c = row / PE_IH, y = y_first + (row - c * PE_IH), x = x_first + col;
+                const int yc = y < 0 ? 0 : (y > S - 1 ? S - 1 : y), xc = x < 0 ? 0 : x;
+                const float u = src[(c * S + yc) * S + xc];
+                h = (y == yc && x == xc) ? u : 0.f;
+            }
         }
     };
     if ((int)blockIdx.x < n_tiles) load_tile(blockIdx.x);
     for (int t = blockIdx.x; t < n_tiles; t += gridDim.x) {
         const int tt = t % n_pos, b = t / n_pos;
         const int oy0 = (tt / tiles_x) * PE_TH, ox0 = (tt % tiles_x) * PE_TW;
+        if constexpr (T > 0) {
+            const int y = 4 * oy0 - 3 + (int)threadIdx.x, x = 4 * ox0 - 3 + (int)threadIdx.x - 64;
+            if (threadIdx.x < PE_IH) tri_tap_store<T>(s_ty + threadIdx.x, img.f.ch[b], S, y < 0 ? 0 : (y > S - 1 ? S - 1 : y));
+            else if (threadIdx.x >= 64 && threadIdx.x < 64 + PE_IW) tri_tap_store<T>(s_tx + (threadIdx.x - 64), img.f.cw[b], S, x < 0 ? 0 : x);
+        }
         __syncthreads();
         f32x4 acc[2][NT];
 #pragma unroll
@@ -386,18 +399,35 @@
 #pragma unroll
             for (int n = 0; n < NT; ++n) acc[m][n] = *(const f32x4 *)(pos + tok * E + 16 * n + 4 * g);
         }
-#pragma unroll
-        for (int j = 0; j < NV; ++j) {
-            const int row = (threadIdx.x >> 5) + 16 * j;
-            if (16 * j + 15 < 3 * PE_IH || row < 3 * PE_IH) {
-                uint2 p;
-                p.x = f2bf(v[j].x) | ((uint32_t)f2bf(v[j].y) << 16); p.y = f2bf(v[j].z) | ((uint32_t)f2bf(v[j].w) << 16);
-                *(uint2 *)(s_img + row * PE_RS + 4 + 4 * (threadIdx.x & 31)) = p;
-            }
-        }
-        {
-            const int i = threadIdx.x, row = i / 3, col = i - 3 * row;
-            if (row < 3 * PE_IH) s_img[row * PE_RS + 1 + col] = f2bf(h);
+        if constexpr (T > 0) {
+            const int y_first = 4 * oy0 - 3, x_first = 4 * ox0 - 3;
+            const uint8_t *src = img.f.src[b];
+            const long long last = (long long)img.f.H[b] * img.f.W[b] * 3 - 4;
+#pragma unroll 2
+            for (int p = threadIdx.x; p < PE_IH * PE_IW; p += 512) {
+                const int r = p / PE_IW, c = p - r * PE_IW, y = y_first + r, x = x_first + c;
+                const Tap ty = s_ty[r], tx = s_tx[c];
+                float o[3];
+                tri_sample<T>(src, img.f.W[b], last, img.f.y0[b], img.f.x0[b], img.f.ch[b], img.f.cw[b], ty.first, ty.w, tx.first, tx.w, img.n.scale, img.n.mean,
+                              img.n.std, o);
+                const bool ok = y >= 0 && y < S && x >= 0;
+                uint16_t *d = s_img + r * PE_RS + 1 + c;
+                d[0] = ok ? f2bf(o[0]) : (uint16_t)0; d[PE_IH * PE_RS] = ok ? f2bf(o[1]) : (uint16_t)0; d[2 * PE_IH * PE_RS] = ok ? f2bf(o[2]) : (uint16_t)0;
+            }
+        } else {
+#pragma unroll
+            for (int j = 0; j < NV; ++j) {
+                const int row = (threadIdx.x >> 5) + 16 * j;
+                if (16 * j + 15 < 3 * PE_IH || row < 3 * PE_IH) {
+                    uint2 p;
+                    p.x = f2bf(v[j].x) | ((uint32_t)f2bf(v[j].y) << 16); p.y = f2bf(v[j].z) | ((uint32_t)f2bf(v[j].w) << 16);
+                    *(uint2 *)(s_img + row * PE_RS + 4 + 4 * (threadIdx.x & 31)) = p;
+                }
+            }
+            {
+                const int i = threadIdx.x, row = i / 3, col = i - 3 * row;
+                if (row < 3 * PE_IH) s_img[row * PE_RS + 1 + col] = f2bf(h);
+            }
         }
         __syncthreads();
 #pragma unroll
@@ -442,12 +472,12 @@
     }
 }
 
-template <int NT>
-int launch_patch_embed7(const float *img, int S, const void *w, int ldw, const float *bias, const float *pos, float *out, int B, hipStream_t s) {
-    const size_t lds = (size_t)(3 * PE_IH * PE_RS + 16 * NT * PE_WS) * 2;
+template <int NT, int T>
+int launch_patch_embed7(typename PeSrc<T>::type img, double src_bytes, int S, const void *w, int ldw, const float *bias, const float *pos, float *out, int B, hipStream_t s) {
+    const size_t lds = (size_t)(3 * PE_IH * PE_RS + 16 * NT * PE_WS) * 2 + (T > 0 ? (PE_IH + PE_IW) * sizeof(TriTap<(T > 0 ? T : 1)>) : 0);
     static bool set = false;
     if (!set) {
-        hipError_t e = hipFuncSetAttribute((const void *)k_patch_embed7<NT>, hipFuncAttributeMaxDynamicSharedMemorySize, (int)lds);
+        hipError_t e = hipFuncSetAttribute((const void *)k_patch_embed7<NT, T>, hipFuncAttributeMaxDynamicSharedMemorySize, (int)lds);
         if (e != hipSuccess) { ovo_set_error("ovo_hiera_forward: hipFuncSetAttribute: %s", hipGetErrorString(e)); return OVO_E_LAUNCH; }
         set = true;
     }
@@ -456,23 +486,79 @@
     if (prof) {
         const double tok = (double)B * S4 * S4;
         ovo_prof_begin(8, 2.0 * tok * 147.0 * 16 * NT, s); ovo_prof_shape((int)tok, 16 * NT, 147); ovo_prof_flags(1 | 2 | 256);
-        ovo_prof_bytes(12.0 * B * S * S + 4.0 * 16 * NT * (tok + (double)S4 * S4));
-    }
-    k_patch_embed7<NT><<<n_tiles < 512 ? n_tiles : 512, 512, lds, s>>>(img, S, (const uint16_t *)w, ldw, bias, pos, out, B, n_tiles);
+        ovo_prof_bytes(src_bytes + 4.0 * 16 * NT * (tok + (double)S4 * S4));
+    }
+    k_patch_embed7<NT, T><<<n_tiles < 512 ? n_tiles : 512, 512, lds, s>>>(img, S, (const uint16_t *)w, ldw, bias, pos, out, B, n_tiles);
     if (prof) ovo_prof_end(s);
     OVO_CHECK_LAUNCH();
     return OVO_OK;
 }
 
+template <int T>
+int patch_embed_width(typename PeSrc<T>::type img, double src_bytes, int S, int E, const void *w, int ldw, const float *bias, const float *pos, float *out, int B, hipStream_t s) {
+    if (S % 128 != 0 || ldw < 147) return OVO_E_UNSUPPORTED;
+    switch (E) {
+        case 96: return launch_patch_embed7<6, T>(img, src_bytes, S, w, ldw, bias, pos, out, B, s);
+        case 112: return launch_patch_embed7<7, T>(img, src_bytes, S, w, ldw, bias, pos, out, B, s);
+        case 144: return launch_patch_embed7<9, T>(img, src_bytes, S, w, ldw, bias, pos, out, B, s);
+        default: return OVO_E_UNSUPPORTED;
+    }
+}
 int patch_embed_direct(const float *img, int S, int E, const void *w, int ldw, const float *bias, const float *pos, float *out, int B, hipStream_t s) {
     if (ovo_knob_set("OVO_HIERA_PATCH_GEMM")) return OVO_E_UNSUPPORTED;
-    if (S % 128 != 0 || ldw < 147) return OVO_E_UNSUPPORTED;
-    switch (E) {
-        case 96: return launch_patch_embed7<6>(img, S, w, ldw, bias, pos, out, B, s);
-        case 112: return launch_patch_embed7<7>(img, S, w, ldw, bias, pos, out, B, s);
-        case 144: return launch_patch_embed7<9>(img, S, w, ldw, bias, pos, out, B, s);
-        default: return OVO_E_UNSUPPORTED;
-    }
+    return patch_embed_width<0>(img, 12.0 * B * S * S, S, E, w, ldw, bias, pos, out, B, s);
+}
+
+struct Frames { const void *const *src; const int32_t *hw; float scale; const float *mean, *std; };
+int check_frames(const Frames &f, int B) {
+    OVO_REQUIRE(f.src && f.hw && B > 0, "null / empty frame list");
+    for (int b = 0; b < B; ++b) OVO_REQUIRE(f.src[b] && f.hw[2 * b] > 0 && f.hw[2 * b + 1] > 0, "null / empty frame");
+    return OVO_OK;
+}
+bool frames_fusable(int S, int E, int ldw) { return !knob_no_front_fuse() && S % 128 == 0 && ldw >= 147 && (E == 96 || E == 112 || E == 144); }
+int frame_taps(const Frames &f, int b, int S) {
+    const int bound = resize_tap_bound(f.hw[2 * b], f.hw[2 * b + 1], S, S);
+    return bound <= 3 ? 3 : (bound <= 6 ? 6 : 0);
+}
+int resize_frames(const Frames &f, int b0, int b1, int S, float *img, size_t img_bytes, ovo_stream_t stream) {
+    const size_t per = (size_t)3 * S * S;
+    OVO_REQUIRE(img && (size_t)(b1 - b0) * per * 4 <= img_bytes, "the workspace cannot hold the resized images");
+    for (int r0 = b0, r1; r0 < b1; r0 = r1) {
+        const int H = f.hw[2 * r0], W = f.hw[2 * r0 + 1], rect[4] = {0, 0, H, W};
+        for (r1 = r0 + 1; r1 < b1 && f.hw[2 * r1] == H && f.hw[2 * r1 + 1] == W;) ++r1;
+        TRY(ovo_resize_normalize_batch(f.src + r0, r1 - r0, 4, 3, H, W, rect, 1, img + (r0 - b0) * per, S, S, 1, f.scale, f.mean, f.std, stream));
+    }
+    return OVO_OK;
+}
+int patch_embed_frames(const Frames &f, int S, int E, const void *w, int ldw, const float *bias, const float *pos, float *out, int B, float *scratch,
+                       size_t scratch_bytes, ovo_stream_t stream) {
+    const long long tok = (long long)(S / 4) * (S / 4);
+    for (int b = 0; b < B && !scratch; ++b)
+        if (frame_taps(f, b, S) == 0) return OVO_E_UNSUPPORTED;
+    for (int b0 = 0, b1; b0 < B; b0 = b1) {
+        const bool fused = frame_taps(f, b0, S) != 0;
+        for (b1 = b0 + 1; b1 < B && (frame_taps(f, b1, S) != 0) == fused && (!fused || b1 - b0 < RESIZE_BATCH_MAX);) ++b1;
+        float *o = out + b0 * tok * E;
+        if (!fused) {
+            TRY(resize_frames(f, b0, b1, S, scratch, scratch_bytes, stream));
+            TRY(patch_embed_width<0>(scratch, 12.0 * (b1 - b0) * S * S, S, E, w, ldw, bias, pos, o, b1 - b0, (hipStream_t)stream));
+            continue;
+        }
+        PeFrames a = {};
+        double bytes = 0.0;
+        int taps = 3;
+        for (int i = 0; i < b1 - b0; ++i) {
+            const int H = f.hw[2 * (b0 + i)], W = f.hw[2 * (b0 + i) + 1];
+            a.f.src[i] = (const uint8_t *)f.src[b0 + i]; a.f.H[i] = a.f.ch[i] = H; a.f.W[i] = a.f.cw[i] = W;
+            bytes += 3.0 * H * W;
+            taps = std::max(taps, frame_taps(f, b0 + i, S));
+        }
+        a.n.scale = f.scale;
+        for (int c = 0; c < 3; ++c) { a.n.mean[c] = f.mean ? f.mean[c] : 0.f; a.n.std[c] = f.std ? f.std[c] : 1.f; }
+        TRY(taps == 3 ? patch_embed_width<3>(a, bytes, S, E, w, ldw, bias, pos, o, b1 - b0, (hipStream_t)stream)
+                      : patch_embed_width<6>(a, bytes, S, E, w, ldw, bias, pos, o, b1 - b0, (hipStream_t)stream));
+    }
+    return OVO_OK;
 }
 
 struct Fwd {
@@ -484,8 +570,9 @@
     long long att_rows; int att_kout;
 };
 
-int patch_embed(const Plan &p, const float *images, Fwd &f) {
+int patch_embed(const Plan &p, const float *images, const Frames *frames, Fwd &f) {
     const ovo_hiera_config_t &c = f.c;
+    if (frames) return patch_embed_frames(*frames, c.image_size, c.dims[0], f.w.patch_w, 192, f.w.patch_b, f.w.pos, f.x, f.B, (float *)f.k.u, f.k.n_u * 2, f.stream);
     const long long T0 = (long long)p.S4 * p.S4; bool direct;
     TRY_FUSED(direct, patch_embed_direct(images, c.image_size, c.dims[0], f.w.patch_w, 192, f.w.patch_b, f.w.pos, f.x, f.B, f.hs));
     if (direct) return OVO_OK;
@@ -630,9 +717,23 @@
     return patch_embed_direct(images, S, E, patch_w, ldw, bias, pos, x, B, (hipStream_t)stream);
 }
 
-int ovo_hiera_forward(const ovo_hiera_config_t *cfg, const ovo_hiera_weights_t *w, const float *images, int B, float *feat0,
-                      float *feat1, float *feat2, void *ws, size_t ws_bytes, ovo_stream_t stream) {
-    OVO_REQUIRE(cfg && w && images && feat0 && feat1 && feat2 && ws && B > 0, "null argument");
+int ovo_hiera_patch_embed_frames(const void *const *frames_host, const int32_t *hw_host, int B, int S, int E, float scale, const float *mean3_host,
+                                 const float *std3_host, const void *patch_w, int ldw, const float *bias, const float *pos, float *x, void *scratch,
+                                 size_t scratch_bytes, ovo_stream_t stream) {
+    OVO_REQUIRE(patch_w && bias && pos && x && B > 0 && S > 0 && E > 0, "bad argument");
+    OVO_REQUIRE((long long)B * (S / 4) * (S / 4) < (1ll << 31) / 256, "too many tokens for one launch");
+    const Frames f = {frames_host, hw_host, scale, mean3_host, std3_host};
+    TRY(check_frames(f, B));
+    if (!frames_fusable(S, E, ldw)) return OVO_E_UNSUPPORTED;
+    return patch_embed_frames(f, S, E, patch_w, ldw, bias, pos, x, B, (float *)scratch, scratch_bytes, stream);
+}
+
+}
+
+namespace {
+int hiera_forward(const ovo_hiera_config_t *cfg, const ovo_hiera_weights_t *w, const float *images, const Frames *frames, int B, float *feat0,
+                  float *feat1, float *feat2, void *ws, size_t ws_bytes, ovo_stream_t stream) {
+    OVO_REQUIRE(cfg && w && (images || frames) && feat0 && feat1 && feat2 && ws && B > 0, "null argument");
     const ovo_hiera_config_t &c = *cfg;
     OVO_REQUIRE(c.image_size % 32 == 0 && c.fpn_dim % 32 == 0 && c.n_global >= 0 && c.n_global <= 8, "bad config");
     for (int s = 0; s < 4; ++s)
@@ -653,8 +754,15 @@
                     "feat0 / feat1 and the neck weights must be 16-byte aligned");
     const Ws k = carve(c, p, B, ws);
     OVO_REQUIRE(ws_bytes >= k.bytes, "workspace too small");
+    if (frames) {
+        TRY(check_frames(*frames, B));
+        if (!frames_fusable(c.image_size, c.dims[0], 192)) {
+            TRY(resize_frames(*frames, 0, B, c.image_size, (float *)k.u, k.n_u * 2, stream));
+            images = (const float *)k.u; frames = nullptr;
+        }
+    }
     Fwd f = {c, *w, k, B, feat0, feat1, stream, (hipStream_t)stream, k.x, k.xr, k.x, false, -1, 0};
-    TRY(patch_embed(p, images, f));
+    TRY(patch_embed(p, images, frames, f));
     for (int i = 0; i < p.n_blocks; ++i) {
         const BlockShape &s = p.b[i]; const ovo_hiera_block_t &L = w->blocks[i];
         TRY(skip_path(s, L, f));
@@ -665,5 +773,21 @@
     }
     return neck_tail(p, f, feat2);
 }
-
-}
+}
+
+extern "C" {
+
+int ovo_hiera_forward(const ovo_hiera_config_t *cfg, const ovo_hiera_weights_t *w, const float *images, int B, float *feat0,
+                      float *feat1, float *feat2, void *ws, size_t ws_bytes, ovo_stream_t stream) {
+    OVO_REQUIRE(images, "null argument");
+    return hiera_forward(cfg, w, images, nullptr, B, feat0, feat1, feat2, ws, ws_bytes, stream);
+}
+
+int ovo_hiera_forward_frames(const ovo_hiera_config_t *cfg, const ovo_hiera_weights_t *w, const void *const *frames_host, const int32_t *hw_host, int B,
+                             float scale, const float *mean3_host, const float *std3_host, float *feat0, float *feat1, float *feat2, void *ws,
+                             size_t ws_bytes, ovo_stream_t stream) {
+    const Frames f = {frames_host, hw_host, scale, mean3_host, std3_host};
+    return hiera_forward(cfg, w, nullptr, &f, B, feat0, feat1, feat2, ws, ws_bytes, stream);
+}
+
+}
diff --git a/ovo_amd/csrc/resize_tri.h b/ovo_amd/csrc/resize_tri.h
--- /dev/null
+++ b/ovo_amd/csrc/resize_tri.h
@@ -0,0 +1,84 @@
+#pragma once
+#include "common.h"
+
+inline bool knob_no_front_fuse() { return ovo_knob_set("OVO_NO_FRONT_FUSE"); }
+
+struct ResizeArgs {
+    const void *src; int src_u8, hwc; int C, H, W, y0, x0, ch, cw, oh, ow, aa;
+    int vh, vw, top, left;
+    float scale, mean[4], std[4];
+};
+constexpr int RESIZE_BATCH_MAX = 64;
+struct ResizeBatch { const void *src[RESIZE_BATCH_MAX]; int y0[RESIZE_BATCH_MAX], x0[RESIZE_BATCH_MAX], ch[RESIZE_BATCH_MAX], cw[RESIZE_BATCH_MAX]; };
+struct FrameBatch {
+    const uint8_t *src[RESIZE_BATCH_MAX];
+    int H[RESIZE_BATCH_MAX], W[RESIZE_BATCH_MAX], y0[RESIZE_BATCH_MAX], x0[RESIZE_BATCH_MAX], ch[RESIZE_BATCH_MAX], cw[RESIZE_BATCH_MAX];
+};
+struct Normalise { float scale, mean[3], std[3]; };
+
+typedef uint32_t __attribute__((aligned(1))) u32_unaligned;
+__device__ __forceinline__ float tri(float x) { x = fabsf(x); return x < 1.f ? 1.f - x : 0.f; }
+
+
+template <int T>
+__device__ __forceinline__ void tri_taps(int n, int nv, int o, int &first, float (&w)[T]) {
+#pragma clang fp contract(off)
+    const float s = (float)n / (float)nv;
+    const float sup = s >= 1.f ? s : 1.f;
+    const float iv = s >= 1.f ? 1.f / s : 1.f;
+    const float o5 = (float)o + 0.5f, c = s * o5;
+    int lo = (int)(__builtin_fmaf(s, o5, -sup) + 0.5f); lo = lo < 0 ? 0 : lo;
+    int hi = (int)(c + sup + 0.5f); hi = hi > n ? n : hi;
+    float tot = 0.f;
+#pragma unroll
+    for (int i = 0; i < T; ++i) {
+        w[i] = lo + i < hi ? tri(((float)(lo + i) - c + 0.5f) * iv) : 0.f;
+        tot += w[i];
+    }
+#pragma unroll
+    for (int i = 0; i < T; ++i) w[i] = w[i] / tot;
+    first = lo;
+}
+
+template <int T>
+__device__ __forceinline__ void tri_sample(const uint8_t *__restrict__ src, int W, long long last, int y0c, int x0c, int ch, int cw, int ymin, const float (&wy)[T],
+                                           int xmin, const float (&wx)[T], float scale, const float *mean, const float *std, float (&o)[3]) {
+#pragma clang fp contract(off)
+    float v0 = 0.f, v1 = 0.f, v2 = 0.f;
+#pragma unroll
+    for (int iy = 0; iy < T; ++iy) {
+        int y = ymin + iy; y = y < ch - 1 ? y : ch - 1;
+        const long long row = (long long)(y0c + y) * W + x0c;
+        float r0 = 0.f, r1 = 0.f, r2 = 0.f;
+#pragma unroll
+        for (int ix = 0; ix < T; ++ix) {
+            int x = xmin + ix; x = x < cw - 1 ? x : cw - 1;
+            const long long off = (row + x) * 3;
+            uint32_t w;
+            if (off <= last) w = *(const u32_unaligned *)(src + off);
+            else w = (uint32_t)src[off] | ((uint32_t)src[off + 1] << 8) | ((uint32_t)src[off + 2] << 16);
+            r0 = __builtin_fmaf(wx[ix], (float)(w & 0xffu), r0); r1 = __builtin_fmaf(wx[ix], (float)((w >> 8) & 0xffu), r1);
+            r2 = __builtin_fmaf(wx[ix], (float)((w >> 16) & 0xffu), r2);
+        }
+        v0 = __builtin_fmaf(wy[iy], r0, v0); v1 = __builtin_fmaf(wy[iy], r1, v1); v2 = __builtin_fmaf(wy[iy], r2, v2);
+    }
+    o[0] = __builtin_fmaf(v0, scale, -mean[0]) / std[0];
+    o[1] = __builtin_fmaf(v1, scale, -mean[1]) / std[1];
+    o[2] = __builtin_fmaf(v2, scale, -mean[2]) / std[2];
+}
+
+inline int resize_tap_bound(int ch, int cw, int vh, int vw) {
+    const float sy = (float)ch / (float)vh, sx = (float)cw / (float)vw;
+    const float supy = sy >= 1.f ? sy : 1.f, supx = sx >= 1.f ? sx : 1.f;
+    return (int)(2.f * (supy > supx ? supy : supx)) + 1;
+}
+
+template <int T> struct TriTap { int first; float w[T]; };
+template <int T>
+__device__ __forceinline__ void tri_tap_store(TriTap<T> *e, int n, int nv, int o) {
+    int first; float w[T];
+    tri_taps<T>(n, nv, o, first, w);
+    e->first = first;
+#pragma unroll
+    for (int i = 0; i < T; ++i) e->w[i] = w[i];
+}
diff --git a/ovo_amd/csrc/vit.hip b/ovo_amd/csrc/vit.hip
--- a/ovo_amd/csrc/vit.hip
+++ b/ovo_amd/csrc/vit.hip
@@ -50,6 +50,8 @@
         const int rc__ = (call);   \
         if (rc__ != OVO_OK) return rc__; \
     } while (0)
+#define TRY_FUSED(ran, call) \
+    do { const int rc__ = (call); if (rc__ != OVO_OK && rc__ != OVO_E_UNSUPPORTED) return rc__; (ran) = rc__ == OVO_OK; } while (0)
 
 extern "C" {
 
@@ -58,9 +60,14 @@
     return carve(*cfg, B, nullptr).bytes;
 }
 
-int ovo_vit_forward(const ovo_vit_config_t *cfg, const ovo_vit_weights_t *w, const float *images, int B, float *out,
-                    void *ws, size_t ws_bytes, ovo_stream_t stream) {
-    OVO_REQUIRE(cfg && w && images && out && ws && B > 0, "null argument");
+}
+
+namespace {
+struct Frames { const void *const *src; int n_src, H, W; const int32_t *crops; int n_crop; float scale; const float *mean, *std; };
+
+int vit_forward(const ovo_vit_config_t *cfg, const ovo_vit_weights_t *w, const float *images, const Frames *frames, int B, float *out,
+                void *ws, size_t ws_bytes, ovo_stream_t stream) {
+    OVO_REQUIRE(cfg && w && (images || frames) && out && ws && B > 0, "null argument");
     const ovo_vit_config_t &c = *cfg;
     OVO_REQUIRE(c.patch > 0 && c.image_size >= c.patch && c.width % c.heads == 0 && c.layers >= 0, "bad config");
     OVO_REQUIRE(c.width % 32 == 0 && c.mlp_dim % 32 == 0 && c.kpad % 32 == 0 && c.kpad >= 3 * c.patch * c.patch, "dims must be multiples of 32");
@@ -77,10 +84,18 @@
     OVO_REQUIRE(ws_bytes >= k.bytes, "workspace too small");
     const int D = c.width;
 
-    TRY(ovo_im2col(images, B, 3, c.image_size, c.image_size, c.patch, c.patch, 0, k.col, c.kpad, stream));
+    bool col_done = false;
+    if (frames) {
+        const Frames &f = *frames;
+        TRY_FUSED(col_done, ovo_frames_im2col(f.src, f.n_src, f.H, f.W, f.crops, f.n_crop, c.image_size, c.patch, f.scale, f.mean, f.std, k.col, c.kpad, stream));
+        if (!col_done) {
+            OVO_REQUIRE((size_t)B * 3 * c.image_size * c.image_size * 4 <= (size_t)M * 3 * D * 2, "the workspace cannot hold the resized crops");
+            TRY(ovo_resize_normalize_batch(f.src, f.n_src, 4, 3, f.H, f.W, f.crops, f.n_crop, (float *)k.qkv, c.image_size, c.image_size, 1, f.scale, f.mean, f.std, stream));
+            images = (const float *)k.qkv;
+        }
+    }
+    if (!col_done) TRY(ovo_im2col(images, B, 3, c.image_size, c.image_size, c.patch, c.patch, 0, k.col, c.kpad, stream));
     TRY(gemm(k.col, c.kpad, w->patch_w, c.kpad, w->patch_b, k.patch, D, 0, nullptr, 0, B * P, D, c.kpad, 0, stream));
-    TRY(ovo_vit_embed(k.patch, w->prefix, c.n_prefix, w->pos, B, P, D, c.pre_ln ? w->ln_pre_g : nullptr,
-                      c.pre_ln ? w->ln_pre_b : nullptr, c.ln_eps, k.x, stream));
 
     const float scale = c.q_prescaled ? 0.0f : 1.0f / sqrtf((float)hd);
     namespace gd = ovo_gemm_detail;
@@ -92,8 +107,13 @@
         const ovo_vit_layer_t &L = w->layers[l];
         fold = L.qkv_wf && L.qkv_bf && L.qkv_cs && L.fc1_wf && L.fc1_bf && L.fc1_cs;
     }
+    const float *pre_g = c.pre_ln ? w->ln_pre_g : nullptr, *pre_b = c.pre_ln ? w->ln_pre_b : nullptr;
+    bool stats_done = false;
+    if (frames && fold)
+        TRY_FUSED(stats_done, ovo_vit_embed_stats(k.patch, w->prefix, c.n_prefix, w->pos, B, P, D, pre_g, pre_b, c.ln_eps, k.x, k.h, k.stats, stream));
+    if (!stats_done) TRY(ovo_vit_embed(k.patch, w->prefix, c.n_prefix, w->pos, B, P, D, pre_g, pre_b, c.ln_eps, k.x, stream));
     if (fold) {
-        TRY(gd::gemm_fold_rowstats(k.x, D, M, D, k.h, D, k.stats, stream));
+        if (!stats_done) TRY(gd::gemm_fold_rowstats(k.x, D, M, D, k.h, D, k.stats, stream));
         int have = 1;
         for (int l = 0; l < c.layers; ++l) {
             const ovo_vit_layer_t &L = w->layers[l];
@@ -174,5 +194,22 @@
     }
     return OVO_OK;
 }
-
-}
+}
+
+extern "C" {
+
+int ovo_vit_forward(const ovo_vit_config_t *cfg, const ovo_vit_weights_t *w, const float *images, int B, float *out,
+                    void *ws, size_t ws_bytes, ovo_stream_t stream) {
+    OVO_REQUIRE(images, "null argument");
+    return vit_forward(cfg, w, images, nullptr, B, out, ws, ws_bytes, stream);
+}
+
+int ovo_vit_forward_frames(const ovo_vit_config_t *cfg, const ovo_vit_weights_t *w, const void *const *frames_host, int n_src, int H, int W,
+                           const int32_t *crops_host, int n_crop, float scale, const float *mean3_host, const float *std3_host, float *out, void *ws,
+                           size_t ws_bytes, ovo_stream_t stream) {
+    OVO_REQUIRE(frames_host && crops_host && n_src > 0 && n_crop > 0, "null / empty frame list");
+    const Frames f = {frames_host, n_src, H, W, crops_host, n_crop, scale, mean3_host, std3_host};
+    return vit_forward(cfg, w, nullptr, &f, n_src * n_crop, out, ws, ws_bytes, stream);
+}
+
+}
diff --git a/ovo_amd/encoders/hiera.py b/ovo_amd/encoders/hiera.py
--- a/ovo_amd/encoders/hiera.py
+++ b/ovo_amd/encoders/hiera.py
@@ -234,6 +234,28 @@
                                       L.ptr(self._ws), need, L.stream()))
         return f0, f1, f2
 
+    def forward_frames(self, frames):
+        s = self.spec
+        imgs = [L.dev(im, torch.uint8, "frame") for im in frames]
+        if not all(im.dim() == 3 and im.shape[-1] == 3 for im in imgs):
+            raise L.OvoHipError("forward_frames takes HWC u8 frames")
+        b, dev = len(imgs), imgs[0].device
+        lib = L.load()
+        need = lib.ovo_hiera_workspace_bytes(C.byref(self._cfg), b)
+        if self._ws is None or self._ws.numel() < need:
+            self._ws = torch.empty(need, dtype=torch.uint8, device=self.device)
+        c0, c1 = (32, 64) if self.hi_res else (s.fpn_dim, s.fpn_dim)
+        s4 = s.image_size // 4
+        f0 = torch.empty((b, s4, s4, c0), dtype=torch.float32, device=dev)
+        f1 = torch.empty((b, s4 // 2, s4 // 2, c1), dtype=torch.float32, device=dev)
+        f2 = torch.empty((b, s4 // 4, s4 // 4, s.fpn_dim), dtype=torch.float32, device=dev)
+        srcs = (C.c_void_p * b)(*[im.data_ptr() for im in imgs])
+        hw = (C.c_int32 * (2 * b))(*[int(v) for im in imgs for v in im.shape[:2]])
+        mean, std = (C.c_float * 3)(*IMAGENET_MEAN), (C.c_float * 3)(*IMAGENET_STD)
+        L.check(lib.ovo_hiera_forward_frames(C.byref(self._cfg), C.byref(self._weights), srcs, hw, b, 1.0 / 255.0, mean, std, L.ptr(f0), L.ptr(f1), L.ptr(f2),
+                                             L.ptr(self._ws), need, L.stream()))
+        return f0, f1, f2
+
     def encode_frame(self, image):
         if isinstance(image, np.ndarray):
             image = torch.from_numpy(np.ascontiguousarray(image.transpose(2, 0, 1))).to(self.device)
diff --git a/ovo_amd/encoders/vit.py b/ovo_amd/encoders/vit.py
--- a/ovo_amd/encoders/vit.py
+++ b/ovo_amd/encoders/vit.py
@@ -335,6 +335,29 @@
         L.check(lib.ovo_vit_forward(C.byref(cfg), C.byref(self._weights), L.ptr(x), b, L.ptr(out), L.ptr(ws), need, L.stream()))
         return out
 
+    def forward_frames(self, frames: Sequence[torch.Tensor], crops: Optional[Sequence[Tuple[int, int, int, int]]] = None, scale: float = 1.0,
+                       tokens: bool = False, out: Optional[torch.Tensor] = None) -> torch.Tensor:
+        s = self.spec
+        imgs = [L.dev(im, torch.uint8, "frame") for im in frames]
+        first = imgs[0]
+        if not all(im.dim() == 3 and im.shape == first.shape and im.shape[-1] == 3 and im.device == first.device for im in imgs):
+            raise L.OvoHipError("forward_frames takes HWC u8 frames of one size")
+        if self.split_streams:
+            raise L.OvoHipError("forward_frames has no two-stream form (OVO_VIT_SPLIT): preprocess_batch + forward")
+        h, w = first.shape[:2]
+        crops = list(crops) if crops is not None else [(0, 0, h, w)]
+        b = len(imgs) * len(crops)
+        cfg = self._config(0 if tokens else (2 if s.map_pool else 1))
+        if out is None:
+            out = torch.empty((b, s.tokens, s.width) if tokens else (b, s.out_dim), dtype=torch.float32, device=first.device)
+        ws, need = self._workspace(cfg, b)
+        srcs = (C.c_void_p * len(imgs))(*[im.data_ptr() for im in imgs])
+        rects = (C.c_int32 * (4 * len(crops)))(*[int(v) for r in crops for v in r])
+        mean, std = (C.c_float * 3)(*s.mean), (C.c_float * 3)(*s.std)
+        L.check(L.load().ovo_vit_forward_frames(C.byref(cfg), C.byref(self._weights), srcs, len(imgs), h, w, rects, len(crops), float(scale), mean, std,
+                                                L.ptr(out), L.ptr(ws), need, L.stream()))
+        return out
+
     def _forward_split(self, lib, cfg, x: torch.Tensor, out: torch.Tensor) -> torch.Tensor:
         b = x.shape[0]
         h0 = (b + 1) // 2
diff --git a/ovo_amd/entities/token_lookahead.py b/ovo_amd/entities/token_lookahead.py
--- a/ovo_amd/entities/token_lookahead.py
+++ b/ovo_amd/entities/token_lookahead.py
@@ -44,18 +44,23 @@
         crops = tr.forward_crops(h, w)
         nc, spec = len(crops), tr.vlm.spec
         n = len(images) * nc
-        if slot["batch"] is None or slot["batch"].shape[0] < n:
+        in_place = all(image.dtype == torch.uint8 and image.is_contiguous() for image in images) and not tr.vlm.split_streams
+        if slot["tokens"] is None or slot["tokens"].shape[0] < n:
+            slot["tokens"] = torch.empty((n, spec.tokens, spec.width), dtype=torch.float32, device=dev)
+        if not in_place and (slot["batch"] is None or slot["batch"].shape[0] < n):
             slot["batch"] = torch.empty((n, 3, spec.image_size, spec.image_size), dtype=torch.float32, device=dev)
-            slot["tokens"] = torch.empty((n, spec.tokens, spec.width), dtype=torch.float32, device=dev)
         side = stream if stream is not None else self.stream
         for ev in (slot["free"], self._outside, *ready):
             if ev is not None:
                 side.wait_event(ev)
         slot["free"] = self._outside = None
         with torch.cuda.stream(side):
-            srcs = [image if image.dtype == torch.uint8 and image.is_contiguous() else image.permute(2, 0, 1).contiguous() for image in images]
-            tr.vlm.preprocess_batch(srcs, crops, scale=1.0 / 255.0, out=slot["batch"][:n])
-            tr.vlm.forward(slot["batch"][:n], tokens=True, out=slot["tokens"][:n])
+            if in_place:
+                tr.vlm.forward_frames(images, crops, scale=1.0 / 255.0, tokens=True, out=slot["tokens"][:n])
+            else:
+                srcs = [image if image.dtype == torch.uint8 and image.is_contiguous() else image.permute(2, 0, 1).contiguous() for image in images]
+                tr.vlm.preprocess_batch(srcs, crops, scale=1.0 / 255.0, out=slot["batch"][:n])
+                tr.vlm.forward(slot["batch"][:n], tokens=True, out=slot["tokens"][:n])
             done = torch.cuda.Event()
             done.record(side)
         slot["left"] = len(images)
diff --git a/ovo_amd/pipeline.py b/ovo_amd/pipeline.py
--- a/ovo_amd/pipeline.py
+++ b/ovo_amd/pipeline.py
@@ -200,11 +200,14 @@
                 if g.ready is not None:
                     side.wait_event(g.ready)
             with torch.cuda.stream(side):
-                s = self.sam.spec.image_size
-                if self._sam_in is None or self._sam_in.shape[0] < len(group):
-                    self._sam_in = torch.empty((len(group), 3, s, s), dtype=torch.float32, device=self.device)
-                self.sam.preprocess_batch([_hwc(g.rgb) for g in group], out=self._sam_in[:len(group)])
-                self.sam_out = self.sam.forward(self._sam_in[:len(group)])
+                if all(g.rgb.dtype == torch.uint8 and g.rgb.is_contiguous() for g in group):
+                    self.sam_out = self.sam.forward_frames([g.rgb for g in group])
+                else:
+                    s = self.sam.spec.image_size
+                    if self._sam_in is None or self._sam_in.shape[0] < len(group):
+                        self._sam_in = torch.empty((len(group), 3, s, s), dtype=torch.float32, device=self.device)
+                    self.sam.preprocess_batch([_hwc(g.rgb) for g in group], out=self._sam_in[:len(group)])
+                    self.sam_out = self.sam.forward(self._sam_in[:len(group)])
                 for k, g in enumerate(group):
                     self._sam_by_frame[g.index] = (self.sam_out, k)
         if self.prefetch:
```
